# preon7/2019global

Measured on AMD Instinct MI355X. Metric: Mray/s + ms/frame at 1920x1080, depth 8; %HBM roofline, higher is better.
Workload: dtype f64

## Files before the change

### 2019global_amd/__init__.py

```python
from __future__ import annotations

import ctypes
import os
import threading
from typing import Optional, Sequence

import numpy as np

from . import scenes as _scenes

__all__ = [
    "GIError", "lib", "Camera", "Material", "Octree", "ImpSphere", "ImpTriangle", "ExpQuad",
    "ExpSphere", "ExpCube", "ExpCone", "ExpRectangle", "ExpBox",
    "RayTracer", "DeviceScene", "MODE_R", "MODE_X", "STAT_RAYS", "STAT_NODES", "STAT_PRIMS",
    "STAT_PIXELS", "TILE", "MultiScene", "devices_from_env", "obj_entities", "RAY_DOUBLES",
    "AOV_OUTPUTS", "camera_rays", "camera_rays_device",
    "DenoiseParams", "DENOISE_ALBEDO_STOP", "denoise", "denoise_scratch_bytes", "denoise_device",
    "MOMENTS_OUTPUTS", "DenoiseVarParams", "DENOISE_VAR_OUTPUTS", "DENOISE_VAR_SIGMA_V", "DENOISE_VAR_FLOOR",
    "denoise_var", "denoise_var_scratch_bytes", "denoise_var_device",
]

HERE = os.path.dirname(os.path.abspath(__file__))
LIB_PATH = os.environ.get("GI_LIB") or os.path.join(HERE, "libgi.so")

MODE_R, MODE_X = 0, 1
FLAG_STATS = 1
FLAG_R_DFS = 2
FLAG_TIME = 4
FLAG_X_NO_SHADOW = 8
FLAG_X_WF = 16
FLAG_X_MEGA = 32
FLAG_X_SEG = 64
KAT_X_TREE, KAT_X_HBM = 1, 2
X_FORMS = ("k_mode_x", "k_wf_bounce", "k_seg")
R_KERNELS = ("k_mode_r", "k_rf_walk", "k_mode_r_batch")
STAT_RAYS, STAT_NODES, STAT_PRIMS, STAT_PIXELS, STAT_X_PATH_MAX = 0, 1, 2, 3, 4
STAT_X_ITERS, STAT_X_TRAV, STAT_X_HANDLE, STAT_X_HLANES, STAT_X_HCLOSE, STAT_X_HSHADOW = 5, 6, 7, 8, 9, 10
STAT_X_CYC_TRAV, STAT_X_CYC_HIT, STAT_X_CYC_NEXT, STAT_X_CYC_ALL = 11, 12, 13, 14
STAT_X_RESOLVED = 15
STAT_X_IT_NODE, STAT_X_LN_NODE, STAT_X_IT_LEAF, STAT_X_LN_LEAF = 16, 17, 18, 19
STAT_X_IT_RS, STAT_X_LN_RS, STAT_X_IT_ST, STAT_X_LN_ST = 20, 21, 22, 23
STAT_R_PAIRS, STAT_R_OVF_TILES = 24, 25
STATS_N = 26
TILE = 8
ABI_VERSION = 18
RAY_DOUBLES = 8
AOV_OUTPUTS = ("t", "normal", "albedo", "prim", "entity", "uv")
_AOV_KINDS = {"t": (np.float64, ()), "normal": (np.float64, (3,)), "albedo": (np.float64, (3,)),
              "prim": (np.int32, ()), "entity": (np.int32, ()), "uv": (np.int32, (2,))}


class GIError(RuntimeError):
    pass


class EntityDesc(ctypes.Structure):
    _fields_ = [("kind", ctypes.c_int32), ("has_material", ctypes.c_int32), ("args", ctypes.c_double * 11),
                ("mat_color", ctypes.c_double * 3), ("mat_shader", ctypes.c_double * 3),
                ("mat_specular_power", ctypes.c_double), ("mat_reflectivity", ctypes.c_double)]


class SceneDesc(ctypes.Structure):
    _fields_ = [("octree_min", ctypes.c_double * 3), ("octree_max", ctypes.c_double * 3),
                ("n_entities", ctypes.c_int32), ("entities", ctypes.POINTER(EntityDesc))]


class CameraDesc(ctypes.Structure):
    _fields_ = [("pos", ctypes.c_double * 3), ("up", ctypes.c_double * 3), ("forward", ctypes.c_double * 3),
                ("focal", ctypes.c_double)]


class Opts(ctypes.Structure):
    _fields_ = [("mode", ctypes.c_int32), ("spp", ctypes.c_int32), ("depth", ctypes.c_int32),
                ("shard_count", ctypes.c_int32), ("shard_index", ctypes.c_int32), ("band_rows", ctypes.c_int32),
                ("flags", ctypes.c_uint32), ("reserved", ctypes.c_int32), ("seed", ctypes.c_uint64),
                ("stats", ctypes.c_void_p), ("sample_begin", ctypes.c_int32), ("sample_end", ctypes.c_int32)]


class SceneInfo(ctypes.Structure):
    _fields_ = [("n_entities", ctypes.c_int32), ("n_nodes", ctypes.c_int32), ("n_leaves", ctypes.c_int32),
                ("max_depth", ctypes.c_int32), ("n_reachable", ctypes.c_int32), ("n_dropped", ctypes.c_int32),
                ("x_nodes", ctypes.c_int32), ("x_prims", ctypes.c_int32), ("device_bytes", ctypes.c_int64),
                ("x_node_bytes", ctypes.c_int32), ("x_lds_resident", ctypes.c_int32),
                ("x_flat_leaves", ctypes.c_int32), ("x_fan_leaves", ctypes.c_int32)]


class Hit(ctypes.Structure):
    _fields_ = [("entity", ctypes.c_int32), ("u", ctypes.c_int32), ("v", ctypes.c_int32),
                ("point", ctypes.c_double * 3), ("normal", ctypes.c_double * 3)]


class AovFrame(ctypes.Structure):
    _fields_ = [("w", ctypes.c_int32), ("h", ctypes.c_int32), ("x0", ctypes.c_int32), ("y0", ctypes.c_int32),
                ("x1", ctypes.c_int32), ("y1", ctypes.c_int32)]


class Aov(ctypes.Structure):
    _fields_ = [("t", ctypes.c_void_p), ("normal", ctypes.c_void_p), ("albedo", ctypes.c_void_p),
                ("prim", ctypes.c_void_p), ("entity", ctypes.c_void_p), ("uv", ctypes.c_void_p)]


DENOISE_ALBEDO_STOP = 1
DENOISE_OUTPUTS = ("rgb", "rgb8")


class DenoiseParams(ctypes.Structure):
    _fields_ = [("levels", ctypes.c_int32), ("normal_pow_log2", ctypes.c_int32), ("flags", ctypes.c_uint32),
                ("reserved", ctypes.c_int32), ("sigma_c", ctypes.c_double), ("sigma_p", ctypes.c_double)]


class DenoiseIO(ctypes.Structure):
    _fields_ = [("rgb", ctypes.c_void_p), ("t", ctypes.c_void_p), ("normal", ctypes.c_void_p), ("albedo", ctypes.c_void_p),
                ("out_rgb", ctypes.c_void_p), ("out_rgb8", ctypes.c_void_p)]


MOMENTS_OUTPUTS = ("mean", "var", "samples")


class Moments(ctypes.Structure):
    _fields_ = [("mean", ctypes.c_void_p), ("var", ctypes.c_void_p), ("samples", ctypes.c_void_p)]


DENOISE_VAR_OUTPUTS = ("rgb", "var", "rgb8")
DENOISE_VAR_SIGMA_V = 1.0
DENOISE_VAR_FLOOR = 1e-6


class DenoiseVarParams(ctypes.Structure):
    _fields_ = [("levels", ctypes.c_int32), ("normal_pow_log2", ctypes.c_int32), ("flags", ctypes.c_uint32),
                ("reserved", ctypes.c_int32), ("sigma_v", ctypes.c_double), ("sigma_p", ctypes.c_double),
                ("var_floor", ctypes.c_double)]


class DenoiseVarIO(ctypes.Structure):
    _fields_ = [("rgb", ctypes.c_void_p), ("var", ctypes.c_void_p), ("t", ctypes.c_void_p), ("normal", ctypes.c_void_p),
                ("albedo", ctypes.c_void_p), ("out_rgb", ctypes.c_void_p), ("out_var", ctypes.c_void_p),
                ("out_rgb8", ctypes.c_void_p)]


TILE_CB = ctypes.CFUNCTYPE(None, ctypes.c_void_p, ctypes.c_int, ctypes.c_int, ctypes.POINTER(ctypes.c_uint8),
                           ctypes.POINTER(ctypes.c_double))

EXPORTS = ["gi_abi_version", "gi_last_error", "gi_camera_init", "gi_scene_create", "gi_scene_destroy",
           "gi_scene_get_info", "gi_render", "gi_render_device", "gi_shard_tiles", "gi_unshard_device",
           "gi_trace_ray", "gi_kat_expbox", "gi_kat_x_query", "gi_kat_x_variant", "gi_kat_x_texel", "gi_scene_kernel_ms", "gi_scene_x_form", "gi_scene_seg_ring", "gi_scene_r_kernel", "gi_octree_create", "gi_octree_destroy",
           "gi_octree_intersect", "gi_multi_create", "gi_multi_destroy", "gi_multi_info", "gi_multi_render", "gi_device_count",
           "gi_device_list", "gi_build_id", "gi_obj_parse", "gi_intersect", "gi_occluded", "gi_intersect_device",
           "gi_occluded_device", "gi_render_aov", "gi_render_aov_device", "gi_camera_rays", "gi_camera_rays_device",
           "gi_denoise_scratch_bytes", "gi_denoise_device", "gi_denoise",
           "gi_frame_samples_info", "gi_frame_moments_device", "gi_frame_moments",
           "gi_denoise_var_scratch_bytes", "gi_denoise_var_device", "gi_denoise_var"]

_lib = None
_lock = threading.Lock()


def lib():
    global _lib
    with _lock:
        if _lib is not None:
            return _lib
        if not os.path.exists(LIB_PATH):
            raise GIError(f"{LIB_PATH} is missing: run `python 2019global_amd/build.py` (no CPU fallback)")
        try:
            import torch
        except ImportError:
            pass
        L = ctypes.CDLL(LIB_PATH)
        vp, i32, dp = ctypes.c_void_p, ctypes.c_int, ctypes.POINTER(ctypes.c_double)
        L.gi_abi_version.restype = i32
        L.gi_last_error.restype = ctypes.c_char_p
        L.gi_camera_init.argtypes = [dp, dp, ctypes.c_double, ctypes.POINTER(CameraDesc)]
        L.gi_scene_create.argtypes = [ctypes.POINTER(SceneDesc), ctypes.POINTER(vp)]
        L.gi_scene_destroy.argtypes = [vp]
        L.gi_scene_destroy.restype = None
        L.gi_scene_get_info.argtypes = [vp, ctypes.POINTER(SceneInfo)]
        L.gi_render.argtypes = [vp, ctypes.POINTER(CameraDesc), dp, i32, i32, ctypes.POINTER(Opts), dp,
                                ctypes.POINTER(ctypes.c_uint8), ctypes.POINTER(ctypes.c_int), TILE_CB, vp]
        L.gi_render_device.argtypes = [vp, ctypes.POINTER(CameraDesc), dp, i32, i32, ctypes.POINTER(Opts), vp, vp, vp]
        L.gi_shard_tiles.argtypes = [i32, i32, i32]
        L.gi_shard_tiles.restype = ctypes.c_int64
        L.gi_unshard_device.argtypes = [i32, i32, i32, vp, vp, vp, vp, vp]
        L.gi_trace_ray.argtypes = [vp, dp, dp, dp, ctypes.POINTER(Hit), dp]
        L.gi_kat_expbox.argtypes = [i32, dp, ctypes.POINTER(ctypes.c_int32)]
        ip = ctypes.POINTER(ctypes.c_int32)
        L.gi_kat_x_query.argtypes = [vp, i32, dp, dp, i32, ip, dp, ip, ip, ip, dp, ip, dp]
        L.gi_kat_x_variant.argtypes = [vp, i32, ip]
        L.gi_kat_x_texel.argtypes = [vp, i32, dp, i32, dp, ip]
        i64 = ctypes.c_int64
        L.gi_intersect.argtypes = [vp, i64, dp, dp, ip, ip, dp]
        L.gi_occluded.argtypes = [vp, i64, dp, ip]
        L.gi_intersect_device.argtypes = [vp, i64, vp, vp, vp, vp, vp, vp]
        L.gi_occluded_device.argtypes = [vp, i64, vp, vp, vp]
        L.gi_render_aov.argtypes = [vp, ctypes.POINTER(CameraDesc), ctypes.POINTER(AovFrame), ctypes.POINTER(Aov)]
        L.gi_render_aov_device.argtypes = [vp, ctypes.POINTER(CameraDesc), ctypes.POINTER(AovFrame), ctypes.POINTER(Aov), vp]
        L.gi_camera_rays.argtypes = [ctypes.POINTER(CameraDesc), ctypes.POINTER(AovFrame), dp]
        L.gi_camera_rays_device.argtypes = [ctypes.POINTER(CameraDesc), ctypes.POINTER(AovFrame), vp, vp]
        L.gi_denoise_scratch_bytes.argtypes = [ctypes.POINTER(AovFrame), ctypes.POINTER(DenoiseParams)]
        L.gi_denoise_scratch_bytes.restype = ctypes.c_int64
        L.gi_denoise_device.argtypes = [ctypes.POINTER(CameraDesc), ctypes.POINTER(AovFrame), ctypes.POINTER(DenoiseParams),
                                        ctypes.POINTER(DenoiseIO), vp, ctypes.c_int64, vp]
        L.gi_denoise.argtypes = [ctypes.POINTER(CameraDesc), ctypes.POINTER(AovFrame), ctypes.POINTER(DenoiseParams),
                                 ctypes.POINTER(DenoiseIO)]
        L.gi_frame_samples_info.argtypes = [vp, ip, ip, ip, ip]
        L.gi_frame_moments_device.argtypes = [vp, ctypes.POINTER(AovFrame), ctypes.POINTER(Moments), vp]
        L.gi_frame_moments.argtypes = [vp, ctypes.POINTER(AovFrame), ctypes.POINTER(Moments)]
        L.gi_denoise_var_scratch_bytes.argtypes = [ctypes.POINTER(AovFrame), ctypes.POINTER(DenoiseVarParams)]
        L.gi_denoise_var_scratch_bytes.restype = ctypes.c_int64
        L.gi_denoise_var_device.argtypes = [ctypes.POINTER(CameraDesc), ctypes.POINTER(AovFrame), ctypes.POINTER(DenoiseVarParams),
                                            ctypes.POINTER(DenoiseVarIO), vp, ctypes.c_int64, vp]
        L.gi_denoise_var.argtypes = [ctypes.POINTER(CameraDesc), ctypes.POINTER(AovFrame), ctypes.POINTER(DenoiseVarParams),
                                     ctypes.POINTER(DenoiseVarIO)]
        L.gi_scene_kernel_ms.argtypes = [vp, ctypes.POINTER(ctypes.c_float), ctypes.POINTER(ctypes.c_int64)]
        L.gi_scene_x_form.argtypes = [vp, ctypes.POINTER(Opts), ctypes.POINTER(ctypes.c_int32)]
        L.gi_scene_seg_ring.argtypes = [vp, ctypes.POINTER(Opts), ctypes.POINTER(ctypes.c_int32)]
        L.gi_scene_r_kernel.argtypes = [vp, ctypes.POINTER(Opts), ctypes.POINTER(ctypes.c_int32)]
        L.gi_octree_create.argtypes = [ctypes.POINTER(SceneDesc), ctypes.POINTER(vp)]
        L.gi_octree_destroy.argtypes = [vp]
        L.gi_octree_destroy.restype = None
        L.gi_octree_intersect.argtypes = [vp, dp, dp, ctypes.POINTER(ctypes.c_int32), ctypes.c_int64,
                                          ctypes.POINTER(ctypes.c_int64)]
        L.gi_multi_create.argtypes = [ctypes.POINTER(SceneDesc), i32, ctypes.POINTER(ctypes.c_int), ctypes.POINTER(vp)]
        L.gi_multi_destroy.argtypes = [vp]
        L.gi_multi_destroy.restype = None
        L.gi_multi_info.argtypes = [vp, ctypes.POINTER(ctypes.c_int), ctypes.POINTER(ctypes.c_int),
                                    ctypes.POINTER(ctypes.c_int)]
        L.gi_multi_render.argtypes = [vp, ctypes.POINTER(CameraDesc), dp, i32, i32, ctypes.POINTER(Opts), dp,
                                      ctypes.POINTER(ctypes.c_uint8), ctypes.POINTER(ctypes.c_int), TILE_CB, vp]
        L.gi_device_list.argtypes = [ctypes.POINTER(ctypes.c_int32), i32]
        L.gi_build_id.restype = ctypes.c_char_p
        L.gi_obj_parse.argtypes = [ctypes.c_char_p, ctypes.c_int64, ctypes.POINTER(EntityDesc),
                                   ctypes.POINTER(EntityDesc), ctypes.c_int64, ctypes.POINTER(ctypes.c_int64)]
        if L.gi_abi_version() != ABI_VERSION:
            raise GIError(f"libgi ABI {L.gi_abi_version()} != {ABI_VERSION}")
        _lib = L
        return L


def build_id() -> str:
    return lib().gi_build_id().decode()


def _check(rc: int, what: str) -> None:
    if rc != 0:
        raise GIError(f"{what} failed ({rc}): {lib().gi_last_error().decode()}")


def _check_rays(rays) -> int:
    if not isinstance(rays, np.ndarray) or rays.dtype != np.float64 or rays.ndim != 2 or rays.shape[1] != RAY_DOUBLES or \
            not rays.flags.c_contiguous:
        raise ValueError(f"rays: a C-contiguous float64 array of shape (n, {RAY_DOUBLES}) -- o[3], d[3], tmax, reserved")
    return int(rays.shape[0])


def _aov_frame(w, h, window) -> AovFrame:
    def whole(v):
        return isinstance(v, (int, np.integer)) and not isinstance(v, bool)
    if not (whole(w) and whole(h)) or w <= 0 or h <= 0 or w >= 2 ** 31 or h >= 2 ** 31:
        raise ValueError("frame: w and h are positive integers")
    if window is None:
        window = (0, 0, w, h)
    window = tuple(window)
    if len(window) != 4 or not all(whole(v) for v in window):
        raise ValueError("window: four integers (x0, y0, x1, y1)")
    x0, y0, x1, y1 = (int(v) for v in window)
    if not (0 <= x0 <= x1 <= w and 0 <= y0 <= y1 <= h):
        raise ValueError(f"window {window}: reversed or not inside the {w} x {h} frame")
    return AovFrame(int(w), int(h), x0, y0, x1, y1)


def _d3(v) -> ctypes.Array:
    return (ctypes.c_double * 3)(*[float(x) for x in v])


class Material:

    def __init__(self, color, shader=(0.1, 0.7, 1.0), specular_power: float = 5.0, reflectivity: float = 0.0):
        self.color = tuple(float(c) for c in color)
        self.shader_parameters = tuple(float(c) for c in shader)
        self.specular_power = float(specular_power)
        self.reflectivity = float(reflectivity)


class _Entity:
    kind = 0

    def __init__(self, args: Sequence[float], material: Optional[Material]):
        self._args = tuple(float(a) for a in args)
        self._material = material

    @property
    def material(self) -> Optional[Material]:
        return self._material

    @material.setter
    def material(self, m: Material) -> None:
        self._material = m

    def _desc(self, d: EntityDesc) -> None:
        d.kind = self.kind
        for i, a in enumerate(self._args):
            d.args[i] = a
        m = self._material
        d.has_material = 1 if m is not None else 0
        if m is not None:
            for i in range(3):
                d.mat_color[i] = m.color[i]
                d.mat_shader[i] = m.shader_parameters[i]
            d.mat_specular_power = m.specular_power
            d.mat_reflectivity = m.reflectivity


class ImpSphere(_Entity):
    kind = _scenes.IMP_SPHERE

    def __init__(self, pos, radius, color):
        super().__init__((*pos, radius, *color), None)


class ImpTriangle(_Entity):
    kind = _scenes.IMP_TRIANGLE

    def __init__(self, p1, p2, p3):
        super().__init__((*p1, *p2, *p3), None)


class ExpQuad(_Entity):
    kind = _scenes.EXP_QUAD

    def __init__(self, pos, width, length, alpha, color):
        super().__init__((*pos, width, length, alpha, *color), None)


class ExpSphere(_Entity):
    kind = _scenes.EXP_SPHERE

    def __init__(self, pos, radius, color):
        super().__init__((*pos, radius, *color), None)


class ExpCube(_Entity):
    kind = _scenes.EXP_CUBE

    def __init__(self, pos, width, length, height, color):
        super().__init__((*pos, width, length, height, *color), None)


class ExpCone(_Entity):
    kind = _scenes.EXP_CONE

    def __init__(self, pos, dir, height, radius, color):
        super().__init__((*pos, *dir, height, radius, *color), None)


class ExpRectangle(_Entity):
    kind = _scenes.EXP_RECTANGLE

    def __init__(self, p1, p2, p3):
        super().__init__((*p1, *p2, *p3), None)


class ExpBox(_Entity):
    kind = _scenes.EXP_BOX

    def __init__(self, mn, mx):
        super().__init__((*mn, *mx), None)


# ... 39 lines not shown
        if self._host is None or self._host_gen != self.generation:
            self._close_host()
            d, keep = self._scene_desc()
            h = ctypes.c_void_p()
            _check(L.gi_octree_create(ctypes.byref(d), ctypes.byref(h)), "gi_octree_create")
            del keep
            self._host, self._host_gen = h, self.generation
        dv = np.asarray(direction, np.float64)
        dv = dv * (1.0 / np.sqrt((dv[0] * dv[0] + dv[1] * dv[1]) + dv[2] * dv[2]))
        n = ctypes.c_int64()
        _check(L.gi_octree_intersect(self._host, _d3(origin), _d3(dv), None, 0, ctypes.byref(n)), "gi_octree_intersect")
        out = (ctypes.c_int32 * max(1, n.value))()
        _check(L.gi_octree_intersect(self._host, _d3(origin), _d3(dv), out, n.value, ctypes.byref(n)),
               "gi_octree_intersect")
        return [self.entities[i] for i in out[:n.value]]

    def _close_host(self):
        if self._host is not None and self._host.value:
            lib().gi_octree_destroy(self._host)
        self._host = None

    def __del__(self):
        try:
            self._close_host()
        except Exception:
            pass

    @classmethod
    def from_scene(cls, s: "_scenes.Scene") -> "Octree":
        o = cls(s.octree_min, s.octree_max)
        for e in s.entities:
            ent = _Entity(e.args, None if e.material is None else
                          Material(e.material.color, e.material.shader, e.material.specular_power,
                                   e.material.reflectivity))
            ent.kind = e.kind
            o.push_back(ent)
        return o

    def _scene_desc(self):
        n = len(self.entities)
        arr = (EntityDesc * max(n, 1))()
        for i, e in enumerate(self.entities):
            e._desc(arr[i])
        d = SceneDesc()
        d.octree_min = _d3(self.min)
        d.octree_max = _d3(self.max)
        d.n_entities = n
        d.entities = ctypes.cast(arr, ctypes.POINTER(EntityDesc))
        return d, arr


class Camera:

    def __init__(self, pos, lookAt=(0.0, 0.0, 0.0), focal: float = 0.04):
        self._c = CameraDesc()
        _check(lib().gi_camera_init(_d3(pos), _d3(lookAt), float(focal), ctypes.byref(self._c)), "gi_camera_init")

    @property
    def pos(self):
        return tuple(self._c.pos)

    @property
    def up(self):
        return tuple(self._c.up)

    @property
    def forward(self):
        return tuple(self._c.forward)

    @property
    def focalDist(self):
        return self._c.focal


class DeviceScene:

    def __init__(self, octree: Octree):
        L = lib()
        d, keep = octree._scene_desc()
        h = ctypes.c_void_p()
        _check(L.gi_scene_create(ctypes.byref(d), ctypes.byref(h)), "gi_scene_create")
        self._h = h
        del keep

    @classmethod
    def from_scene(cls, s: "_scenes.Scene") -> "DeviceScene":
        return cls(Octree.from_scene(s))

    def close(self) -> None:
        if getattr(self, "_h", None) and self._h.value:
            lib().gi_scene_destroy(self._h)
            self._h = ctypes.c_void_p()

    def __del__(self):
        try:
            self.close()
        except Exception:
            pass

    def info(self) -> dict:
        i = SceneInfo()
        _check(lib().gi_scene_get_info(self._h, ctypes.byref(i)), "gi_scene_get_info")
        return {f: getattr(i, f) for f, _ in SceneInfo._fields_}

    @staticmethod
    def opts(mode=MODE_R, spp=1, depth=1, seed=0, shard_count=1, shard_index=0, band_rows=0, stats_ptr=0,
             flags=0, samples=None) -> Opts:
        o = Opts()
        o.mode, o.spp, o.depth, o.seed = mode, spp, depth, seed
        o.shard_count, o.shard_index, o.band_rows = shard_count, shard_index, band_rows
        o.flags = (FLAG_STATS if stats_ptr else 0) | flags
        o.stats = stats_ptr or None
        if samples is not None:
            o.sample_begin, o.sample_end = samples
        return o

    def render(self, cam: Camera, light, w: int, h: int, mode=MODE_R, spp=1, depth=1, seed=0, band_rows=0,
               cancel: Optional[ctypes.c_int] = None, callback=None, out=None, flags=0, samples=None):
        if out is None:
            rgb, rgb8 = np.zeros((h, w, 3), np.float64), np.zeros((h, w, 3), np.uint8)
        else:
            rgb, rgb8 = out
        for a, dt in ((rgb, np.float64), (rgb8, np.uint8)):
            if a is not None and (a.dtype != dt or a.size != w * h * 3 or not a.flags.c_contiguous):
                raise ValueError("render: out arrays must be C-contiguous [h, w, 3] float64 / uint8")
        cb = TILE_CB(callback) if callback is not None else TILE_CB()
        o = self.opts(mode, spp, depth, seed, band_rows=band_rows, flags=flags, samples=samples)
        _check(lib().gi_render(self._h, ctypes.byref(cam._c), _d3(light), w, h, ctypes.byref(o),
                               rgb.ctypes.data_as(ctypes.POINTER(ctypes.c_double)) if rgb is not None else None,
                               rgb8.ctypes.data_as(ctypes.POINTER(ctypes.c_uint8)) if rgb8 is not None else None,
                               ctypes.byref(cancel) if cancel is not None else None, cb, None), "gi_render")
        return rgb, rgb8

    def render_device(self, cam: Camera, light, w: int, h: int, d_rgb: int, d_rgb8: int = 0, stream: int = 0,
                      mode=MODE_R, spp=1, depth=1, seed=0, shard_count=1, shard_index=0, stats_ptr=0,
                      flags=0, samples=None) -> None:
        o = self.opts(mode, spp, depth, seed, shard_count, shard_index, stats_ptr=stats_ptr, flags=flags,
                      samples=samples)
        _check(lib().gi_render_device(self._h, ctypes.byref(cam._c), _d3(light), w, h, ctypes.byref(o),
                                      d_rgb or None, d_rgb8 or None, stream or None), "gi_render_device")

    def x_form(self, mode=MODE_X, spp=1, depth=1, flags=0) -> str:
        o = self.opts(mode, spp, depth, 0, flags=flags)
        f = ctypes.c_int32()
        _check(lib().gi_scene_x_form(self._h, ctypes.byref(o), ctypes.byref(f)), "gi_scene_x_form")
        return X_FORMS[f.value]

    def seg_ring(self, mode=MODE_X, spp=1, depth=1, flags=0) -> bool:
        o = self.opts(mode, spp, depth, 0, flags=flags)
        f = ctypes.c_int32()
        _check(lib().gi_scene_seg_ring(self._h, ctypes.byref(o), ctypes.byref(f)), "gi_scene_seg_ring")
        return bool(f.value)

    def r_kernel(self, flags=0) -> str:
        o = self.opts(MODE_R, 1, 1, 0, flags=flags)
        k = ctypes.c_int32()
        _check(lib().gi_scene_r_kernel(self._h, ctypes.byref(o), ctypes.byref(k)), "gi_scene_r_kernel")
        return R_KERNELS[k.value]

    def kernel_ms(self):
        ms, n = ctypes.c_float(), ctypes.c_int64()
        _check(lib().gi_scene_kernel_ms(self._h, ctypes.byref(ms), ctypes.byref(n)), "gi_scene_kernel_ms")
        return float(ms.value), int(n.value)

    def trace_ray(self, origin, direction, light):
        hit = Hit()
        rgb = (ctypes.c_double * 3)()
        _check(lib().gi_trace_ray(self._h, _d3(origin), _d3(direction), _d3(light), ctypes.byref(hit), rgb),
               "gi_trace_ray")
        return hit, tuple(rgb)

    INTERSECT_OUTPUTS = ("t", "prim", "entity", "normal")

    def intersect(self, rays: np.ndarray, want=INTERSECT_OUTPUTS) -> dict:
        n = _check_rays(rays)
        want = tuple(want)
        if not want or any(k not in self.INTERSECT_OUTPUTS for k in want) or len(set(want)) != len(want):
            raise ValueError(f"intersect: want is a non-empty selection of {self.INTERSECT_OUTPUTS}")
        m = max(n, 1)
        bufs = {"t": np.empty(m, np.float64), "prim": np.empty(m, np.int32), "entity": np.empty(m, np.int32),
                "normal": np.empty((m, 3), np.float64)}
        ip, dp = ctypes.POINTER(ctypes.c_int32), ctypes.POINTER(ctypes.c_double)
        ptr = {k: (bufs[k].ctypes.data_as(dp if bufs[k].dtype == np.float64 else ip) if k in want else None)
               for k in self.INTERSECT_OUTPUTS}
        _check(lib().gi_intersect(self._h, n, rays.ctypes.data_as(dp), ptr["t"], ptr["prim"], ptr["entity"], ptr["normal"]),
               "gi_intersect")
        return {k: bufs[k][:n] for k in want}

    def occluded(self, rays: np.ndarray) -> np.ndarray:
        n = _check_rays(rays)
        out = np.empty(max(n, 1), np.int32)
        _check(lib().gi_occluded(self._h, n, rays.ctypes.data_as(ctypes.POINTER(ctypes.c_double)),
                                 out.ctypes.data_as(ctypes.POINTER(ctypes.c_int32))), "gi_occluded")
        return out[:n]

    def intersect_device(self, n: int, d_rays: int, d_t: int = 0, d_prim: int = 0, d_entity: int = 0, d_normal: int = 0,
                         stream: int = 0) -> None:
        _check(lib().gi_intersect_device(self._h, int(n), d_rays or None, d_t or None, d_prim or None, d_entity or None,
                                         d_normal or None, stream or None), "gi_intersect_device")

    def occluded_device(self, n: int, d_rays: int, d_occluded: int, stream: int = 0) -> None:
        _check(lib().gi_occluded_device(self._h, int(n), d_rays or None, d_occluded or None, stream or None),
               "gi_occluded_device")

    def render_aov(self, cam: "Camera", w: int, h: int, window=None, want=AOV_OUTPUTS) -> dict:
        want = tuple(want)
        if not want or any(k not in AOV_OUTPUTS for k in want) or len(set(want)) != len(want):
            raise ValueError(f"render_aov: want is a non-empty selection of {AOV_OUTPUTS}")
        f = _aov_frame(w, h, window)
        rows, cols = f.y1 - f.y0, f.x1 - f.x0
        bufs = {k: np.empty((rows, cols) + _AOV_KINDS[k][1], _AOV_KINDS[k][0]) for k in want}
        a = Aov(**{k: bufs[k].ctypes.data if bufs[k].size else _scratch_ptr() for k in want})
        _check(lib().gi_render_aov(self._h, ctypes.byref(cam._c), ctypes.byref(f), ctypes.byref(a)), "gi_render_aov")
        return bufs

    def render_aov_device(self, cam: "Camera", w: int, h: int, window=None, d_t: int = 0, d_normal: int = 0,
                          d_albedo: int = 0, d_prim: int = 0, d_entity: int = 0, d_uv: int = 0, stream: int = 0) -> None:
        f = _aov_frame(w, h, window)
        a = Aov(d_t or None, d_normal or None, d_albedo or None, d_prim or None, d_entity or None, d_uv or None)
        _check(lib().gi_render_aov_device(self._h, ctypes.byref(cam._c), ctypes.byref(f), ctypes.byref(a), stream or None),
               "gi_render_aov_device")

    def frame_samples_info(self) -> dict:
        v = [ctypes.c_int32() for _ in range(4)]
        _check(lib().gi_frame_samples_info(self._h, *(ctypes.byref(x) for x in v)), "gi_frame_samples_info")
        return dict(zip(("w", "h", "n", "spp"), (int(x.value) for x in v)))

    def frame_moments(self, w: int, h: int, window=None, want=("mean", "var")) -> dict:
        want = tuple(want)
        if not want or any(k not in MOMENTS_OUTPUTS for k in want) or len(set(want)) != len(want):
            raise ValueError(f"frame_moments: want is a non-empty selection of {MOMENTS_OUTPUTS}")
        f = _aov_frame(w, h, window)
        rows, cols = f.y1 - f.y0, f.x1 - f.x0
        n = self.frame_samples_info()["n"] if "samples" in want else 0
        bufs = {k: np.empty((rows, cols, n, 3) if k == "samples" else (rows, cols, 3), np.float64) for k in want}
        m = Moments(**{k: bufs[k].ctypes.data if bufs[k].size else _scratch_ptr() for k in want})
        _check(lib().gi_frame_moments(self._h, ctypes.byref(f), ctypes.byref(m)), "gi_frame_moments")
        return bufs

    def frame_moments_device(self, w: int, h: int, window=None, d_mean: int = 0, d_var: int = 0, d_samples: int = 0,
                             stream: int = 0) -> None:
        f = _aov_frame(w, h, window)
        m = Moments(d_mean or None, d_var or None, d_samples or None)
        _check(lib().gi_frame_moments_device(self._h, ctypes.byref(f), ctypes.byref(m), stream or None), "gi_frame_moments_device")

    def kat_x_variant(self, flags: int = 0) -> dict:
        out = (ctypes.c_int32 * 6)()
        _check(lib().gi_kat_x_variant(self._h, int(flags), out), "gi_kat_x_variant")
        return dict(zip(("LDS", "W4", "SH", "TRI", "CN", "FLAT"), (bool(v) for v in out)))

    def kat_x_query(self, recs: np.ndarray, cam_pos, flags: int = 0) -> dict:
        recs = np.ascontiguousarray(recs, np.float64).reshape(-1, 12)
        n = recs.shape[0]
        out = dict(prim1=np.zeros(n, np.int32), t1=np.zeros(n), occl=np.zeros(n, np.int32), skip_s=np.zeros(n, np.int32),
                   prim2=np.zeros(n, np.int32), t2=np.zeros(n), skip2=np.zeros(n, np.int32))
        sc = ctypes.c_double(float("nan"))
        ip, dp = ctypes.POINTER(ctypes.c_int32), ctypes.POINTER(ctypes.c_double)
        _check(lib().gi_kat_x_query(self._h, n, recs.ctypes.data_as(dp), _d3(cam_pos), int(flags),
                                    out["prim1"].ctypes.data_as(ip), out["t1"].ctypes.data_as(dp),
                                    out["occl"].ctypes.data_as(ip), out["skip_s"].ctypes.data_as(ip),
                                    out["prim2"].ctypes.data_as(ip), out["t2"].ctypes.data_as(dp),
                                    out["skip2"].ctypes.data_as(ip), ctypes.byref(sc)), "gi_kat_x_query")
        out["skip_cos"] = sc.value if n else None
        return out

    def kat_x_texel(self, ents, points, exact: bool = False):
        pts = np.ascontiguousarray(points, np.float64).reshape(-1, 3)
        n = pts.shape[0]
        recs = np.empty((n, 4), np.float64)
        recs[:, 0] = np.asarray(ents, np.float64).reshape(n)
        recs[:, 1:] = pts
        tex, how = np.zeros((n, 3)), np.zeros(n, np.int32)
        ip, dp = ctypes.POINTER(ctypes.c_int32), ctypes.POINTER(ctypes.c_double)
        _check(lib().gi_kat_x_texel(self._h, n, recs.ctypes.data_as(dp), 1 if exact else 0, tex.ctypes.data_as(dp),
                                    how.ctypes.data_as(ip)), "gi_kat_x_texel")
        return tex, how


_scratch = None


def _scratch_ptr() -> int:
    global _scratch
    if _scratch is None:
        _scratch = np.zeros(8)
    return _scratch.ctypes.data


def camera_rays(cam: "Camera", w: int, h: int, window=None) -> np.ndarray:
    f = _aov_frame(w, h, window)
    rays = np.empty(((f.y1 - f.y0) * (f.x1 - f.x0), RAY_DOUBLES), np.float64)
    p = rays.ctypes.data_as(ctypes.POINTER(ctypes.c_double)) if rays.size else \
        ctypes.cast(_scratch_ptr(), ctypes.POINTER(ctypes.c_double))
    _check(lib().gi_camera_rays(ctypes.byref(cam._c), ctypes.byref(f), p), "gi_camera_rays")
    return rays


def camera_rays_device(cam: "Camera", w: int, h: int, d_rays: int, window=None, stream: int = 0) -> None:
    f = _aov_frame(w, h, window)
    _check(lib().gi_camera_rays_device(ctypes.byref(cam._c), ctypes.byref(f), d_rays or None, stream or None),
           "gi_camera_rays_device")


def _denoise_params(levels, sigma_c, sigma_p, normal_pow_log2, albedo_stop) -> DenoiseParams:
    return DenoiseParams(int(levels), int(normal_pow_log2), DENOISE_ALBEDO_STOP if albedo_stop else 0, 0, float(sigma_c),
                         float(sigma_p))
# ... 254 lines not shown
```

### 2019global_amd/csrc/gi_build.cpp

```cpp
#include <algorithm>
#include <cmath>
#include <cstdlib>
#include <cstring>
#include <string>

#include "gi.h"
#include "gi_fan_pair.h"
#include "gi_scene.h"

namespace gi {

namespace {

struct BEnt {
    REnt rec;
    V3 bmin, bmax;
    std::vector<TriRec> tris;
};

REnt blank_rec(int kind) {
    REnt r;
    memset(&r, 0, sizeof r);
    r.kind = kind;
    r.color[0] = 1; r.color[1] = 0; r.color[2] = 0;
// ... 280 lines not shown
    void push_obj(int ni, int32_t e) {
        nodes[ni].ents.push_back(e);
        partition(ni);
        if (nodes[ni].child0 < 0) return;
        const BEnt& E = (*ents)[e];
        for (int c = 0; c < 8; ++c) {
            const int ci = nodes[ni].child0 + c;
            if (le3(nodes[ci].mn, E.bmin) && le3(E.bmax, nodes[ci].mx)) push_obj(ci, e);
            else if (bb_overlap(nodes[ci].mn, nodes[ci].mx, E.bmin, E.bmax)) nodes[ci].ents.push_back(e);
        }
    }
};

struct Box {
    double mn[3], mx[3];
};
const int XLEAF_MAX = 4;
const int XMAX_DEPTH = 12;

bool tri_box_overlap(const double* c, const double* hs, const XPrim& p) {
    double v[3][3];
    for (int k = 0; k < 3; ++k) {
        v[0][k] = p.a[k] - c[k];
        v[1][k] = p.a[k] + p.b[k] - c[k];
        v[2][k] = p.a[k] + p.c[k] - c[k];
    }
    for (int k = 0; k < 3; ++k) {
        const double mn = std::min(std::min(v[0][k], v[1][k]), v[2][k]);
        const double mx = std::max(std::max(v[0][k], v[1][k]), v[2][k]);
        if (mn > hs[k] || mx < -hs[k]) return false;
    }
    double e[3][3];
    for (int k = 0; k < 3; ++k) {
        e[0][k] = v[1][k] - v[0][k];
        e[1][k] = v[2][k] - v[1][k];
        e[2][k] = v[0][k] - v[2][k];
    }
    for (int i = 0; i < 3; ++i)
        for (int j = 0; j < 3; ++j) {
            double a[3] = {0, 0, 0};
            const int j1 = (j + 1) % 3, j2 = (j + 2) % 3;
            a[j1] = -e[i][j2];
            a[j2] = e[i][j1];
            const double p0 = a[0] * v[0][0] + a[1] * v[0][1] + a[2] * v[0][2];
            const double p1 = a[0] * v[1][0] + a[1] * v[1][1] + a[2] * v[1][2];
            const double p2 = a[0] * v[2][0] + a[1] * v[2][1] + a[2] * v[2][2];
            const double r = hs[0] * std::fabs(a[0]) + hs[1] * std::fabs(a[1]) + hs[2] * std::fabs(a[2]);
            const double mn = std::min(std::min(p0, p1), p2), mx = std::max(std::max(p0, p1), p2);
            if (mn > r * (1 + 1e-12) || mx < -r * (1 + 1e-12)) return false;
        }
    const double n[3] = {e[0][1] * e[1][2] - e[0][2] * e[1][1], e[0][2] * e[1][0] - e[0][0] * e[1][2],
                         e[0][0] * e[1][1] - e[0][1] * e[1][0]};
    const double d = n[0] * v[0][0] + n[1] * v[0][1] + n[2] * v[0][2];
    const double r = hs[0] * std::fabs(n[0]) + hs[1] * std::fabs(n[1]) + hs[2] * std::fabs(n[2]);
    return std::fabs(d) <= r * (1 + 1e-12);
}

bool prim_box_overlap(const XPrim& p, const double* mn, const double* mx) {
    double c[3], hs[3];
    for (int k = 0; k < 3; ++k) { c[k] = 0.5 * (mn[k] + mx[k]); hs[k] = 0.5 * (mx[k] - mn[k]); }
    if (p.kind == 0) return tri_box_overlap(c, hs, p);
    double d2 = 0;
    for (int k = 0; k < 3; ++k) {
        const double q = std::max(mn[k] - p.a[k], std::max(0.0, p.a[k] - mx[k]));
        d2 += q * q;
    }
    return d2 <= p.b[0] * p.b[0] * (1 + 1e-12);
}

struct XBuild {
    const std::vector<Box>* pb;
    const std::vector<XPrim>* prims;
    std::vector<XNode>* out;
    std::vector<int32_t>* idx;
    double pad;
    int max_depth = 0;
    int leaf_max = XLEAF_MAX;

    static bool overlap(const Box& a, const Box& b) {
        for (int k = 0; k < 3; ++k)
            if (a.mx[k] < b.mn[k] || b.mx[k] < a.mn[k]) return false;
        return true;
    }
    Box tight(const Box& cell, const std::vector<int32_t>& prims) const {
        Box u;
        for (int k = 0; k < 3; ++k) { u.mn[k] = INFINITY; u.mx[k] = -INFINITY; }
        for (int32_t p : prims)
            for (int k = 0; k < 3; ++k) {
                u.mn[k] = std::min(u.mn[k], (*pb)[p].mn[k]);
                u.mx[k] = std::max(u.mx[k], (*pb)[p].mx[k]);
            }
        Box t;
        for (int k = 0; k < 3; ++k) {
            t.mn[k] = std::max(cell.mn[k], u.mn[k]) - pad;
            t.mx[k] = std::min(cell.mx[k], u.mx[k]) + pad;
        }
        return t;
    }
    void build(int ni, const Box& cell, std::vector<int32_t>& prims, int depth) {
        max_depth = std::max(max_depth, depth);
        const Box tb = tight(cell, prims);
        XNode& n0 = (*out)[ni];
        for (int k = 0; k < 3; ++k) { n0.mn[k] = tb.mn[k]; n0.mx[k] = tb.mx[k]; }
        n0.child_base = -1; n0.child_mask = 0; n0.prim_off = 0; n0.prim_cnt = 0;
        std::vector<int32_t> kids[8];
        Box cb[8];
        bool split = (int)prims.size() > leaf_max && depth < XMAX_DEPTH;
        if (split) {
            double mid[3];
            for (int k = 0; k < 3; ++k) mid[k] = 0.5 * (cell.mn[k] + cell.mx[k]);
            bool progress = false;
            for (int c = 0; c < 8; ++c) {
                for (int k = 0; k < 3; ++k) {
                    const bool hi = (c >> k) & 1;
                    cb[c].mn[k] = hi ? mid[k] : cell.mn[k];
                    cb[c].mx[k] = hi ? cell.mx[k] : mid[k];
                }
                Box test = cb[c];
                for (int k = 0; k < 3; ++k) { test.mn[k] -= pad; test.mx[k] += pad; }
                for (int32_t p : prims)
                    if (overlap(test, (*pb)[p]) && prim_box_overlap((*this->prims)[p], test.mn, test.mx)) kids[c].push_back(p);
                if (!kids[c].empty() && kids[c].size() < prims.size()) progress = true;
            }
            split = progress;
        }
        if (!split) {
            XNode& n = (*out)[ni];
            n.prim_off = (int32_t)idx->size();
            n.prim_cnt = (int32_t)prims.size();
            idx->insert(idx->end(), prims.begin(), prims.end());
            return;
        }
        int mask = 0, cnt = 0;
        for (int c = 0; c < 8; ++c)
            if (!kids[c].empty()) { mask |= 1 << c; ++cnt; }
        const int base = (int)out->size();
        out->resize(out->size() + cnt);
        (*out)[ni].child_base = base;
        (*out)[ni].child_mask = mask;
        std::vector<int32_t>().swap(prims);
        int k = 0;
        for (int c = 0; c < 8; ++c)
            if (!kids[c].empty()) build(base + k++, cb[c], kids[c], depth + 1);
    }
};

constexpr int kXNoPlane = 255;
void assign_plane_groups(HostScene& hs) {
    const size_t np = hs.xprims.size();
    hs.x_skip_a = 0.0;
    hs.x_skip_b = 2.0;
    for (XPrim& p : hs.xprims) p.pad[0] = kXNoPlane;
    for (XWNode& w : hs.xwnodes) memset(w.pad, 0xFF, sizeof w.pad);
    double E = 0.0;
    for (const XPrim& p : hs.xprims)
        for (int k = 0; k < 3; ++k) {
            if (p.kind == 1) {
                E = std::max(E, std::fabs(p.a[k]) + std::fabs(p.b[0]));
            } else {
                E = std::max(E, std::fabs(p.a[k]));
                E = std::max(E, std::fabs(p.a[k] + p.b[k]));
                E = std::max(E, std::fabs(p.a[k] + p.c[k]));
            }
        }
    struct G {
        V3 n;
        double off;
    };
    std::vector<G> groups;
    double s_min = 1.0, tau = 0.0;
    const double tol = 1e-12 * std::max(E, 1.0);
    for (size_t i = 0; i < np; ++i) {
        XPrim& p = hs.xprims[i];
        if (p.kind != 0) continue;
        const V3 v0 = ld3(p.a), e1 = ld3(p.b), e2 = ld3(p.c), e3 = e2 - e1;
        const V3 cr = cross(e1, e2);
        const double area2 = std::sqrt(dot(cr, cr)), l1 = std::sqrt(dot(e1, e1)), l2 = std::sqrt(dot(e2, e2)),
                     l3 = std::sqrt(dot(e3, e3));
        if (!(area2 > 0.0) || !std::isfinite(area2)) continue;
        const double s = std::min(std::min(area2 / (l1 * l2), area2 / (l1 * l3)), area2 / (l2 * l3));
        if (!(s >= 1e-3)) continue;
        V3 n = cr * (1.0 / area2);
        if (n.x < 0 || (n.x == 0 && (n.y < 0 || (n.y == 0 && n.z < 0)))) n = -n;
        const V3 vs[3] = {v0, v0 + e1, v0 + e2};
        int g = -1;
        double dev = 0.0;
        for (size_t k = 0; k < groups.size() && g < 0; ++k) {
            const V3 dn = n - groups[k].n;
            if (std::max(std::fabs(dn.x), std::max(std::fabs(dn.y), std::fabs(dn.z))) > 1e-12) continue;
            double m = 0.0;
            for (const V3& v : vs) m = std::max(m, std::fabs(dot(groups[k].n, v) - groups[k].off));
            if (m <= tol) {
                g = (int)k;
                dev = m;
            }
        }
        if (g < 0) {
            if (groups.size() >= 254) continue;
            groups.push_back(G{n, dot(n, v0)});
            g = (int)groups.size() - 1;
            for (const V3& v : vs) dev = std::max(dev, std::fabs(dot(n, v) - groups[g].off));
        }
        p.pad[0] = g;
        tau = std::max(tau, dev);
        s_min = std::min(s_min, s);
    }
    if (groups.empty()) return;
    for (XWNode& w : hs.xwnodes) {
        uint8_t* b = reinterpret_cast<uint8_t*>(w.pad);
        for (int c = 0; c < 8; ++c) {
            if (w.child[c] >= 0 || w.child[c] == XEMPTY || w.cnt[c] == 0) continue;
            int g = hs.xprims[hs.xhot[~w.child[c]].prim].pad[0];
            for (int j = 1; j < w.cnt[c] && g != kXNoPlane; ++j)
                if (hs.xprims[hs.xhot[~w.child[c] + j].prim].pad[0] != g) g = kXNoPlane;
            b[c] = (uint8_t)g;
        }
    }
    const double K = 2000.0, u = 0x1.0p-53, tmin = 1e-7;
    hs.x_skip_a = K * u / (s_min * tmin);
    hs.x_skip_b = K * (4.0 * u * E / s_min + tau + 4.0 * u * E) / tmin;
}

}

void build_xflat(HostScene& hs) {
    hs.xflat.clear();
    hs.n_fan_leaves = 0;
    bool ok = true;
    for (const XWNode& w : hs.xwnodes) {
        const uint8_t* g = reinterpret_cast<const uint8_t*>(w.pad);
        for (int c = 0; c < 8; ++c) {
            if (w.child[c] >= 0 || w.child[c] == XEMPTY) continue;
            XFlatLeaf f;
            for (int k = 0; k < 3; ++k) { f.lo[k] = w.lo[k][c]; f.hi[k] = w.hi[k][c]; }
            f.off = ~w.child[c];
            f.cnt = w.cnt[c];
            f.group = g[c];
            f.fan = (f.cnt == 2 && fan_pair_ok(hs.xhot[(size_t)f.off], hs.xhot[(size_t)f.off + 1])) ? 1 : 0;
            hs.n_fan_leaves += f.fan;
            ok = ok && f.cnt <= 255 && f.off < 65536;
            hs.xflat.push_back(f);
        }
    }
    hs.x_flat_ok = ok && hs.xflat.size() <= (size_t)GI_XFLAT_MAX;
    hs.x_fan_all = !hs.xflat.empty() && (size_t)hs.n_fan_leaves == hs.xflat.size();
}

bool build_host_scene(const gi_scene_desc& desc, HostScene& hs, std::string& err) {
    std::vector<BEnt> ents((size_t)desc.n_entities);
    for (int i = 0; i < desc.n_entities; ++i)
        if (!build_entity(desc.entities[i], ents[i], err)) return false;

    hs.ents.clear();
    hs.tris.clear();
    for (BEnt& e : ents) {
        e.rec.tri_first = (int32_t)hs.tris.size();
        e.rec.tri_count = (int32_t)e.tris.size();
        hs.tris.insert(hs.tris.end(), e.tris.begin(), e.tris.end());
        hs.ents.push_back(e.rec);
    }

    RBuild rb;
    rb.ents = &ents;
    RBuild::N root;
    root.mn = v3(desc.octree_min[0], desc.octree_min[1], desc.octree_min[2]);
    root.mx = v3(desc.octree_max[0], desc.octree_max[1], desc.octree_max[2]);
    rb.nodes.push_back(root);
    hs.n_dropped = 0;
    for (int32_t i = 0; i < desc.n_entities; ++i) {
        if (!bb_overlap(rb.nodes[0].mn, rb.nodes[0].mx, ents[i].bmin, ents[i].bmax)) { ++hs.n_dropped; continue; }
        rb.push_obj(0, i);
    }
    const size_t nn = rb.nodes.size();
    hs.rnodes.assign(nn, RNode());
    hs.leaf_ents.clear();
    std::vector<int32_t> depth(nn, 0);
    std::vector<char> reach((size_t)desc.n_entities, 0);
    hs.n_leaves = 0;
    hs.max_depth = 0;
    for (size_t i = 0; i < nn; ++i) {
        const RBuild::N& s = rb.nodes[i];
        RNode& d = hs.rnodes[i];
        st3(d.mn, s.mn);
        st3(d.mx, s.mx);
        d.child0 = s.child0;
        if (i == 0) d.parent = -1;
        d.ent_cnt = (int32_t)s.ents.size();
        d.ent_off = -1;
        if (s.child0 < 0) {
            d.ent_off = (int32_t)hs.leaf_ents.size();
            hs.leaf_ents.insert(hs.leaf_ents.end(), s.ents.begin(), s.ents.end());
            for (int32_t e : s.ents) reach[e] = 1;
            ++hs.n_leaves;
        } else {
            for (int c = 0; c < 8; ++c) {
                hs.rnodes[s.child0 + c].parent = (int32_t)i;
                depth[s.child0 + c] = depth[i] + 1;
            }
        }
        hs.max_depth = std::max(hs.max_depth, depth[i]);
    }
    hs.n_reachable = 0;
    for (char r : reach) hs.n_reachable += r;
    build_rcand(hs);

    hs.xprims.clear();
    std::vector<Box> pb;
    for (int32_t i = 0; i < desc.n_entities; ++i) {
        const REnt& r = hs.ents[i];
        if (r.kind == K_IMP_SPHERE) {
            XPrim p;
            memset(&p, 0, sizeof p);
            p.kind = 1; p.ent = i;
            p.a[0] = r.pos[0]; p.a[1] = r.pos[1]; p.a[2] = r.pos[2];
            p.b[0] = (double)r.radius;
            hs.xprims.push_back(p);
            Box b;
            for (int k = 0; k < 3; ++k) { b.mn[k] = r.pos[k] - (double)r.radius; b.mx[k] = r.pos[k] + (double)r.radius; }
            pb.push_back(b);
        } else {
            for (int t = 0; t < r.tri_count; ++t) {
                const TriRec& tr = hs.tris[r.tri_first + t];
                XPrim p;
                memset(&p, 0, sizeof p);
                p.kind = 0; p.ent = i;
                const V3 p1 = ld3(tr.p1), e1 = ld3(tr.p2) - p1, e2 = ld3(tr.p3) - p1;
                st3(p.a, p1); st3(p.b, e1); st3(p.c, e2);
                for (int k = 0; k < 3; ++k) p.n[k] = tr.n[k];
                hs.xprims.push_back(p);
                Box b;
                for (int k = 0; k < 3; ++k) {
                    b.mn[k] = std::min(std::min(tr.p1[k], tr.p2[k]), tr.p3[k]);
                    b.mx[k] = std::max(std::max(tr.p1[k], tr.p2[k]), tr.p3[k]);
                }
                pb.push_back(b);
            }
        }
    }
    hs.xnodes.clear();
    hs.xprim_idx.clear();
    const char* accel = std::getenv("GI_XACCEL");
    if (!(accel && std::string(accel) == "octree")) {
        std::vector<double> bounds(6 * pb.size());
        for (size_t i = 0; i < pb.size(); ++i)
            for (int k = 0; k < 3; ++k) { bounds[6 * i + k] = pb[i].mn[k]; bounds[6 * i + 3 + k] = pb[i].mx[k]; }
        int leaf_max = 4;
        if (const char* lm = std::getenv("GI_XLEAF_MAX")) leaf_max = std::max(1, std::atoi(lm));
        build_xbvh(hs.xprims, bounds, leaf_max, hs, true);
        assign_plane_groups(hs);
        build_xflat(hs);
        return true;
    }
    hs.xnodes.resize(1);
    Box rootb;
    for (int k = 0; k < 3; ++k) { rootb.mn[k] = INFINITY; rootb.mx[k] = -INFINITY; }
    for (const Box& b : pb)
        for (int k = 0; k < 3; ++k) { rootb.mn[k] = std::min(rootb.mn[k], b.mn[k]); rootb.mx[k] = std::max(rootb.mx[k], b.mx[k]); }
    if (pb.empty()) {
        for (int k = 0; k < 3; ++k) { rootb.mn[k] = 0; rootb.mx[k] = 0; }
    }
    double ext = 1.0;
    for (int k = 0; k < 3; ++k) ext = std::max(ext, std::max(std::fabs(rootb.mn[k]), std::fabs(rootb.mx[k])));
    XBuild xb;
    xb.pb = &pb;
    xb.prims = &hs.xprims;
    xb.out = &hs.xnodes;
    xb.idx = &hs.xprim_idx;
    xb.pad = 1e-9 * ext;
    if (const char* lm = std::getenv("GI_XLEAF_MAX")) xb.leaf_max = std::max(1, std::atoi(lm));
    std::vector<int32_t> all(pb.size());
    for (size_t i = 0; i < pb.size(); ++i) all[i] = (int32_t)i;
    if (pb.empty()) {
        XNode& n = hs.xnodes[0];
        memset(&n, 0, sizeof n);
        n.mn[0] = n.mn[1] = n.mn[2] = 1.0;
        n.mx[0] = n.mx[1] = n.mx[2] = -1.0;
        n.child_base = -1;
    } else {
        xb.build(0, rootb, all, 0);
    }
    hs.x_max_depth = xb.max_depth;

    double pad32 = 1e-5 * ext;
    auto lo32 = [&](double v) {
        float f = (float)(v - pad32);
        if ((double)f > v - pad32) f = std::nextafter(f, -INFINITY);
        return f;
    };
    auto hi32 = [&](double v) {
        float f = (float)(v + pad32);
        if ((double)f < v + pad32) f = std::nextafter(f, INFINITY);
        return f;
    };
    const size_t nx = hs.xnodes.size();
    std::vector<int32_t> ref(nx, 0);
    int32_t nwide = 0, nleaf = 0;
    for (size_t i = 0; i < nx; ++i) {
        if (hs.xnodes[i].child_mask != 0) ref[i] = nwide++;
// ... 73 lines not shown
```

### 2019global_amd/csrc/gi_capi.cpp

```cpp
#include <hip/hip_runtime_api.h>

#include <algorithm>
#include <cmath>
#include <cstring>
#include <memory>
#include <mutex>
#include <new>
#include <string>
#include <vector>

#include "gi.h"
#include "gi_internal.h"
#include "gi_launch.h"
#include "gi_scene.h"

using namespace gi;

struct HostPath {
    static constexpr int kSlots = 2;
    hipStream_t render = nullptr, copy = nullptr;
    hipEvent_t rendered[kSlots] = {}, copied[kSlots] = {};
    double* d_rgb[kSlots] = {};
    uint8_t* d_rgb8[kSlots] = {};
    double* h_rgb[kSlots] = {};
// ... 326 lines not shown
    const V3 fwd = v3(c.forward[0], c.forward[1], c.forward[2]);
    d.rx = 0.0002;
    d.ry = 0.0002;
    d.left = normalize(cross(d.up, fwd));
    d.top_left = (((d.pos + c.focal * fwd) + ((d.left * (double)w) * 0.5) * d.rx) + ((d.up * (double)w) * 0.5) * d.ry) - d.pos;
    return d;
}

int check_opts(int w, int h, const gi_opts* o) {
    if (!o) return fail(GI_ERR_ARG, "null opts");
    if (w <= 0 || h <= 0 || (int64_t)w * h > (int64_t)1 << 34) return fail(GI_ERR_ARG, "bad frame size");
    if (o->mode != GI_MODE_R && o->mode != GI_MODE_X) return fail(GI_ERR_ARG, "bad mode");
    if (o->shard_count < 1 || o->shard_index < 0 || o->shard_index >= o->shard_count) return fail(GI_ERR_ARG, "bad shard");
    if (o->mode == GI_MODE_X && (o->spp < 1 || o->depth < 1 || o->depth > 0xFFFF))
        return fail(GI_ERR_ARG, "mode X needs spp >= 1, 1 <= depth <= 65535");
    if ((o->flags & GI_FLAG_STATS) && !o->stats) return fail(GI_ERR_ARG, "GI_FLAG_STATS without stats buffer");
    if ((o->sample_begin != 0 || o->sample_end != 0) &&
        (o->mode != GI_MODE_X || o->spp < 2 || o->sample_begin < 0 || o->sample_begin >= o->sample_end || o->sample_end > o->spp))
        return fail(GI_ERR_ARG, "progressive pass: mode X, spp > 1, 0 <= sample_begin < sample_end <= spp");
    return GI_OK;
}

namespace {
uint64_t prog_key(const gi_camera& c, const double light[3], int w, int h, const gi_opts& o) {
    uint64_t k = 1469598103934665603ull;
    auto mix = [&](const void* p, size_t n) {
        for (size_t i = 0; i < n; ++i) k = (k ^ static_cast<const unsigned char*>(p)[i]) * 1099511628211ull;
    };
    mix(&c, sizeof c);
    mix(light, 3 * sizeof(double));
    const int64_t v[8] = {w, h, o.spp, o.depth, (int64_t)o.seed, o.shard_count, o.shard_index,
                          (int64_t)(o.flags & ~(GI_FLAG_STATS | GI_FLAG_TIME))};
    mix(v, sizeof v);
    return k;
}
int prog_check(gi_scene* s, const gi_camera& c, const double light[3], int w, int h, const gi_opts& o) {
    if (o.sample_end == 0) {
        s->prog_next = -1;
        return GI_OK;
    }
    const uint64_t key = prog_key(c, light, w, h, o);
    if (o.sample_begin > 0 && s->prog_next == o.sample_begin && s->launched) {
        const hipError_t e = hipEventQuery(s->last);
        if (e != hipSuccess && e != hipErrorNotReady) {
            s->prog_next = -1;
            return hip_fail(e, "progressive pass: the previous pass failed on the device; restart the frame at sample 0");
        }
    }
    if (o.sample_begin > 0 && (s->prog_next != o.sample_begin || s->prog_key != key)) {
        s->prog_next = -1;
        return fail(GI_ERR_ARG, "progressive pass out of order: a pass continues the previous pass's frame "
                                "(same camera, light, size, spp, depth, seed, shard) from its sample_end");
    }
    s->prog_key = key;
    s->prog_next = -1;
    return GI_OK;
}
void prog_done(gi_scene* s, const gi_opts& o) {
    s->prog_next = (o.sample_end > 0 && o.sample_end < o.spp) ? o.sample_end : -1;
}
void keep_frame(gi_scene* s, const CamDev& cd, int w, int h, const gi_opts& o) {
    if (o.mode != GI_MODE_X || o.spp < 2 || o.shard_count != 1) return;
    s->keep_w = w;
    s->keep_h = h;
    s->keep_n = o.sample_end > 0 ? o.sample_end : o.spp;
    s->keep_spp = o.spp;
    s->keep_cam = cd;
}
}

int band_rows_of(const gi_opts* o, int h) {
    int band = o->band_rows > 0 ? o->band_rows : h;
    band = ((band + GI_TILE - 1) / GI_TILE) * GI_TILE;
    return std::min(band, ((h + GI_TILE - 1) / GI_TILE) * GI_TILE);
}

int scene_create_on(const gi_scene_desc* desc, int device, gi_scene** out) {
    *out = nullptr;
    int rc = bind_device(device);
    if (rc || (rc = check_device(device))) return rc;
    std::unique_ptr<gi_scene, void (*)(gi_scene*)> s(new gi_scene(), [](gi_scene* p) { destroy_scene(p); });
    s->device = device;
    std::string err;
    if (!build_host_scene(*desc, s->host, err)) return fail(GI_ERR_SCENE, err);
    DevScene& d = s->dev;
    memset(&d, 0, sizeof d);
    const HostScene& h = s->host;
    hipError_t e;
    gi_scene* sp = s.get();
    if ((e = upload(sp, h.rnodes, &d.rnodes)) != hipSuccess || (e = upload(sp, h.leaf_ents, &d.leaf_ents)) != hipSuccess ||
        (e = upload(sp, h.ents, &d.ents)) != hipSuccess || (e = upload(sp, h.tris, &d.tris)) != hipSuccess ||
        (e = upload(sp, h.xwnodes, &d.xwnodes)) != hipSuccess || (e = upload(sp, h.xhot, &d.xhot)) != hipSuccess ||
        (e = upload(sp, h.xbox, &d.xbox)) != hipSuccess ||
        (e = upload(sp, h.xprims, &d.xprims)) != hipSuccess || (e = upload(sp, h.xflat, &d.xflat)) != hipSuccess ||
        (e = upload(sp, std::vector<unsigned>(16, 0u), const_cast<const unsigned**>(&d.work))) != hipSuccess ||
        (e = upload(sp, h.app_off, &d.app_off)) != hipSuccess || (e = upload(sp, h.app_rec, &d.app_rec)) != hipSuccess ||
        (e = upload(sp, h.rpath_rec, &d.rpath_rec)) != hipSuccess || (e = upload(sp, h.rc_nodes, &d.rc_nodes)) != hipSuccess ||
        (e = upload(sp, h.rc_ent, &d.rc_ent)) != hipSuccess || (e = upload(sp, h.rc_maxkey, &d.rc_maxkey)) != hipSuccess ||
        (e = upload(sp, h.r_always, &d.r_always)) != hipSuccess ||
        (e = upload(sp, h.r_leaf_of_rank, &d.r_leaf_of_rank)) != hipSuccess)
        return hip_fail(e, "scene upload");
    d.n_rnodes = (int32_t)h.rnodes.size();
    d.n_ents = (int32_t)h.ents.size();
    d.n_xwnodes = (int32_t)h.xwnodes.size();
    d.n_xprims = (int32_t)h.xprims.size();
    d.x_max_depth = h.x_max_depth;
    d.x_handle8 = h.x_handle8;
    d.x_flags = h.x_flags;
    d.x_skip_a = h.x_skip_a;
    d.x_skip_b = h.x_skip_b;
    d.n_xhot = (int32_t)h.xhot.size();
    d.n_r_always = (int32_t)h.r_always.size();
    d.rc_ext = (float)h.rc_ext;
    {
        const size_t bytes = h.xwnodes.size() * sizeof(XWNode) + h.xhot.size() * sizeof(XHot) +
                             h.xprims.size() * sizeof(XPrim) + h.ents.size() * sizeof(REnt);
        d.x_lds_bytes = bytes <= 40 * 1024 ? (int32_t)bytes : 0;
        d.n_xflat = (int32_t)h.xflat.size();
        d.x_flat = (d.x_lds_bytes > 0 && h.x_flat_ok) ? 1 : 0;
        d.x_fan = (d.x_flat && h.x_fan_all && x_env().fan) ? 1 : 0;
        const size_t per_wg = bytes + 256 * 10 * sizeof(double) + 4 * 68 * sizeof(unsigned);
        d.x_waves4 = (d.x_lds_bytes > 0 && 4 * per_wg <= 160 * 1024) ? 1 : 0;
        d.x_tri_only = 1;
        for (const REnt& r : h.ents)
            if (r.kind == K_IMP_SPHERE || r.kind == K_EXP_SPHERE || r.kind == K_EXP_CONE || r.kind == K_EXP_RECTANGLE) {
                d.x_waves4 = 0;
                d.x_tri_only = 0;
            }
        for (const XPrim& xp : h.xprims)
            if (xp.kind != 0) d.x_tri_only = 0;
        d.r_tri_only = 1;
        for (const REnt& r : h.ents)
            if (r.kind != K_IMP_TRIANGLE) d.r_tri_only = 0;
    }
    const bool want_cn = h.xwnodes.size() * sizeof(XWNode) > (size_t)2 << 20;
    if (d.x_lds_bytes == 0 && want_cn && encode_xcnodes(h.xwnodes, s->host.xcnodes) &&
        (e = upload(sp, h.xcnodes, &d.xcnodes)) != hipSuccess)
        return hip_fail(e, "scene upload (quantised nodes)");
    for (int k = 0; k < 3; ++k) { d.root_lo[k] = INFINITY; d.root_hi[k] = -INFINITY; }
    if (!h.xwnodes.empty())
        for (int c = 0; c < 8; ++c)
            if (h.xwnodes[0].child[c] != XEMPTY)
                for (int k = 0; k < 3; ++k) {
                    d.root_lo[k] = std::min(d.root_lo[k], h.xwnodes[0].lo[k][c]);
                    d.root_hi[k] = std::max(d.root_hi[k], h.xwnodes[0].hi[k][c]);
                }
    d.x_far_r = INFINITY;
    for (int k = 0; k < 3; ++k)
        if (d.root_lo[k] <= d.root_hi[k]) {
            const float m = 16.0f * std::max(std::fabs(d.root_lo[k]), std::fabs(d.root_hi[k]));
            d.x_far_r = std::isinf(d.x_far_r) ? m : std::max(d.x_far_r, m);
        }
    if ((e = x_launch_config(d, device, s->xcfg)) != hipSuccess) return hip_fail(e, "occupancy query");
    *out = s.release();
    return GI_OK;
}

void scene_destroy(gi_scene* s) noexcept { destroy_scene(s); }
int scene_device(const gi_scene* s) { return s->device; }
std::mutex& scene_mutex(gi_scene* s) { return s->mu; }

int scene_render_band(gi_scene* s, const CamDev& cd, const double light[3], int w, int h, int y0, const gi_opts& o,
                      double* d_rgb, uint8_t* d_rgb8, hipStream_t stream, bool timer) {
    s->keep_n = 0;
    int rc = bind_device(s->device);
    if (rc || (rc = ensure_xscratch(s, w, h, &o)) || (timer && (rc = ensure_timer(s, &o)))) return rc;
    return issue_render(s, cd, v3(light[0], light[1], light[2]), w, h, y0, o, d_rgb, d_rgb8, stream, timer);
}

int unshard(int w, int h, int n, const double* packed, const uint8_t* packed8, double* rgb, uint8_t* rgb8,
            hipStream_t stream) {
    const hipError_t e = launch_unshard(w, h, n, packed, packed8, rgb, rgb8, stream);
    return e == hipSuccess ? GI_OK : hip_fail(e, "unshard launch");
}

}

extern "C" {

int gi_abi_version(void) { return GI_ABI_VERSION; }
const char* gi_last_error(void) { return g_err.c_str(); }

int gi_device_list(int32_t* out, int cap) {
    int ndev = 0, n = 0;
    if (hipGetDeviceCount(&ndev) != hipSuccess) return 0;
    for (int d = 0; d < ndev; ++d) {
        hipDeviceProp_t prop;
        if (hipGetDeviceProperties(&prop, d) == hipSuccess && std::strncmp(prop.gcnArchName, "gfx950", 6) == 0) {
            if (out && n < cap) out[n] = d;
            ++n;
        }
    }
    return n;
}

int gi_device_count(void) { return gi_device_list(nullptr, 0); }

#ifndef GI_BUILD_ID
#define GI_BUILD_ID "unknown"
#endif
const char* gi_build_id(void) { return GI_BUILD_ID; }

int gi_camera_init(const double pos[3], const double look_at[3], double focal, gi_camera* out) {
    if (!pos || !look_at || !out) return fail(GI_ERR_ARG, "null argument");
    const V3 p = v3(pos[0], pos[1], pos[2]);
    const V3 f = normalize(v3(look_at[0], look_at[1], look_at[2]) - p);
    st3(out->pos, p);
    out->up[0] = 0; out->up[1] = 0; out->up[2] = 1.0;
    st3(out->forward, f);
    out->focal = focal;
    return GI_OK;
}

int gi_scene_create(const gi_scene_desc* desc, gi_scene** out) {
    return guard([&]() -> int {
        if (!desc || !out || desc->n_entities < 0 || (desc->n_entities > 0 && !desc->entities))
            return fail(GI_ERR_ARG, "bad scene descriptor");
        *out = nullptr;
        int ndev = 0;
        hipError_t e = hipGetDeviceCount(&ndev);
        if (e != hipSuccess || ndev <= 0) return fail(GI_ERR_DEVICE, "no HIP device (libgi renders only on gfx950)");
        int dev = 0;
        if ((e = hipGetDevice(&dev)) != hipSuccess) return hip_fail(e, "hipGetDevice");
        return scene_create_on(desc, dev, out);
    });
}

void gi_scene_destroy(gi_scene* s) { destroy_scene(s); }

int gi_scene_get_info(const gi_scene* s, gi_scene_info* info) {
    if (!s || !info) return fail(GI_ERR_ARG, "null argument");
    info->n_entities = (int32_t)s->host.ents.size();
    info->n_nodes = (int32_t)s->host.rnodes.size();
    info->n_leaves = s->host.n_leaves;
    info->max_depth = s->host.max_depth;
    info->n_reachable = s->host.n_reachable;
    info->n_dropped = s->host.n_dropped;
    info->x_nodes = (int32_t)(s->host.xnodes.empty() ? s->host.xwnodes.size() : s->host.xnodes.size());
    info->x_prims = (int32_t)s->host.xprims.size();
    info->device_bytes = s->bytes;
    info->x_node_bytes = s->dev.xcnodes ? (int32_t)sizeof(XCNode) : (int32_t)sizeof(XWNode);
    info->x_lds_resident = s->dev.x_lds_bytes > 0 ? 1 : 0;
    info->x_flat_leaves = (int32_t)s->host.xflat.size();
    info->x_fan_leaves = s->host.n_fan_leaves;
    return GI_OK;
}

int64_t gi_shard_tiles(int w, int h, int shard_count) {
    if (w <= 0 || h <= 0 || shard_count < 1) return -1;
    return shard_tiles(w, h, shard_count);
}

int gi_render_device(gi_scene* s, const gi_camera* cam, const double light[3], int w, int h, const gi_opts* o,
                     double* d_rgb, uint8_t* d_rgb8, void* stream) {
    return guard([&]() -> int {
        DeviceRestore keep;
        if (!s) return fail(GI_ERR_ARG, "null scene");
        std::lock_guard<std::mutex> lk(s->mu);
        s->keep_n = 0;
        int rc = check_opts(w, h, o);
        if (rc) return rc;
        if (!cam || !light) return fail(GI_ERR_ARG, "null camera or light");
        if ((rc = prog_check(s, *cam, light, w, h, *o))) return rc;
        const CamDev cd = make_cam(*cam, w);
        rc = scene_render_band(s, cd, light, w, h, 0, *o, d_rgb, d_rgb8, static_cast<hipStream_t>(stream), true);
        if (rc == GI_OK) {
            prog_done(s, *o);
            keep_frame(s, cd, w, h, *o);
        }
        return rc;
    });
}

int gi_render(gi_scene* s, const gi_camera* cam, const double light[3], int w, int h, const gi_opts* o, double* rgb,
              uint8_t* rgb8, const volatile int* cancel, gi_tile_cb cb, void* user) {
    return guard([&]() -> int {
        DeviceRestore keep;
        if (!s) return fail(GI_ERR_ARG, "null scene");
        std::lock_guard<std::mutex> lk(s->mu);
        s->keep_n = 0;
        int rc = check_opts(w, h, o);
        if (rc) return rc;
        if (!cam || !light) return fail(GI_ERR_ARG, "null camera or light");
        if (o->shard_count != 1) return fail(GI_ERR_ARG, "gi_render renders whole frames; use gi_render_device or gi_multi to shard");
        if ((rc = bind_device(s->device))) return rc;
        const int band = band_rows_of(o, h);
        const size_t band_px = (size_t)w * (size_t)band;
        const int n_bands = (h + band - 1) / band;
        if (o->sample_end > 0 && n_bands > 1)
            return fail(GI_ERR_ARG, "progressive passes render whole frames: band_rows 0 or >= h");
        if ((rc = prog_check(s, *cam, light, w, h, *o))) return rc;
        if ((rc = ensure_hostpath(s, band_px, std::min(n_bands, HostPath::kSlots)))) return rc;
        HostPath& hp = s->hp;
        const CamDev cd = make_cam(*cam, w);
        const bool want_rgb = rgb || cb, want_rgb8 = rgb8 || cb;
        const bool direct = n_bands == 1;
        double* const dst_rgb = direct && rgb ? rgb : hp.h_rgb[0];
        uint8_t* const dst_rgb8 = direct && rgb8 ? rgb8 : hp.h_rgb8[0];
        auto issue = [&](int i) -> int {
            const int k = i % HostPath::kSlots, y0 = i * band, rows = std::min(band, h - y0);
            const size_t n = (size_t)w * rows * 3;
            hipError_t e = hipSuccess;
            if (i >= HostPath::kSlots && (e = hipStreamWaitEvent(hp.render, hp.copied[k], 0)) != hipSuccess)
                return hip_fail(e, "render");
            const int r = scene_render_band(s, cd, light, w, rows, y0, *o, hp.d_rgb[k], hp.d_rgb8[k], hp.render, false);
            if (r) return r;
            e = hipEventRecord(hp.rendered[k], hp.render);
            if (e == hipSuccess) e = hipStreamWaitEvent(hp.copy, hp.rendered[k], 0);
            double* const to = i == 0 ? dst_rgb : hp.h_rgb[k];
            uint8_t* const to8 = i == 0 ? dst_rgb8 : hp.h_rgb8[k];
            if (e == hipSuccess && want_rgb) e = hipMemcpyAsync(to, hp.d_rgb[k], n * sizeof(double), hipMemcpyDeviceToHost, hp.copy);
            if (e == hipSuccess && want_rgb8) e = hipMemcpyAsync(to8, hp.d_rgb8[k], n, hipMemcpyDeviceToHost, hp.copy);
            if (e == hipSuccess) e = hipEventRecord(hp.copied[k], hp.copy);
            return e == hipSuccess ? GI_OK : hip_fail(e, "render");
        };
        hipError_t e = hipSuccess;
        if (cancel && *cancel) rc = fail(GI_ERR_CANCELLED, "cancelled");
        else rc = issue(0);
        for (int i = 0; rc == GI_OK && i < n_bands; i++) {
            if (i + 1 < n_bands) {
                if (cancel && *cancel) { rc = fail(GI_ERR_CANCELLED, "cancelled"); break; }
                if ((rc = issue(i + 1)) != GI_OK) break;
            }
            const int k = i % HostPath::kSlots, y0 = i * band, rows = std::min(band, h - y0);
            const size_t n = (size_t)w * rows * 3;
            if ((e = hipEventSynchronize(hp.copied[k])) != hipSuccess) { rc = hip_fail(e, "render"); break; }
            const double* hr = i == 0 ? dst_rgb : hp.h_rgb[k];
            const uint8_t* hr8 = i == 0 ? dst_rgb8 : hp.h_rgb8[k];
            if (rgb && hr != rgb) { std::memcpy(rgb + (size_t)y0 * w * 3, hr, n * sizeof(double)); hr = rgb + (size_t)y0 * w * 3; }
            if (rgb8 && hr8 != rgb8) { std::memcpy(rgb8 + (size_t)y0 * w * 3, hr8, n); hr8 = rgb8 + (size_t)y0 * w * 3; }
            if (cb) cb(user, y0, rows, hr8, hr);
        }
        const hipError_t e1 = hipStreamSynchronize(hp.render), e2 = hipStreamSynchronize(hp.copy);
        if (rc == GI_OK && (e1 != hipSuccess || e2 != hipSuccess)) rc = hip_fail(e1 != hipSuccess ? e1 : e2, "render");
        if (rc == GI_OK) prog_done(s, *o);
        if (rc == GI_OK && n_bands == 1) keep_frame(s, cd, w, h, *o);
        else s->keep_n = 0;
        return rc;
    });
}

int gi_scene_kernel_ms(gi_scene* s, float* avg_ms, int64_t* n) {
    return guard([&]() -> int {
        DeviceRestore keep;
        if (!s || !avg_ms) return fail(GI_ERR_ARG, "null argument");
        std::lock_guard<std::mutex> lk(s->mu);
        KTimer& kt = s->kt;
        if (kt.recorded == 0) return fail(GI_ERR_ARG, "no render issued with GI_FLAG_TIME since the last read");
        int rc = bind_device(s->device);
        if (rc) return rc;
        const long long first = kt.recorded > KTimer::kRing ? kt.recorded - KTimer::kRing : 0;
        for (long long r = std::max(first, kt.folded); r < kt.recorded; r++) {
            const hipError_t e = fold_timer(kt, (int)(r % KTimer::kRing));
            if (e != hipSuccess) return hip_fail(e, "gi_scene_kernel_ms");
        }
        *avg_ms = (float)(kt.sum_ms / (double)kt.folded);
        if (n) *n = kt.folded;
        kt.recorded = 0;
        kt.folded = 0;
        kt.sum_ms = 0.0;
        return GI_OK;
    });
}

int gi_scene_x_form(gi_scene* s, const gi_opts* o, int32_t* form) {
    return guard([&]() -> int {
        if (!s || !o || !form) return fail(GI_ERR_ARG, "null argument");
        std::lock_guard<std::mutex> lk(s->mu);
        *form = x_form_choice(s->dev, s->xcfg, *o);
        return GI_OK;
    });
}

int gi_scene_seg_ring(gi_scene* s, const gi_opts* o, int32_t* on) {
    return guard([&]() -> int {
        if (!s || !o || !on) return fail(GI_ERR_ARG, "null argument");
        std::lock_guard<std::mutex> lk(s->mu);
        *on = (x_form_choice(s->dev, s->xcfg, *o) == XFORM_SEG && s->xcfg.seg_ring) ? 1 : 0;
        return GI_OK;
    });
}

int gi_scene_r_kernel(gi_scene* s, const gi_opts* o, int32_t* kernel) {
    return guard([&]() -> int {
        if (!s || !o || !kernel) return fail(GI_ERR_ARG, "null argument");
        std::lock_guard<std::mutex> lk(s->mu);
        *kernel = r_kernel_choice(s->dev, *o);
        if (*kernel == RK_FLAT && s->xs.rf_failed > 0 && s->xs.rf_slots == 0) *kernel = RK_BATCH;
        return GI_OK;
    });
}

int gi_unshard_device(int w, int h, int shard_count, const double* d_packed, const uint8_t* d_packed8, double* d_rgb,
                      uint8_t* d_rgb8, void* stream) {
    return guard([&]() -> int {
        if (w <= 0 || h <= 0 || shard_count < 1) return fail(GI_ERR_ARG, "bad unshard arguments");
        if ((d_rgb && !d_packed) || (d_rgb8 && !d_packed8)) return fail(GI_ERR_ARG, "missing packed input");
        return unshard(w, h, shard_count, d_packed, d_packed8, d_rgb, d_rgb8, static_cast<hipStream_t>(stream));
    });
}

int gi_trace_ray(gi_scene* s, const double origin[3], const double dir[3], const double light[3], gi_hit* hit,
                 double rgb[3]) {
    return guard([&]() -> int {
        DeviceRestore keep;
        if (!s || !origin || !dir || !light || !hit || !rgb) return fail(GI_ERR_ARG, "null argument");
        std::lock_guard<std::mutex> lk(s->mu);
        int rc = bind_device(s->device);
        if (rc) return rc;
        int32_t* d_i = nullptr;
        double* d_d = nullptr;
        hipError_t e;
        if ((e = hipMalloc((void**)&d_i, 4 * sizeof(int32_t))) != hipSuccess) return hip_fail(e, "hipMalloc");
        if ((e = hipMalloc((void**)&d_d, 9 * sizeof(double))) != hipSuccess) { (void)hipFree(d_i); return hip_fail(e, "hipMalloc"); }
        const V3 o = v3(origin[0], origin[1], origin[2]);
        const V3 d = normalize(v3(dir[0], dir[1], dir[2]));
        e = launch_trace_ray(s->dev, o, d, v3(light[0], light[1], light[2]), d_i, d_d, nullptr);
        int32_t hi[3] = {-1, 0, 0};
        double hd[9] = {0};
        if (e == hipSuccess) e = hipMemcpy(hi, d_i, 3 * sizeof(int32_t), hipMemcpyDeviceToHost);
        if (e == hipSuccess) e = hipMemcpy(hd, d_d, 9 * sizeof(double), hipMemcpyDeviceToHost);
        (void)hipFree(d_i);
        (void)hipFree(d_d);
        if (e != hipSuccess) return hip_fail(e, "trace_ray");
        hit->entity = hi[0];
        hit->u = hi[1];
        hit->v = hi[2];
        for (int k = 0; k < 3; ++k) { hit->point[k] = hd[k]; hit->normal[k] = hd[3 + k]; rgb[k] = hd[6 + k]; }
        return GI_OK;
    });
}

namespace {
int check_ray_args(const gi_scene* s, int64_t n, const double* rays) {
    if (!s) return fail(GI_ERR_ARG, "null scene");
    if (n < 0) return fail(GI_ERR_ARG, "negative ray count");
    if (n > 0 && !rays) return fail(GI_ERR_ARG, "null rays");
    return GI_OK;
}
int ray_query_device(gi_scene* s, bool any, const CastIO& io, hipStream_t stream) {
    if (reinterpret_cast<uintptr_t>(io.rays) & 15) return fail(GI_ERR_ARG, "device ray records must be 16-byte aligned");
    int rc = bind_device(s->device);
    if (rc) return rc;
    const hipError_t e = launch_cast(s->dev, x_query_cfg(s->xcfg, 0, any ? WK_OCCL : WK_CAST), any, io, stream);
    return e == hipSuccess ? GI_OK : hip_fail(e, any ? "gi_occluded launch" : "gi_intersect launch");
}
struct DevBuf {
    void* p = nullptr;
    ~DevBuf() { (void)hipFree(p); }
    hipError_t alloc(size_t bytes) { return hipMalloc(&p, bytes); }
};
}

int gi_intersect_device(gi_scene* s, int64_t n, const double* d_rays, double* d_t, int32_t* d_prim, int32_t* d_entity,
                        double* d_normal, void* stream) {
    return guard([&]() -> int {
        DeviceRestore keep;
        int rc = check_ray_args(s, n, d_rays);
        if (rc) return rc;
        if (!d_t && !d_prim && !d_entity && !d_normal) return fail(GI_ERR_ARG, "gi_intersect: every output is null");
        if (n == 0) return GI_OK;
        return ray_query_device(s, false, CastIO{d_rays, (long long)n, d_t, d_prim, d_entity, d_normal, nullptr},
                                static_cast<hipStream_t>(stream));
    });
}

int gi_occluded_device(gi_scene* s, int64_t n, const double* d_rays, int32_t* d_occluded, void* stream) {
    return guard([&]() -> int {
        DeviceRestore keep;
        int rc = check_ray_args(s, n, d_rays);
        if (rc) return rc;
        if (!d_occluded) return fail(GI_ERR_ARG, "gi_occluded: null output");
        if (n == 0) return GI_OK;
        return ray_query_device(s, true, CastIO{d_rays, (long long)n, nullptr, nullptr, nullptr, nullptr, d_occluded},
                                static_cast<hipStream_t>(stream));
    });
}

int gi_intersect(gi_scene* s, int64_t n, const double* rays, double* t, int32_t* prim, int32_t* entity, double* normal) {
    return guard([&]() -> int {
        DeviceRestore keep;
        int rc = check_ray_args(s, n, rays);
        if (rc) return rc;
        if (!t && !prim && !entity && !normal) return fail(GI_ERR_ARG, "gi_intersect: every output is null");
        if (n == 0) return GI_OK;
        if ((rc = bind_device(s->device))) return rc;
        const size_t m = (size_t)n;
        DevBuf dr, dt, dp, de, dn;
        hipError_t e = dr.alloc(m * GI_RAY_DOUBLES * sizeof(double));
        if (e == hipSuccess && t) e = dt.alloc(m * sizeof(double));
        if (e == hipSuccess && prim) e = dp.alloc(m * sizeof(int32_t));
        if (e == hipSuccess && entity) e = de.alloc(m * sizeof(int32_t));
        if (e == hipSuccess && normal) e = dn.alloc(m * 3 * sizeof(double));
        if (e != hipSuccess) return hip_fail(e, "hipMalloc (ray query staging)");
        if ((e = hipMemcpy(dr.p, rays, m * GI_RAY_DOUBLES * sizeof(double), hipMemcpyHostToDevice)) != hipSuccess)
            return hip_fail(e, "gi_intersect");
        rc = ray_query_device(s, false, CastIO{static_cast<const double*>(dr.p), (long long)n, static_cast<double*>(dt.p),
                                               static_cast<int32_t*>(dp.p), static_cast<int32_t*>(de.p),
                                               static_cast<double*>(dn.p), nullptr}, nullptr);
        if (rc) return rc;
        if (t) e = hipMemcpy(t, dt.p, m * sizeof(double), hipMemcpyDeviceToHost);
        if (e == hipSuccess && prim) e = hipMemcpy(prim, dp.p, m * sizeof(int32_t), hipMemcpyDeviceToHost);
        if (e == hipSuccess && entity) e = hipMemcpy(entity, de.p, m * sizeof(int32_t), hipMemcpyDeviceToHost);
        if (e == hipSuccess && normal) e = hipMemcpy(normal, dn.p, m * 3 * sizeof(double), hipMemcpyDeviceToHost);
        return e == hipSuccess ? GI_OK : hip_fail(e, "gi_intersect");
    });
}

int gi_occluded(gi_scene* s, int64_t n, const double* rays, int32_t* occluded) {
    return guard([&]() -> int {
        DeviceRestore keep;
        int rc = check_ray_args(s, n, rays);
        if (rc) return rc;
        if (!occluded) return fail(GI_ERR_ARG, "gi_occluded: null output");
        if (n == 0) return GI_OK;
        if ((rc = bind_device(s->device))) return rc;
        const size_t m = (size_t)n;
        DevBuf dr, dc;
        hipError_t e = dr.alloc(m * GI_RAY_DOUBLES * sizeof(double));
        if (e == hipSuccess) e = dc.alloc(m * sizeof(int32_t));
        if (e != hipSuccess) return hip_fail(e, "hipMalloc (ray query staging)");
        if ((e = hipMemcpy(dr.p, rays, m * GI_RAY_DOUBLES * sizeof(double), hipMemcpyHostToDevice)) != hipSuccess)
            return hip_fail(e, "gi_occluded");
        rc = ray_query_device(s, true, CastIO{static_cast<const double*>(dr.p), (long long)n, nullptr, nullptr, nullptr, nullptr,
                                              static_cast<int32_t*>(dc.p)}, nullptr);
        if (rc) return rc;
// ... 490 lines not shown
```

### 2019global_amd/csrc/gi_kernels.hip

```cpp
#include <hip/hip_runtime.h>

#include <algorithm>
#include <cfloat>
#include <cmath>
#include <cstdlib>
#include <mutex>

#include "gi.h"
#include "gi_dev.h"
#include "gi_launch.h"
#include "gi_scene.h"

namespace gi {

namespace {

enum : int { PH_CLOSEST = 0, PH_SHADOW = 1, PH_NEED = 2, PH_START = 3, PH_DEAD = 4, PH_DONEPX = 5, PH_HELP = 6 };

#ifndef GI_X_START_BURST
#define GI_X_START_BURST 16
#endif
#ifndef GI_X_MIN_WAVES
#define GI_X_MIN_WAVES 3
#endif
// ... 787 lines not shown
    const double* mine = s_row + lane * kMomRow;
    const double n = (double)a.n;
    double sa = 0, sb = 0, sc = 0, ma = 0, mb = 0, mc = 0;
    double* out = (a.samples && o >= 0) ? a.samples + 3 * (size_t)o * (size_t)a.n : nullptr;
    for (int pass = 0; pass < 2; ++pass) {
        if (pass == 1 && !a.var && !a.samples) break;
        for (int s0 = 0; s0 < a.n; s0 += kMomChunk) {
            const unsigned cn = (unsigned)(a.n - s0 < kMomChunk ? a.n - s0 : kMomChunk), per = 3u * cn, total = cnt * per;
            for (unsigned e = lane; e < total; e += 64u) {
                const unsigned px = e / per, k = e - px * per;
                s_row[px * kMomRow + k] = rows[3 * ((size_t)px * (size_t)a.spp + (size_t)s0) + k];
            }
            __syncthreads();
            if (o >= 0) {
                for (unsigned k = 0; k < cn; ++k) {
                    const double x0 = mine[3 * k], x1 = mine[3 * k + 1], x2 = mine[3 * k + 2];
                    if (pass == 0) {
                        sa = sa + x0;
                        sb = sb + x1;
                        sc = sc + x2;
                    } else {
                        const double da = x0 - ma, db = x1 - mb, dc = x2 - mc;
                        sa = sa + da * da;
                        sb = sb + db * db;
                        sc = sc + dc * dc;
                        if (out) { out[3 * (s0 + k)] = x0; out[3 * (s0 + k) + 1] = x1; out[3 * (s0 + k) + 2] = x2; }
                    }
                }
            }
            __syncthreads();
        }
        if (pass == 0) {
            ma = sa / n; mb = sb / n; mc = sc / n;
            if (o >= 0) moments_store(a, o, ma, mb, mc, 0, 0, 0, false);
            sa = sb = sc = 0;
        } else if (o >= 0) {
            moments_store(a, o, 0, 0, 0, sa, sb, sc, true);
        }
    }
}
#endif

__global__ __launch_bounds__(256) void k_x_moments_fill(DevScene sc, CamDev cam, XMoments a) {
    const long long n_px = (long long)a.cols * (long long)a.rows;
    for (long long o = (long long)blockIdx.x * blockDim.x + threadIdx.x; o < n_px; o += (long long)gridDim.x * blockDim.x) {
        const int y = (int)(o / a.cols), x = (int)(o - (long long)y * a.cols);
        if (!pixel_misses_box(cam, x + a.x0, y + a.y0, sc.root_lo, sc.root_hi)) continue;
        if (a.mean) { a.mean[3 * o] = 0; a.mean[3 * o + 1] = 0; a.mean[3 * o + 2] = 0; }
        if (a.var) { a.var[3 * o] = 0; a.var[3 * o + 1] = 0; a.var[3 * o + 2] = 0; }
        if (a.samples) {
            double* out = a.samples + 3 * (size_t)o * (size_t)a.n;
            for (int k = 0; k < 3 * a.n; ++k) out[k] = 0;
        }
    }
}

__global__ __launch_bounds__(256) void k_unshard(TileMap m, const double* packed, const uint8_t* packed8, double* rgb,
                                                  uint8_t* rgb8) {
    const long long i = (long long)blockIdx.x * blockDim.x + threadIdx.x;
    const long long t = i / (kTile * kTile);
    if (t >= m.n_tiles) return;
    const int lane = (int)(i % (kTile * kTile));
    const int ty = (int)(t / m.tiles_x), tx = (int)(t % m.tiles_x);
    const int x = tx * kTile + (lane & 7), y = ty * kTile + (lane >> 3);
    if (x >= m.w || y >= m.h) return;
    const long long r = t % m.shard_count, lt = t / m.shard_count;
    const long long src = (r * m.n_local + lt) * (kTile * kTile) + lane;
    const long long dst = (long long)y * m.w + x;
    if (rgb) { rgb[3 * dst] = packed[3 * src]; rgb[3 * dst + 1] = packed[3 * src + 1]; rgb[3 * dst + 2] = packed[3 * src + 2]; }
    if (rgb8) { rgb8[3 * dst] = packed8[3 * src]; rgb8[3 * dst + 1] = packed8[3 * src + 1]; rgb8[3 * dst + 2] = packed8[3 * src + 2]; }
}


}

long long shard_tiles(int w, int h, int shard_count) { return make_map(w, h, shard_count, 0).n_local; }

const XEnv& x_env() {
    static XEnv env;
    static std::once_flag once;
    std::call_once(once, [] {
        if (const char* v = std::getenv("GI_X_HELP")) env.help = std::atoi(v) != 0;
        if (const char* v = std::getenv("GI_X_FLAT")) env.flat = std::atoi(v) != 0;
        if (const char* v = std::getenv("GI_X_FAN")) env.fan = std::atoi(v) != 0;
        if (const char* v = std::getenv("GI_SEG_RING")) env.seg_ring = std::atoi(v) != 0;
        if (const char* v = std::getenv("GI_R_FLAT")) env.r_flat = std::atoi(v);
        if (const char* v = std::getenv("GI_RF_PER_SLOT")) env.rf_per_slot = std::max(0, std::min(1024, std::atoi(v)));
        if (const char* v = std::getenv("GI_X_WF")) env.wf = std::atoi(v);
        if (const char* v = std::getenv("GI_RF_GROUP")) env.rf_group = (std::atoi(v) == 1 || std::atoi(v) == 4) ? std::atoi(v) : 0;
        const char* v = std::getenv("GI_X_MAX_RUN");
        const int r = v ? std::max(1, std::min(128, std::atoi(v))) : GI_X_MAX_RUN;
        int lg = 0;
        while ((2 << lg) <= r) ++lg;
        env.run_log2 = lg;
    });
    return env;
}

#ifndef GI_WF_MAX_DEPTH
#define GI_WF_MAX_DEPTH 64
#endif
XForm x_form_choice(const DevScene& sc, const XLaunchCfg& xc, const gi_opts& o) {
    if (o.mode != GI_MODE_X || (o.flags & GI_FLAG_X_MEGA)) return XFORM_MEGA;
    if (o.flags & GI_FLAG_X_SEG) return XFORM_SEG;
    const XForm wf = o.depth <= GI_WF_MAX_DEPTH ? XFORM_WF : XFORM_MEGA;
    if (o.flags & GI_FLAG_X_WF) return wf;
    const XEnv& env = x_env();
    if (env.wf >= 0) return env.wf == XFORM_WF ? wf : env.wf == XFORM_SEG ? XFORM_SEG : XFORM_MEGA;
    return (xc.var.lds || (size_t)sc.n_xwnodes * sizeof(XWNode) <= ((size_t)1 << 20)) ? XFORM_SEG : XFORM_MEGA;
}

namespace {
template <typename F>
void x_dispatch(const DevScene& sc, bool help, bool stats, F&& f) {
    with_bools([&](auto S, auto HP, auto C, auto H, auto T) { f(&k_mode_x<S.value, HP.value, C.value, H.value, T.value>); },
               stats, help, sc.xcnodes != nullptr, sc.x_max_depth <= 7, sc.x_tri_only != 0);
}

hipError_t launch_mode_x(const DevScene& sc, const XLaunchCfg& xc, const CamDev& cam, V3 light, const TileMap& m,
                         const gi_opts& o, double* rgb, uint8_t* rgb8, const XScratch& xs, hipStream_t stream,
                         hipEvent_t ev_begin, hipEvent_t ev_end) {
    const dim3 block(64 * kWavesPerBlock);
    unsigned long long* st = reinterpret_cast<unsigned long long*>(o.stats);
    const bool stats = (o.flags & GI_FLAG_STATS) && st;
    const XEnv& env = x_env();
    const long long n_slots = m.n_local * (kTile * kTile);
    const bool help = env.help && n_slots * (long long)o.spp <= 32ll * 256ll * (long long)xc.resident;
    const long long want = (n_slots * (long long)o.spp / 64 + kWavesPerBlock - 1) / kWavesPerBlock;
    const dim3 pgrid((unsigned)std::max<long long>(1, std::min<long long>(want, xc.resident)));
    if (!xs.list || (unsigned long long)xs.cap < (unsigned long long)n_slots || (o.spp > 1 && (!xs.part || xs.spp < o.spp)))
        return hipErrorInvalidValue;
    const int s0 = o.sample_end > 0 ? o.sample_begin : 0, s1 = o.sample_end > 0 ? o.sample_end : o.spp;
    const bool cont = s0 > 0;
    hipError_t e = hipMemsetAsync(sc.work, 0, (cont ? 1 : 16) * sizeof(unsigned), stream);
    if (e == hipSuccess && cont) e = hipMemsetAsync(sc.work + 2, 0, 14 * sizeof(unsigned), stream);
    if (e != hipSuccess) return e;
    const XWork wk{xs.list, sc.work + 1, xs.part, sc.work, s0, s1};
    const dim3 sgrid((unsigned)((n_slots + 255) / 256));
    const dim3 cgrid((unsigned)((n_slots + kClassifyBlock - 1) / kClassifyBlock));
    const XForm form = x_form_choice(sc, xc, o);
    unsigned* zero2 = form == XFORM_SEG ? xs.wcnt : nullptr;
    unsigned* cl = cont ? nullptr : xs.list;
    with_bools([&](auto S) {
        hipLaunchKernelGGL(k_x_classify<S.value>, cgrid, dim3(kClassifyBlock), 0, stream, sc, cam, m, s1 - s0, rgb, rgb8, cl, sc.work + 1, st, zero2);
    }, stats);
    const int h8 = sc.x_handle8;
    const int xf = sc.x_flags | (env.run_log2 << XF_RUN_SHIFT) | ((o.flags & GI_FLAG_X_NO_SHADOW) ? XF_NO_SHADOW : 0) |
                   (env.help ? XF_HANDOFF : 0) | (help ? XF_SPREAD : 0) | XF_PIXEL_MAJOR | (env.flat ? 0 : XF_NO_FLAT) |
                   (xc.seg_ring ? XF_SEG_RING : 0);
    if (form != XFORM_MEGA) {
        if (!xs.wcnt || (form == XFORM_WF && (!xs.wq[0] || !xs.wq[1] || xs.wcap <= 0))) return hipErrorInvalidValue;
        const bool seg = form == XFORM_SEG;
        const XKernelCfg c{xc.var, env.flat != 0, seg ? xc.seg_lds_bytes : xc.wf_lds_bytes, xc.wf_grid[seg ? WK_SEG : WK_BOUNCE]};
        e = launch_wf(sc, c, form, cam, light, m.w, m.h, m.y0, o, rgb, rgb8, xs, sc.work + 1, stats ? st : nullptr, xf, stream,
                      ev_begin, ev_end);
        if (e != hipSuccess) return e;
    } else {
        if (ev_begin) (void)hipEventRecord(ev_begin, stream);
        x_dispatch(sc, help, stats, [&](auto kernel) {
            hipLaunchKernelGGL(kernel, pgrid, block, xc.lds_bytes, stream, sc, cam, light, m, o.spp, o.depth, o.seed, rgb, rgb8, st, wk,
                               h8, xf);
        });
        if (ev_end) (void)hipEventRecord(ev_end, stream);
    }
    if (o.spp > 1) hipLaunchKernelGGL(k_x_reduce, sgrid, dim3(256), 0, stream, m, wk, o.spp, rgb, rgb8);
    return hipSuccess;
}
}

hipError_t x_launch_config(const DevScene& sc, int device, XLaunchCfg& cfg) {
    const bool lds = sc.x_lds_bytes > 0;
    cfg.lds_bytes = 16 * 256 * sizeof(int) + 256 * (7 * sizeof(double) + 2 * sizeof(int));
    cfg.var = XVariant{lds, lds && sc.x_waves4};
    int cus = 0, per_cu = 0;
    hipError_t e = hipDeviceGetAttribute(&cus, hipDeviceAttributeMultiprocessorCount, device);
    if (e != hipSuccess) return e;
    x_dispatch(sc, false, false, [&](auto kernel) {
        e = hipOccupancyMaxActiveBlocksPerMultiprocessor(&per_cu, reinterpret_cast<const void*>(kernel), 64 * kWavesPerBlock,
                                                         cfg.lds_bytes);
    });
    if (e != hipSuccess) return e;
    cfg.resident = std::max(1, cus) * std::max(1, per_cu);
    const bool flat = sc.x_flat && x_env().flat;
    cfg.wf_lds_bytes = wf_lds_bytes(sc, lds, flat);
    cfg.wf_tree_lds_bytes = wf_lds_bytes(sc, lds, false);
    int wf_per_cu[WK_COUNT] = {};
    for (int k = 0; k < WK_COUNT; ++k) {
        const XKernelCfg c{cfg.var, flat, cfg.wf_lds_bytes + (k == WK_SEG_RING ? wf_seg_ring_bytes() : 0), 0};
        e = wf_occupancy(sc, (WfKernel)k, c, &wf_per_cu[k]);
        if (e != hipSuccess) return e;
        cfg.wf_grid[k] = std::max(1, cus) * std::max(1, wf_per_cu[k]);
    }
    cfg.seg_ring = x_env().seg_ring && wf_per_cu[WK_SEG_RING] >= wf_per_cu[WK_SEG] && wf_per_cu[WK_SEG] >= 1;
    cfg.seg_lds_bytes = cfg.wf_lds_bytes + (cfg.seg_ring ? wf_seg_ring_bytes() : 0);
    return hipSuccess;
}

hipError_t launch_render(const DevScene& sc, const XLaunchCfg& xc, const CamDev& cam, V3 light, int w, int h, int y0,
                         const gi_opts& o, double* rgb, uint8_t* rgb8, const XScratch& xs, KTimer* kt,
                         hipStream_t stream) {
    const bool timed = (o.flags & GI_FLAG_TIME) && kt && kt->ev0[0];
    const int slot = timed ? (int)(kt->recorded % KTimer::kRing) : 0;
    hipEvent_t ev_begin = timed ? static_cast<hipEvent_t>(kt->ev0[slot]) : nullptr;
    hipEvent_t ev_end = timed ? static_cast<hipEvent_t>(kt->ev1[slot]) : nullptr;
    const TileMap m = make_map(w, h, o.shard_count, o.shard_index, y0);
    if (m.n_local == 0) return hipSuccess;
    const hipError_t e = o.mode == GI_MODE_R ? launch_mode_r(sc, cam, light, w, h, y0, o, rgb, rgb8, xs, stream, ev_begin, ev_end)
                                             : launch_mode_x(sc, xc, cam, light, m, o, rgb, rgb8, xs, stream, ev_begin, ev_end);
    if (e != hipSuccess) return e;
    if (timed) kt->recorded++;
    return hipGetLastError();
}

hipError_t launch_unshard(int w, int h, int shard_count, const double* packed, const uint8_t* packed8, double* rgb,
                          uint8_t* rgb8, hipStream_t stream) {
    const TileMap m = make_map(w, h, shard_count, 0);
    const long long n = m.n_tiles * kTile * kTile;
    hipLaunchKernelGGL(k_unshard, dim3((unsigned)((n + 255) / 256)), dim3(256), 0, stream, m, packed, packed8, rgb, rgb8);
    return hipGetLastError();
}

hipError_t launch_moments(const DevScene& sc, const XScratch& xs, const CamDev& cam, int w, int h, const MomentsIO& io,
                          hipStream_t stream) {
    const TileMap m = make_map(w, h, 1, 0);
    const long long n_slots = m.n_local * (kTile * kTile);
    if (!xs.list || !xs.part || xs.cap < n_slots || xs.spp < io.spp || io.n < 2 || io.n > io.spp) return hipErrorInvalidValue;
    const XMoments a{xs.list, sc.work + 1, xs.part, io.spp, io.n, io.x0, io.y0, io.cols, io.rows, io.mean, io.var, io.samples};
    const long long n_px = (long long)io.cols * (long long)io.rows;
    const long long fgrid = std::min<long long>((n_px + 255) / 256, 1ll << 20);
    hipLaunchKernelGGL(k_x_moments_fill, dim3((unsigned)fgrid), dim3(256), 0, stream, sc, cam, a);
    const int block = GI_MOMENTS_LDS ? 64 : 256;
    hipLaunchKernelGGL(k_x_moments, dim3((unsigned)((n_slots + block - 1) / block)), dim3(block), 0, stream, m, a);
    return hipGetLastError();
}

}
```

### 2019global_amd/csrc/gi_launch.h

```cpp
#pragma once

#include <hip/hip_runtime_api.h>

#include "gi.h"
#include "gi_scene.h"

namespace gi {

struct XEnv {
    int run_log2 = 0, help = 1, wf = -1, flat = 1, seg_ring = 1, fan = 1;
    int r_flat = -1;
    int rf_per_slot = 16;
    int rf_group = 0;
};
const XEnv& x_env();

struct XKernelCfg {
    XVariant var;
    bool flat;
    size_t lds_bytes;
    int resident;
};

long long shard_tiles(int w, int h, int shard_count);
constexpr long long kXWfChunk = 8ll << 20;
hipError_t x_launch_config(const DevScene& sc, int device, XLaunchCfg& cfg);
XForm x_form_choice(const DevScene& sc, const XLaunchCfg& xc, const gi_opts& o);
hipError_t launch_render(const DevScene& sc, const XLaunchCfg& xc, const CamDev& cam, V3 light, int w, int h, int y0,
                         const gi_opts& o, double* rgb, uint8_t* rgb8, const XScratch& xs, KTimer* kt,
                         hipStream_t stream);
hipError_t launch_unshard(int w, int h, int shard_count, const double* packed, const uint8_t* packed8, double* rgb,
                          uint8_t* rgb8, hipStream_t stream);

struct MomentsIO {
    int x0, y0, cols, rows;
    int spp, n;
    double *mean, *var, *samples;
};
hipError_t launch_moments(const DevScene& sc, const XScratch& xs, const CamDev& cam, int w, int h, const MomentsIO& io,
                          hipStream_t stream);

RKernel r_kernel_choice(const DevScene& sc, const gi_opts& o);
unsigned rf_own_pairs();
unsigned rf_page_pairs();
unsigned rf_max_pages();
unsigned rf_seg_pairs();
hipError_t launch_mode_r(const DevScene& sc, const CamDev& cam, V3 light, int w, int h, int y0, const gi_opts& o,
                         double* rgb, uint8_t* rgb8, const XScratch& xs, hipStream_t stream, hipEvent_t ev_begin,
                         hipEvent_t ev_end);
hipError_t launch_trace_ray(const DevScene& sc, V3 o, V3 d, V3 light, int32_t* out_i, double* out_d, hipStream_t stream);
hipError_t launch_box_kat(int n, const double* recs, int32_t* out, hipStream_t stream);

size_t wf_lds_bytes(const DevScene& sc, bool lds, bool flat);
size_t wf_seg_ring_bytes();
hipError_t wf_occupancy(const DevScene& sc, WfKernel k, const XKernelCfg& c, int* per_cu);
XKernelCfg x_query_cfg(const XLaunchCfg& xc, int flags, WfKernel k);
hipError_t launch_wf(const DevScene& sc, const XKernelCfg& c, XForm form, const CamDev& cam, V3 light, int w, int h, int y0,
                     const gi_opts& o, double* rgb, uint8_t* rgb8, const XScratch& xs, const unsigned* n_list_dev,
                     unsigned long long* stats, int xflags, hipStream_t stream, hipEvent_t ev_begin, hipEvent_t ev_end);
hipError_t launch_x_query_kat(const DevScene& sc, const XKernelCfg& c, V3 cam_pos, int n, const double* recs, int32_t* oi,
                              double* od, hipStream_t stream);
hipError_t launch_x_texel_kat(const DevScene& sc, XVariant var, int n, int mode, const double* recs, int32_t* oi, double* od,
                              hipStream_t stream);
hipError_t launch_cast(const DevScene& sc, const XKernelCfg& c, bool any, const CastIO& io, hipStream_t stream);
hipError_t launch_aov(const DevScene& sc, const XKernelCfg& c, const CamDev& cam, const AovIO& io, hipStream_t stream);
hipError_t launch_cam_rays(const CamDev& cam, int x0, int y0, int cols, int rows, double* rays, hipStream_t stream);
void wf_variant(const DevScene& sc, const XKernelCfg& c, int32_t out[6]);

struct DnIO {
    int x0, y0, cols, rows;
    const double *rgb, *t, *nrm, *alb;
    double* out;
    uint8_t* out8;
};
long long dn_scratch_bytes(long long n_px, int levels, bool albedo_stop);
hipError_t launch_denoise(const CamDev& cam, const DnIO& io, const gi_denoise_params& p, void* scratch, hipStream_t stream);
struct DnvIO {
    int x0, y0, cols, rows;
    const double *rgb, *var, *t, *nrm, *alb;
    double *out, *out_var;
    uint8_t* out8;
};
long long dnv_scratch_bytes(long long n_px, int levels, bool albedo_stop);
hipError_t launch_denoise_var(const CamDev& cam, const DnvIO& io, const gi_denoise_var_params& p, void* scratch, hipStream_t stream);

}
```

### 2019global_amd/csrc/gi_scene.h

```cpp
#pragma once
#include <stdint.h>
#include <string>
#include <type_traits>
#include <vector>

#include "gi.h"
#include "gi_math.h"

namespace gi {

struct CamDev {
    V3 pos, up, left, top_left;
    double rx, ry;
};

enum EntKind : int32_t { K_IMP_SPHERE = 1, K_IMP_TRIANGLE = 2, K_EXP_QUAD = 3, K_EXP_SPHERE = 4, K_EXP_CUBE = 5,
                         K_EXP_CONE = 6, K_EXP_RECTANGLE = 7, K_EXP_BOX = 8 };

struct RNode {
    double mn[3], mx[3];
    int32_t child0;
    int32_t parent;
    int32_t ent_off;
    int32_t ent_cnt;
};
static_assert(sizeof(RNode) == 64, "RNode layout");

struct RPathRec {
    double mn[3], mx[3];
    int32_t node;
    int32_t ent_cnt;
    int32_t pad[2];
};
static_assert(sizeof(RPathRec) == 64, "RPathRec layout");
struct RApp {
    int64_t rank;
    int32_t p0, p1;
};
static_assert(sizeof(RApp) == 16, "RApp layout");

struct REnt {
    int32_t kind, tri_first, tri_count, pad0;
    double pos[3];
    float radius, width, length, alpha;
    double qv0[3], qv1[3], qv2[3];
    double color[3], shader[3];
    double spec_pow;
    float height, pad1;
    double sin_theta;
    double refl;
};
static_assert(sizeof(REnt) == 208, "REnt layout");

struct XPrim {
    double a[3];
    double b[3];
    double c[3];
    double n[3];
    int32_t kind;
    int32_t ent;
    int32_t pad[2];
};
static_assert(sizeof(XPrim) == 112, "XPrim layout");

struct XNode {
    double mn[3], mx[3];
    int32_t child_base;
    int32_t child_mask;
    int32_t prim_off;
    int32_t prim_cnt;
};
static_assert(sizeof(XNode) == 64, "XNode layout");

constexpr int32_t XEMPTY = (int32_t)0x80000000;
struct XWNode {
    float lo[3][8];
    float hi[3][8];
    int32_t child[8];
    int32_t parent;
    uint16_t cnt[8];
    int32_t exists;
    int32_t pad[2];
};
static_assert(sizeof(XWNode) == 256, "XWNode layout");
struct XCNode {
    float org[3];
    int8_t ex[3];
    uint8_t exists;
    uint8_t qlo[3][8];
    uint8_t qhi[3][8];
    int32_t child[8];
    uint8_t cnt[8];
    int32_t parent;
    int32_t pad[5];
};
static_assert(sizeof(XCNode) == 128, "XCNode layout");
bool encode_xcnodes(const std::vector<XWNode>& w, std::vector<XCNode>& out);

struct XHot {
    double a[3], b[3], c[3];
    int32_t prim;
    int32_t kind;
};
static_assert(sizeof(XHot) == 80, "XHot layout");
struct XBox {
    float lo[3], hi[3];
    int32_t pad[2];
};
static_assert(sizeof(XBox) == 32, "XBox layout");
struct XLeaf {
    int32_t off, cnt;
};
#ifndef GI_XFLAT_MAX
#define GI_XFLAT_MAX 32
#endif
static_assert(GI_XFLAT_MAX >= 1 && GI_XFLAT_MAX <= 32, "the candidate mask is one 32-bit word");
struct XFlatLeaf {
    float lo[3], hi[3];
    int32_t off;
    uint16_t cnt;
    uint8_t group;
    uint8_t fan;
};
static_assert(sizeof(XFlatLeaf) == 32, "XFlatLeaf layout");

struct HostScene {
    std::vector<RNode> rnodes;
    std::vector<int32_t> leaf_ents;
    std::vector<REnt> ents;
    std::vector<TriRec> tris;
    int32_t max_depth = 0, n_leaves = 0, n_reachable = 0, n_dropped = 0;
    std::vector<XNode> xnodes;
    std::vector<XWNode> xwnodes;
    std::vector<XCNode> xcnodes;
    std::vector<XLeaf> xleaves;
    std::vector<int32_t> xprim_idx;
    std::vector<XHot> xhot;
    std::vector<XBox> xbox;
    std::vector<XPrim> xprims;
    int32_t x_max_depth = 0;
    std::vector<int32_t> app_off;
    std::vector<int32_t> app_leaf;
    std::vector<int64_t> app_rank;
    std::vector<int32_t> rpath_off;
    std::vector<int32_t> rpath;
    std::vector<RPathRec> rpath_rec;
    std::vector<RApp> app_rec;
    std::vector<XWNode> rc_nodes;
    std::vector<int32_t> rc_ent;
    std::vector<int64_t> rc_maxkey;
    std::vector<int32_t> r_always;
    std::vector<int32_t> r_leaf_of_rank;
    double rc_ext = 0;
    int32_t x_handle8 = 6;
    int32_t x_flags = 0;
    double x_est_nodes = 0, x_est_prims = 0;
    bool x_spatial = false;
    double x_skip_a = 0.0, x_skip_b = 2.0;
    std::vector<XFlatLeaf> xflat;
    bool x_flat_ok = false;
    int32_t n_fan_leaves = 0;
    bool x_fan_all = false;
};
bool build_host_scene(const gi_scene_desc& desc, HostScene& hs, std::string& err);
void build_xflat(HostScene& hs);

inline void finalize_xwnodes(std::vector<XWNode>& w) {
    for (XWNode& n : w) {
        n.exists = 0;
        for (int c = 0; c < 8; ++c)
            if (n.child[c] != XEMPTY) n.exists |= 1 << c;
    }
}

void build_xbvh(const std::vector<XPrim>& prims, const std::vector<double>& bounds, int leaf_max, HostScene& hs,
                bool geometric = false);
void build_rcand(HostScene& hs);

struct DevScene {
    const RNode* rnodes;
    const int32_t* leaf_ents;
    const REnt* ents;
    const TriRec* tris;
    const XWNode* xwnodes;
    const XCNode* xcnodes;
    const XHot* xhot;
    const XBox* xbox;
    const XPrim* xprims;
    unsigned* work;
    int32_t n_rnodes, n_ents, n_xwnodes, n_xprims;
    int32_t x_max_depth;
    int32_t x_handle8;
    int32_t x_flags;
    int32_t n_xhot;
    int32_t x_lds_bytes;
    int32_t x_waves4;
    int32_t x_tri_only;
    int32_t r_tri_only;
    float root_lo[3], root_hi[3];
    double x_skip_a, x_skip_b;
    const int32_t* app_off;
    const RApp* app_rec;
    const RPathRec* rpath_rec;
    const XWNode* rc_nodes;
    const int32_t* rc_ent;
    const int64_t* rc_maxkey;
    const int32_t* r_always;
    const int32_t* r_leaf_of_rank;
    int32_t n_r_always;
    float rc_ext;
    const XFlatLeaf* xflat;
    int32_t n_xflat;
    int32_t x_flat;
    float x_far_r;
    int32_t x_fan;
};
static_assert(sizeof(DevScene) == 264, "DevScene layout");

struct KTimer {
    static constexpr int kRing = 64;
    void* ev0[kRing] = {};
    void* ev1[kRing] = {};
    long long recorded = 0;
    double sum_ms = 0.0;
    long long folded = 0;
};

struct XScratch {
    unsigned* list = nullptr;
    double* part = nullptr;
    long long cap = 0;
    int spp = 0;
    double* wq[2] = {nullptr, nullptr};
    unsigned* wid[2] = {nullptr, nullptr};
    unsigned* wcnt = nullptr;
    long long wcap = 0;
    unsigned* rf_pairs = nullptr;
    unsigned* rf_pt = nullptr;
    unsigned long long* rf_best = nullptr;
    double* rf_dir = nullptr;
    unsigned* rf_cnt = nullptr;
    unsigned* rf_ovf = nullptr;
    unsigned* rf_rcnt = nullptr;
    unsigned* rf_soff = nullptr;
    unsigned* rf_shc = nullptr;
    unsigned* rf_sreg = nullptr;
    unsigned* rf_hoff = nullptr;
    unsigned rf_pages = 0;
    long long rf_slots = 0;
    size_t rf_bytes = 0;
    long long rf_failed = 0;
};

enum XFlag : int {
    XF_INLINE_SHADOW = 1 << 0,
    XF_NO_SHADOW = 1 << 2,
    XF_HANDOFF = 1 << 3,
    XF_SPREAD = 1 << 4,
    XF_PIXEL_MAJOR = 1 << 5,
    XF_NO_FLAT = 1 << 6,
    XF_SEG_RING = 1 << 7,
    XF_RUN_SHIFT = 8, XF_RUN_MASK = 7,
};

struct XVariant {
    bool lds = false;
    bool w4 = false;
};
template <bool STATS, bool LDS, bool W4, bool SH, bool TRI, bool CN, bool FLAT>
struct XTag {
    static constexpr bool stats = STATS, lds = LDS, w4 = W4, sh = SH, tri = TRI, cn = CN, flat = FLAT;
};
template <bool... Bs, typename F>
void with_bools(F&& f) {
    f(std::integral_constant<bool, Bs>{}...);
}
template <bool... Bs, typename F, typename... R>
void with_bools(F&& f, bool b, R... r) {
    if (b) with_bools<Bs..., true>(f, r...);
    else with_bools<Bs..., false>(f, r...);
}

enum XForm : int { XFORM_MEGA = 0, XFORM_WF = 1, XFORM_SEG = 2 };
enum RKernel : int { RK_PIXEL = 0, RK_FLAT = 1, RK_BATCH = 2 };
enum WfKernel { WK_BOUNCE, WK_SEG, WK_SEG_RING, WK_CAST, WK_OCCL, WK_AOV, WK_COUNT };

struct XLaunchCfg {
    XVariant var;
    size_t lds_bytes = 0;
    int resident = 1;
    size_t wf_lds_bytes = 0;
    size_t wf_tree_lds_bytes = 0;
    int wf_grid[WK_COUNT] = {};
    bool seg_ring = false;
    size_t seg_lds_bytes = 0;
};

struct CastIO {
    const double* rays;
    long long n;
    double* t;
    int32_t* prim;
    int32_t* ent;
    double* nrm;
    int32_t* occl;
};

struct AovIO {
    int x0, y0, cols, rows;
    double* t;
    double* nrm;
    double* alb;
    int32_t* prim;
    int32_t* ent;
    int32_t* uv;
};

}
```

### 2019global_amd/csrc/gi_wf.hip

```cpp
#include <hip/hip_runtime.h>

#include <algorithm>
#include <cstdlib>
#include <mutex>
#include <type_traits>

#include "gi.h"
#include "gi_dev.h"
#include "gi_fan_pair.h"
#include "gi_launch.h"
#include "gi_scene.h"
#include "gi_seg_ring.h"

namespace gi {
namespace {

constexpr long long kWfTile = 8;

#ifndef GI_WF_MIN_WAVES_LDS
#define GI_WF_MIN_WAVES_LDS 4
#endif
#ifndef GI_WF_MIN_WAVES
#define GI_WF_MIN_WAVES 3
#endif
// ... 16 lines not shown
struct WFQ {
    double* r;
    uint2* id;
    long long cap;
};

template <bool ANY, bool PAIR, bool AXIS, bool SH, bool TRI, bool NST, typename NodeP, typename HotP>
__device__ __forceinline__ int wf_trace(float far_r, NodeP W, HotP H, V3 o, V3 d, double tmax, bool act, int* nst, double& t_out,
                                        uint32_t& nnode, uint32_t& nprim, uint32_t& nsteps, int skip = 254) {
    constexpr bool kSkip = std::is_same<NodeP, const XWNode*>::value;
    const F3 of = ray_org32(o, d, far_r);
    const F3 ivf = inv_dir(d);
    const int dmask = (d.x < 0 ? 1 : 0) | (d.y < 0 ? 2 : 0) | (d.z < 0 ? 4 : 0);
    double tb = tmax;
    float tbf = up32(tmax);
    int best = -1;
    uint64_t mlo = 0, mhi = 0;
    int node = 0, level = 0;
    bool raying = false;
    if (act) {
        uint32_t rm;
        if constexpr (kSkip) rm = children_mask<AXIS, true>(W, of, ivf, tbf, dmask, skip);
        else rm = children_mask<AXIS>(W, of, ivf, tbf, dmask);
        lvl_set<SH>(mlo, mhi, 0, rm);
        raying = rm != 0;
    }
    while (raying) {
        ++nsteps;
        const auto* nd = W + node;
        const uint32_t msk = lvl_get<SH>(mlo, mhi, level);
        const int kc = __builtin_ctz(msk);
        lvl_set<SH>(mlo, mhi, level, msk & (msk - 1));
        const int c = kc ^ dmask;
        bool keep = true;
        if (!ANY && !NST && best >= 0) {
            keep = child_hit(nd, c, of, ivf, tbf);
        }
        const int ch = nd->child[c];
        if (keep) {
            if (ch < 0) {
                const int cnt = nd->cnt[c];
                const auto* hp = H + ~ch;
                if constexpr (PAIR) {
                    for (int j = 0; j < cnt; j += 2) {
                        const bool two = j + 1 < cnt;
                        const XHotR r0 = load_hot(hp + j), r1 = load_hot(hp + (two ? j + 1 : j));
                        const double ta = x_prim_t<TRI>(r0.h, o, d, MX_TMIN);
                        const double tq = two ? x_prim_t<TRI>(r1.h, o, d, MX_TMIN) : INFINITY;
                        nprim += two ? 2 : 1;
                        if (ANY) {
                            if ((ta < tmax) | (tq < tmax)) {
                                best = ta < tmax ? r0.h.prim : r1.h.prim;
                                break;
                            }
                        } else {
                            const bool ua = (ta < tb) | ((ta == tb) & (r0.h.prim < best));
                            tb = ua ? ta : tb;
                            best = ua ? r0.h.prim : best;
                            const bool uq = (tq < tb) | ((tq == tb) & (r1.h.prim < best));
                            tb = uq ? tq : tb;
                            best = uq ? r1.h.prim : best;
                            tbf = up32(tb);
                        }
                    }
                } else {
                    XHotR cur = load_hot(hp);
                    for (int j = 0; j < cnt; ++j) {
                        const XHotR rec = cur;
                        if (j + 1 < cnt) cur = load_hot(hp + j + 1);
                        ++nprim;
                        const double t = x_prim_t<TRI>(rec.h, o, d, MX_TMIN);
                        if (ANY) {
                            if (t < tmax) { best = rec.h.prim; break; }
                        } else {
                            const bool u = (t < tb) | ((t == tb) & (rec.h.prim < best));
                            tb = u ? t : tb;
                            best = u ? rec.h.prim : best;
                            tbf = u ? up32(t) : tbf;
                        }
                    }
                }
            } else {
                ++nnode;
                uint32_t cm;
                if constexpr (kSkip) cm = children_mask<AXIS, true>(W + ch, of, ivf, tbf, dmask, skip);
                else cm = children_mask<AXIS>(W + ch, of, ivf, tbf, dmask);
                if (cm) {
                    node = ch;
                    ++level;
                    lvl_set<SH>(mlo, mhi, level, cm);
                    if (NST) nst[level * 256] = ch;
                }
            }
        }
        if (ANY && best >= 0) break;
        uint32_t rest = lvl_get<SH>(mlo, mhi, level);
        if (rest == 0 && level > 0) {
            if constexpr (NST) {
                const uint64_t lm = level >= 8 ? mlo : mlo & ((1ull << (8 * level)) - 1);
                const uint64_t hm = level <= 8 ? 0ull : mhi & ((1ull << (8 * (level - 8))) - 1);
                level = hm ? 8 + (63 - __clzll((long long)hm)) / 8 : lm ? (63 - __clzll((long long)lm)) / 8 : 0;
                rest = lvl_get<SH>(mlo, mhi, level);
                node = level == 0 ? 0 : nst[level * 256];
            } else {
                do {
                    --level;
                    node = level == 0 ? 0 : W[node].parent;
                    rest = lvl_get<SH>(mlo, mhi, level);
                } while (rest == 0 && level > 0);
            }
        }
        raying = rest != 0;
    }
    t_out = tb;
    return best;
}

constexpr size_t kFlatPkBytes = GI_XFLAT_MAX * sizeof(uint32_t);
typedef uint32_t u32x8 __attribute__((ext_vector_type(8)));
__device__ __forceinline__ u32x8 flat_rec_uniform(const XFlatLeaf* tab, int k) {
    return *(const __attribute__((address_space(4))) u32x8*)(uintptr_t)(tab + k);
}
__device__ __forceinline__ uint32_t flat_pack(uint32_t off, int k, uint32_t w7) { return off | ((uint32_t)k << 16) | ((w7 & 0xFFu) << 24); }
__device__ __forceinline__ uint32_t flat_shift_in(uint32_t m, unsigned long long hm) {
    uint32_t r;
    asm("v_addc_co_u32 %0, vcc, %1, %1, %2" : "=v"(r) : "v"(m), "s"(hm) : "vcc");
    return r;
}
__device__ __forceinline__ int flat_key(float tn, int k) {
    int r;
    asm("v_bfi_b32 %0, 31, %1, %2" : "=v"(r) : "s"(k), "v"(tn));
    return r;
}
__device__ __forceinline__ int flat_med3(int a, int b, int c) { return max(min(a, b), min(max(a, b), c)); }
__device__ __forceinline__ float flat_key_floor(int e) { return __int_as_float(e & ~31); }
__device__ __forceinline__ uint32_t flat_pk_of(const uint32_t* pkw, int k) { return pkw[k]; }
__device__ __forceinline__ bool flat_hit(const XFlatLeaf* r, F3 no, F3 ivf, int sm, float tmax, uint32_t& pk, int k) {
    const int4* q = reinterpret_cast<const int4*>(r);
    const int4 a = q[0], b = q[1];
    const float lx = __int_as_float(a.x), ly = __int_as_float(a.y), lz = __int_as_float(a.z);
    const float hx = __int_as_float(a.w), hy = __int_as_float(b.x), hz = __int_as_float(b.y);
    const float nx = (sm & 1) ? hx : lx, fx = (sm & 1) ? lx : hx;
    const float ny = (sm & 2) ? hy : ly, fy = (sm & 2) ? ly : hy;
    const float nz = (sm & 4) ? hz : lz, fz = (sm & 4) ? lz : hz;
    const float tn = fmaxf(fmaxf(__builtin_fmaf(nx, ivf.x, no.x), __builtin_fmaf(ny, ivf.y, no.y)),
                           fmaxf(__builtin_fmaf(nz, ivf.z, no.z), 0.0f));
    const float tf = fminf(fminf(__builtin_fmaf(fx, ivf.x, no.x), __builtin_fmaf(fy, ivf.y, no.y)),
                           fminf(__builtin_fmaf(fz, ivf.z, no.z), tmax));
    pk = flat_pack((uint32_t)b.z, k, (uint32_t)b.w);
    return tn <= tf;
}
template <bool ANY, bool TRI>
__device__ __forceinline__ int wf_flat(float far_r, const XFlatLeaf* tab, const uint32_t* pkw, int n, const XHot* H, V3 o, V3 d, double tmax, bool act,
                                       double& t_out, uint32_t& nnode, uint32_t& nprim, uint32_t& nsteps, int skip, bool fan) {
    const F3 of = ray_org32(o, d, far_r);
    const F3 ivf = inv_dir(d);
    const F3 no = neg_oiv(of, ivf);
    const int sm = iv_signs(ivf);
    const bool sx = (sm & 1) != 0, sy = (sm & 2) != 0, sz = (sm & 4) != 0;
    double tb = tmax;
    float tbf = up32(tmax);
    int best = -1;
    const float tfa = __builtin_canonicalizef(act ? tbf : -1.0f);
    constexpr int kNone = 0x7F800000;
    uint32_t m = 0, pk = 0;
    int e1 = kNone, e2 = kNone;
    auto step = [&](const u32x8 w, int k) {
        const float lx = __uint_as_float(w[0]), ly = __uint_as_float(w[1]), lz = __uint_as_float(w[2]);
        const float hx = __uint_as_float(w[3]), hy = __uint_as_float(w[4]), hz = __uint_as_float(w[5]);
        const float ax = __builtin_fmaf(lx, ivf.x, no.x), bx = __builtin_fmaf(hx, ivf.x, no.x);
        const float ay = __builtin_fmaf(ly, ivf.y, no.y), by = __builtin_fmaf(hy, ivf.y, no.y);
        const float az = __builtin_fmaf(lz, ivf.z, no.z), bz = __builtin_fmaf(hz, ivf.z, no.z);
        const float tn = fmaxf(fmaxf(sx ? bx : ax, sy ? by : ay), fmaxf(sz ? bz : az, 0.0f));
        const float tf = fminf(fminf(sx ? ax : bx, sy ? ay : by), fminf(sz ? az : bz, tfa));
        const bool in = tn <= tf, other = (int)((w[7] >> 16) & 0xFFu) != skip;
        m = flat_shift_in(m, __builtin_amdgcn_ballot_w64(in) & __builtin_amdgcn_ballot_w64(other));
        if (!ANY) {
            const int key = flat_key(tn, k);
            const int eh = (in & other) ? key : kNone;
            e2 = flat_med3(e1, e2, eh);
            e1 = min(e1, eh);
        }
    };
    int k0 = 0;
    for (; k0 + 4 <= n; k0 += 4) {
        const u32x8 w0 = flat_rec_uniform(tab, k0), w1 = flat_rec_uniform(tab, k0 + 1);
        const u32x8 w2 = flat_rec_uniform(tab, k0 + 2), w3 = flat_rec_uniform(tab, k0 + 3);
        step(w0, k0);
        step(w1, k0 + 1);
        step(w2, k0 + 2);
        step(w3, k0 + 3);
    }
#pragma unroll 1
    for (int k = k0; k < n; ++k) step(flat_rec_uniform(tab, k), k);
    if (act) nnode += (uint32_t)((n * (int)sizeof(XFlatLeaf) + 255) / 256);
    bool go = m != 0;
    if (go) {
        const int bit = (ANY || e1 == kNone) ? __builtin_ctz(m) : n - 1 - (e1 & 31);
        m &= ~(1u << bit);
        pk = flat_pk_of(pkw, n - 1 - bit);
    }
    while (go) {
        ++nsteps;
        const int cnt = (int)(pk >> 24);
        const XHot* hp = H + (pk & 0xFFFFu);
        if (TRI && fan) {
            const XHotR r0 = load_hot(hp);
            const int ch = fan_pair_choice(r0.h, o, d);
            const XHotR rc = load_hot(hp + (ch == FAN_T2 ? 1 : 0));
            const double ta = x_prim_t<TRI>(rc.h, o, d, MX_TMIN);
            double tq = INFINITY;
            int pq = rc.h.prim;
            if (__builtin_amdgcn_ballot_w64(ch == FAN_BOTH) != 0) {
                if (ch == FAN_BOTH) {
                    const XHotR r1 = load_hot(hp + 1);
                    tq = x_prim_t<TRI>(r1.h, o, d, MX_TMIN);
                    pq = r1.h.prim;
                }
            }
            nprim += 2;
            if (ANY) {
                if ((ta < tmax) | (tq < tmax)) best = ta < tmax ? rc.h.prim : pq;
            } else {
                const bool ua = (ta < tb) | ((ta == tb) & (rc.h.prim < best));
                tb = ua ? ta : tb;
                best = ua ? rc.h.prim : best;
                const bool uq = (tq < tb) | ((tq == tb) & (pq < best));
                tb = uq ? tq : tb;
                best = uq ? pq : best;
                tbf = up32(tb);
            }
        } else
        for (int j = 0; j < cnt; j += 2) {
            const bool two = j + 1 < cnt;
            const XHotR r0 = load_hot(hp + j), r1 = load_hot(hp + (two ? j + 1 : j));
            const double ta = x_prim_t<TRI>(r0.h, o, d, MX_TMIN);
            const double tq = two ? x_prim_t<TRI>(r1.h, o, d, MX_TMIN) : INFINITY;
            nprim += two ? 2 : 1;
            if (ANY) {
                if ((ta < tmax) | (tq < tmax)) {
                    best = ta < tmax ? r0.h.prim : r1.h.prim;
                    break;
                }
            } else {
                const bool ua = (ta < tb) | ((ta == tb) & (r0.h.prim < best));
                tb = ua ? ta : tb;
                best = ua ? r0.h.prim : best;
                const bool uq = (tq < tb) | ((tq == tb) & (r1.h.prim < best));
                tb = uq ? tq : tb;
                best = uq ? r1.h.prim : best;
                tbf = up32(tb);
            }
        }
        go = false;
        if (ANY) {
            if (best < 0 && m != 0) {
                const int bit = __builtin_ctz(m);
                m &= m - 1;
                pk = flat_pk_of(pkw, n - 1 - bit);
                go = true;
            }
        } else {
            if (flat_key_floor(e2) > tbf) m = 0;
            while (m != 0) {
                const int bit = 31 - __builtin_clz(m);
                m &= ~(1u << bit);
                const int k = n - 1 - bit;
                if (flat_hit(tab + k, no, ivf, sm, tbf, pk, k)) {
                    go = true;
                    break;
                }
            }
        }
    }
    t_out = tb;
    return best;
}

struct WFArgs {
    const unsigned* list;
    const unsigned* n_list;
    double* part;
    unsigned* take;
    const unsigned* n_in;
    unsigned* n_out;
    unsigned long long u0, u1;
    unsigned s0, ns;
};

struct WFView {
    const XWNode* LW = nullptr;
    const XHot* LH = nullptr;
    const XPrim* XP = nullptr;
    const REnt* EN = nullptr;
    const XFlatLeaf* FT = nullptr;
    const uint32_t* FP = nullptr;
    int* nst = nullptr;
    double* pl = nullptr;
};
template <bool LDS, bool FLAT = false>
__device__ __forceinline__ WFView wf_stage(const DevScene& sc, int4* lds) {
    WFView v;
    v.XP = sc.xprims;
    v.EN = sc.ents;
    v.FT = sc.xflat;
    if constexpr (LDS) {
        const int nw = FLAT ? 0 : sc.n_xwnodes * (int)(sizeof(XWNode) / sizeof(int4));
        const int nh = sc.n_xhot * (int)(sizeof(XHot) / sizeof(int4));
        const int np = sc.n_xprims * (int)(sizeof(XPrim) / sizeof(int4));
        const int ne = sc.n_ents * (int)(sizeof(REnt) / sizeof(int4));
        const int4* gw = reinterpret_cast<const int4*>(sc.xwnodes);
        const int4* gh = reinterpret_cast<const int4*>(sc.xhot);
        const int4* gp = reinterpret_cast<const int4*>(sc.xprims);
        const int4* ge = reinterpret_cast<const int4*>(sc.ents);
        for (int i = threadIdx.x; i < nw; i += blockDim.x) lds[i] = gw[i];
        for (int i = threadIdx.x; i < nh; i += blockDim.x) lds[nw + i] = gh[i];
        for (int i = threadIdx.x; i < np; i += blockDim.x) lds[nw + nh + i] = gp[i];
        for (int i = threadIdx.x; i < ne; i += blockDim.x) lds[nw + nh + np + i] = ge[i];
        constexpr int nk = FLAT ? (int)(kFlatPkBytes / sizeof(int4)) : 0;
        if constexpr (FLAT) {
            uint32_t* pkw = reinterpret_cast<uint32_t*>(lds + nw + nh + np + ne);
            for (int i = threadIdx.x; i < sc.n_xflat; i += blockDim.x) pkw[i] = flat_pack((uint32_t)sc.xflat[i].off, i, (uint32_t)sc.xflat[i].cnt);
            v.FP = pkw;
        }
        __syncthreads();
        if constexpr (!FLAT) v.LW = reinterpret_cast<const XWNode*>(lds);
        v.LH = reinterpret_cast<const XHot*>(lds + nw);
        v.XP = reinterpret_cast<const XPrim*>(lds + nw + nh);
        v.EN = reinterpret_cast<const REnt*>(lds + nw + nh + np);
        v.pl = reinterpret_cast<double*>(lds + nw + nh + np + ne + nk) + threadIdx.x;
    } else {
        v.nst = reinterpret_cast<int*>(lds) + threadIdx.x;
        v.pl = reinterpret_cast<double*>(reinterpret_cast<int*>(lds) + 16 * 256) + threadIdx.x;
    }
    return v;
}

__device__ __forceinline__ V3 wf_primary(const CamDev& cam, const TileMap& m, unsigned ps, int spp, uint64_t seed,
                                         unsigned li, unsigned smp, long long& idx, uint64_t& key) {
    int x = 0, y = 0;
    slot_pixel(m, (long long)(ps >> 6), (int)(ps & 63), idx, x, y);
    y += m.y0;
    if (spp > 1) idx = (long long)li;
    key = mx_key(seed, (uint64_t)y * (uint64_t)m.w + (uint64_t)x);
    double jx = 0.0, jy = 0.0;
    if (spp > 1) {
        jx = mx_u01k(key, smp, 0xFFFF, 0);
        jy = mx_u01k(key, smp, 0xFFFF, 1);
    }
    return primary_dir(cam, (double)x + jx, (double)y + jy);
}
__device__ __forceinline__ bool wf_primary_misses(const DevScene& sc, const CamDev& cam, V3 d0) {
    const F3 iv0 = f3(__builtin_amdgcn_rcpf((float)d0.x), __builtin_amdgcn_rcpf((float)d0.y), __builtin_amdgcn_rcpf((float)d0.z));
    return !root_hit(sc, ray_org32(cam.pos, d0, ray_far_r(sc, cam.pos)), iv0);
}
__device__ __forceinline__ void wf_store(double* part, double* rgb, uint8_t* rgb8, int spp, long long idx, unsigned smp, V3 L) {
    if (spp > 1) {
        double* q = part + 3 * ((size_t)idx * (size_t)spp + (size_t)smp);
        q[0] = L.x; q[1] = L.y; q[2] = L.z;
    } else {
        const double c0 = smin((0.0 + L.x) / 1.0, 1.0), c1 = smin((0.0 + L.y) / 1.0, 1.0), c2 = smin((0.0 + L.z) / 1.0, 1.0);
        if (rgb) { rgb[3 * idx] = c0; rgb[3 * idx + 1] = c1; rgb[3 * idx + 2] = c2; }
        if (rgb8) quantize(c0, c1, c2, rgb8 + 3 * idx);
    }
}

struct WFSegStats {
    uint64_t it_c = 0, ln_c = 0, it_s = 0, ln_s = 0, segs = 0, live = 0, iters = 0;
    uint64_t cyc_c = 0, cyc_s = 0, cyc_sh = 0, cyc_ref = 0, cyc_all = 0;
};
__device__ __forceinline__ void wf_wave_steps(uint32_t n, uint64_t& it, uint64_t& ln) {
    uint32_t mx = n, sm = n;
    for (int off = 32; off > 0; off >>= 1) {
        mx = max(mx, (uint32_t)__shfl_xor(mx, off));
        sm += __shfl_xor(sm, off);
    }
    if ((threadIdx.x & 63) == 0) { it += mx; ln += sm; }
}
template <bool ANY, bool LDS, bool SH, bool TRI, bool CN, bool FLAT>
__device__ __forceinline__ int x_query(const DevScene& sc, const WFView& v, float far_r, const V3& o, const V3& d, double tmax,
                                       bool act, double& t_out, uint32_t& nnode, uint32_t& nprim, uint32_t& st_steps, int skip) {
    if constexpr (FLAT) return wf_flat<ANY, TRI>(far_r, v.FT, v.FP, sc.n_xflat, v.LH, o, d, tmax, act, t_out, nnode, nprim, st_steps, skip, sc.x_fan != 0);
    else if constexpr (LDS) return wf_trace<ANY, true, false, SH, TRI, false>(far_r, v.LW, v.LH, o, d, tmax, act, v.nst, t_out, nnode, nprim, st_steps, skip);
    else if constexpr (CN) return wf_trace<ANY, false, false, SH, TRI, true>(far_r, sc.xcnodes, sc.xhot, o, d, tmax, act, v.nst, t_out, nnode, nprim, st_steps);
    else return wf_trace<ANY, false, false, SH, TRI, true>(far_r, sc.xwnodes, sc.xhot, o, d, tmax, act, v.nst, t_out, nnode, nprim, st_steps, skip);
}
__device__ __forceinline__ int x_own_plane(int pg, const V3& pn, const V3& dir, double skip_cos) {
    return (pg < 254 && fabs(dot(dir, pn)) >= skip_cos) ? pg : 254;
}
struct XHitFrame { V3 P, Ld, pn; double ldist; int pg; };
__device__ __forceinline__ XHitFrame x_hit_frame(const WFView& v, const V3& light, const V3& o, const V3& d, bool hit, int best, double t) {
    XHitFrame h{o, v3(0, 0, 1), v3(0, 0, 1), 0.0, 254};
    if (hit) {
        h.P = o + t * d;
        const V3 lv = light - h.P;
        h.ldist = gsqrt(dot(lv, lv));
        h.Ld = normalize(lv);
        const XPrim& px = v.XP[best];
        h.pg = px.pad[0] < 254 ? px.pad[0] : 254;
        h.pn = ld3(px.n);
    }
    return h;
}

template <bool STATS, bool LDS, bool SH, bool TRI, bool CN, bool FLAT, typename KeyF>
__device__ __forceinline__ bool x_segment(const DevScene& sc, const WFView& v, const V3& light, int depth, bool no_shadow, bool act,
                                          const KeyF& id_of, V3& o, V3& d, V3& L, V3& T,
                                          uint32_t& nnode, uint32_t& nprim, uint32_t& nrays, WFSegStats& ws,
                                          double skip_cos = 2.0, int* splane = nullptr, float far_r = INFINITY) {
    uint32_t st_steps = 0;
    uint64_t c0 = STATS ? clock64() : 0;
    bool occl = false;
    double tbest = INFINITY;
    const int skip_c = splane ? (*splane & kSegPlaneMask) : 254;
    const int best = x_query<false, LDS, SH, TRI, CN, FLAT>(sc, v, far_r, o, d, INFINITY, act, tbest, nnode, nprim, st_steps, skip_c);
    if (act) ++nrays;
    if (STATS) {
        wf_wave_steps(st_steps, ws.it_c, ws.ln_c);
        st_steps = 0;
        const uint64_t c1 = clock64();
        ws.cyc_c += c1 - c0;
        c0 = c1;
    }
    const bool hit = act && best >= 0;
    const XHitFrame h = x_hit_frame(v, light, o, d, hit, best, tbest);
    const V3 &P = h.P, &Ld = h.Ld;
    if (!no_shadow) {
        double tdummy;
        const int skip_s = x_own_plane(h.pg, h.pn, Ld, skip_cos);
        occl = x_query<true, LDS, SH, TRI, CN, FLAT>(sc, v, INFINITY, P, Ld, h.ldist, hit, tdummy, nnode, nprim, st_steps, skip_s) >= 0;
        if (STATS) wf_wave_steps(st_steps, ws.it_s, ws.ln_s);
    }
    if (STATS) {
        const uint64_t c1 = clock64();
        ws.cyc_s += c1 - c0;
        c0 = c1;
    }
    {
        L = v3(v.pl[0], v.pl[256], v.pl[512]);
        T = v3(v.pl[768], v.pl[1024], v.pl[1280]);
    }
    bool cont = false;
    if (hit) {
        ++nrays;
        const XPrim& p = v.XP[best];
        V3 N = (TRI || p.kind == 0) ? ld3(p.n) : normalize(P - ld3(p.a));
        N = dot(d, N) < 0 ? N : -N;
        const REnt& e = v.EN[p.ent];
        const V3 tc = x_texel<TRI>(sc, e, P);
        const V3 la = tc * e.shader[0];
        V3 loc = la;
        if (!occl) {
            const V3 ldf = (smax(0.0, dot(N, Ld)) * (tc * 0.5)) * e.shader[1];
            const V3 bis = normalize(normalize(-d) + Ld);
            const double spw = mx_pow(smax(0.0, dot(N, bis)), e.spec_pow);
            const V3 ls = v3(spw, spw, spw) * e.shader[2];
            loc = (la + ldf) + ls;
        }
        L = L + vmul(T, v3(smin(loc.x, 1.0), smin(loc.y, 1.0), smin(loc.z, 1.0)));
        const PathId id = id_of();
        const uint64_t key = id.key;
        const unsigned smp = id.smp;
        const int b = id.b;
        if (b != depth - 1) {
            if (e.refl > 0.0 && mx_u01k(key, smp, b, 4) < e.refl) {
                d = normalize(d - N * (2.0 * dot(d, N)));
                cont = true;
            } else {
                T = vmul(T, tc * 0.5);
                if (!((T.x == 0.0) & (T.y == 0.0) & (T.z == 0.0))) {
                    double sx, sy, r2;
                    mx_disk(mx_u01k(key, smp, b, 2), mx_u01k(key, smp, b, 3), sx, sy, r2);
                    const double sz = gsqrt(1.0 - r2);
                    const double sg = N.z >= 0.0 ? 1.0 : -1.0;
                    const double aa = -1.0 / (sg + N.z);
                    const double bb = N.x * N.y * aa;
                    const V3 bt1 = v3(1.0 + sg * N.x * N.x * aa, sg * bb, -sg * N.x);
                    const V3 bt2 = v3(bb, sg + N.y * N.y * aa, -N.y);
                    d = normalize((bt1 * sx + bt2 * sy) + N * sz);
                    cont = true;
                }
            }
            o = P;
        }
        if (cont) {
            v.pl[0] = L.x; v.pl[256] = L.y; v.pl[512] = L.z;
            v.pl[768] = T.x; v.pl[1024] = T.y; v.pl[1280] = T.z;
            if (splane) *splane = (*splane & ~kSegPlaneMask) | x_own_plane(h.pg, h.pn, d, skip_cos);
        }
    }
    if (STATS) ws.cyc_sh += clock64() - c0;
    return cont;
}

template <bool STATS, bool LDS, bool W4, bool SH, bool TRI, bool CN, bool FLAT>
__global__ __launch_bounds__(256, (LDS && W4) ? GI_WF_MIN_WAVES_LDS : GI_WF_MIN_WAVES) void k_wf_bounce(
    DevScene sc, CamDev cam, V3 light, TileMap m, int spp, int depth, uint64_t seed, int b, double* rgb, uint8_t* rgb8,
    unsigned long long* stats, WFArgs a, WFQ qin, WFQ qout, int xflags) {
    unsigned n_in;
    if (b == 0) {
        const unsigned long long tot = (unsigned long long)*a.n_list * (unsigned long long)a.ns;
        n_in = (unsigned)(min(tot, a.u1) > a.u0 ? min(tot, a.u1) - a.u0 : 0ull);
    } else {
        n_in = *a.n_in;
    }
    if (*(volatile unsigned*)a.take >= n_in) return;
    extern __shared__ int4 lds_dyn[];
    const WFView v = wf_stage<LDS, FLAT>(sc, lds_dyn);
    const bool no_shadow = (xflags & XF_NO_SHADOW) != 0;
    const int lane = threadIdx.x & 63;
    uint32_t nnode = 0, nprim = 0, nrays = 0, nres = 0, npx = 0;
    const long long qc = qin.cap, oc = qout.cap;
    const unsigned take = (unsigned)max(1u, min((unsigned)GI_WF_TAKE, n_in / (64u * 8u * (gridDim.x * (blockDim.x >> 6)))));
    unsigned base = 0, left = 0;
    for (;;) {
        if (left == 0) {
            if (lane == 0) base = atomicAdd(a.take, 64u * take);
            base = __shfl(base, 0);
            left = take;
        }
        if (base >= n_in) break;
        const unsigned j = base + (unsigned)lane;
        base += 64u;
        --left;
        bool act = j < n_in;
        unsigned li = 0, smp = 0;
        V3 o = cam.pos, d = v3(1, 0, 0), L = v3(0, 0, 0), T = v3(1, 1, 1);
        long long idx = -1;
        uint64_t key = 0;
        if (act) {
            if (b == 0) {
                const unsigned long long u = a.u0 + j;
                if (u < (1ull << 32)) {
                    li = (unsigned)u / a.ns;
                    smp = a.s0 + ((unsigned)u - li * a.ns);
                } else {
                    li = (unsigned)(u / (unsigned long long)a.ns);
                    smp = a.s0 + (unsigned)(u - (unsigned long long)li * (unsigned long long)a.ns);
                }
            } else {
                const uint2 id = qin.id[j];
                li = id.x;
                smp = id.y;
                const double* r = qin.r + j;
                o = v3(r[0], r[qc], r[2 * qc]);
                d = v3(r[3 * qc], r[4 * qc], r[5 * qc]);
                L = v3(r[6 * qc], r[7 * qc], r[8 * qc]);
                T = v3(r[9 * qc], r[10 * qc], r[11 * qc]);
            }
            const V3 d0 = wf_primary(cam, m, a.list[li], spp, seed, li, smp, idx, key);
            if (b == 0) {
                if (smp == 0) ++npx;
                if (wf_primary_misses(sc, cam, d0)) {
                    ++nrays;
                    ++nres;
                    act = false;
                    wf_store(a.part, rgb, rgb8, spp, idx, smp, v3(0, 0, 0));
                } else {
                    d = normalize(d0);
                }
            }
            v.pl[0] = L.x; v.pl[256] = L.y; v.pl[512] = L.z;
            v.pl[768] = T.x; v.pl[1024] = T.y; v.pl[1280] = T.z;
        }
        WFSegStats ws;
        const double skip_cos = x_skip_cos(sc, cam.pos);
        const float far_r = ray_far_r(sc, cam.pos);
        int splane = 254;
        const bool cont = x_segment<false, LDS, SH, TRI, CN, FLAT>(sc, v, light, depth, no_shadow, act, [&] { return PathId{key, smp, b}; }, o, d, L, T,
                                                             nnode, nprim, nrays, ws, skip_cos, &splane, far_r);
        const unsigned long long mc = __ballot(cont);
        if (mc) {
            const int leader = __ffsll((long long)mc) - 1;
            unsigned ob = 0;
            if (lane == leader) ob = atomicAdd(a.n_out, (unsigned)__popcll(mc));
            ob = __shfl(ob, leader);
            if (cont) {
                const unsigned k = ob + (unsigned)__popcll(mc & ((1ull << lane) - 1));
                qout.id[k] = make_uint2(li, smp);
                double* r = qout.r + k;
                r[0] = o.x; r[oc] = o.y; r[2 * oc] = o.z;
                r[3 * oc] = d.x; r[4 * oc] = d.y; r[5 * oc] = d.z;
                r[6 * oc] = L.x; r[7 * oc] = L.y; r[8 * oc] = L.z;
                r[9 * oc] = T.x; r[10 * oc] = T.y; r[11 * oc] = T.z;
            }
        }
        if (act && !cont) wf_store(a.part, rgb, rgb8, spp, idx, smp, L);
    }
    if (STATS) {
        wave_add_stats(stats, nrays, nnode, nprim, npx);
        uint64_t r = nres;
        for (int off = 32; off > 0; off >>= 1) r += __shfl_xor(r, off);
        if (lane == 0 && r) atomicAdd(stats + GI_STAT_X_RESOLVED, (unsigned long long)r);
    }
}

#ifndef GI_SEG_BURST
#define GI_SEG_BURST 16
#endif
#ifndef GI_SEG_TAKE
#define GI_SEG_TAKE 2
#endif
#ifndef GI_SEG_TAKE_TRI
#define GI_SEG_TAKE_TRI 1
#endif
struct SegRay {
    V3 d;
    uint64_t key, is;
};
__device__ __forceinline__ bool seg_make_unit(const DevScene& sc, const CamDev& cam, const TileMap& m, const WFArgs& a, int spp,
                                              uint64_t seed, double* rgb, uint8_t* rgb8, unsigned long long u, SegRay& r,
                                              uint32_t& nrays, uint32_t& nres, uint32_t& npx) {
    unsigned li, smp;
    if (u < (1ull << 32)) {
        li = (unsigned)u / a.ns;
        smp = a.s0 + ((unsigned)u - li * a.ns);
    } else {
        li = (unsigned)(u / (unsigned long long)a.ns);
        smp = a.s0 + (unsigned)(u - (unsigned long long)li * (unsigned long long)a.ns);
    }
    const unsigned ps = a.list[li];
    long long idx = -1;
    const V3 d0 = wf_primary(cam, m, ps, spp, seed, li, smp, idx, r.key);
    if (smp == 0) ++npx;
    if (wf_primary_misses(sc, cam, d0)) {
        ++nrays;
        ++nres;
        wf_store(a.part, rgb, rgb8, spp, idx, smp, v3(0, 0, 0));
        return false;
    }
    r.d = normalize(d0);
    r.is = (uint64_t)(uint32_t)idx | ((uint64_t)smp << 32);
    return true;
}
__device__ __forceinline__ unsigned seg_rank(unsigned long long mask) {
    return __builtin_amdgcn_mbcnt_hi((unsigned)(mask >> 32), __builtin_amdgcn_mbcnt_lo((unsigned)mask, 0u));
}
__device__ __forceinline__ unsigned long long seg_uniform64(unsigned long long v) {
    const unsigned lo = (unsigned)__builtin_amdgcn_readfirstlane((int)(unsigned)v);
    const unsigned hi = (unsigned)__builtin_amdgcn_readfirstlane((int)(unsigned)(v >> 32));
    return ((unsigned long long)hi << 32) | lo;
}

template <bool STATS, bool LDS, bool W4, bool SH, bool TRI, bool CN, bool FLAT, bool RING>
__global__ __launch_bounds__(256, (LDS && W4) ? GI_WF_MIN_WAVES_LDS : GI_WF_MIN_WAVES) void k_seg(
    DevScene sc, CamDev cam, V3 light, TileMap m, int spp, int depth, uint64_t seed, double* rgb, uint8_t* rgb8,
    unsigned long long* stats, WFArgs a, int xflags) {
    extern __shared__ int4 lds_dyn[];
    const WFView v = wf_stage<LDS, FLAT>(sc, lds_dyn);
    const bool no_shadow = (xflags & XF_NO_SHADOW) != 0;
    const int lane = threadIdx.x & 63;
    const unsigned long long total = (unsigned long long)*a.n_list * (unsigned long long)a.ns;
    constexpr long long kTake = (LDS && TRI) ? GI_SEG_TAKE_TRI : GI_SEG_TAKE;
    const unsigned long long n_waves = (unsigned long long)gridDim.x * (blockDim.x >> 6);
    const unsigned long long run = 64ull * (unsigned long long)max(1ll, min(kTake, (long long)(total / (64ull * 8ull * n_waves))));
    uint32_t nnode = 0, nprim = 0, nrays = 0, nres = 0, npx = 0;
    SegUnits su;
    bool live = false;
    V3 o = cam.pos, d = v3(1, 0, 0), L = v3(0, 0, 0), T = v3(1, 1, 1);
    int splane = 254;
    uint64_t* const rq = reinterpret_cast<uint64_t*>(v.pl - threadIdx.x + kWfSlotBytes / sizeof(double)) +
                         (threadIdx.x >> 6) * (kSegRingPlanes * kSegBatch);
    auto begin_path = [&](const V3& dir, uint64_t key, uint64_t is) {
        live = true;
        o = cam.pos;
        d = dir;
        splane = 254;
        L = v3(0, 0, 0);
        T = v3(1, 1, 1);
        v.pl[0] = 0.0; v.pl[256] = 0.0; v.pl[512] = 0.0;
        v.pl[768] = 1.0; v.pl[1024] = 1.0; v.pl[1280] = 1.0;
        slot_put_u64(v.pl, 6, key);
        slot_put_u64(v.pl, 7, is);
    };
    const double skip_cos = x_skip_cos(sc, cam.pos);
    const float far_r = ray_far_r(sc, cam.pos);
    WFSegStats ws;
    const uint64_t t_begin = STATS ? clock64() : 0;
    for (;;) {
        if (STATS && lane == 0) ++ws.iters;
        const uint64_t t_ref = STATS ? clock64() : 0;
        for (int burst = 0; burst < GI_SEG_BURST; ++burst) {
            const unsigned long long m_need = __ballot(!live);
            if (m_need == 0 || su.done()) break;
            const unsigned rank = seg_rank(m_need);
            const unsigned n_need = (unsigned)__popcll(m_need);
            if constexpr (RING) {
                if (su.wants_batch(n_need)) {
                    if (su.wants_run()) {
                        unsigned long long nb = 0;
                        if (lane == 0) nb = atomicAdd(reinterpret_cast<unsigned long long*>(a.take), run);
                        su.give_run(seg_uniform64(nb), run, total);
                    }
                    unsigned long long first = 0;
                    const unsigned n_batch = su.take_batch(first);
                    if (n_batch != 0) {
                        __builtin_amdgcn_fence(__ATOMIC_ACQ_REL, "wavefront");
                        __builtin_amdgcn_wave_barrier();
                        SegRay r{};
                        bool hit = false;
                        if ((unsigned)lane < n_batch) hit = seg_make_unit(sc, cam, m, a, spp, seed, rgb, rgb8, first + (unsigned)lane, r, nrays, nres, npx);
                        const unsigned long long m_hit = __ballot(hit);
                        if (hit) {
                            uint64_t* e = rq + seg_rank(m_hit);
                            e[0] = (uint64_t)__double_as_longlong(r.d.x);
                            e[kSegBatch] = (uint64_t)__double_as_longlong(r.d.y);
                            e[2 * kSegBatch] = (uint64_t)__double_as_longlong(r.d.z);
                            e[3 * kSegBatch] = r.key;
                            e[4 * kSegBatch] = r.is;
                        }
                        su.push((unsigned)__popcll(m_hit));
                        __builtin_amdgcn_fence(__ATOMIC_ACQ_REL, "wavefront");
                        __builtin_amdgcn_wave_barrier();
                    }
                }
                unsigned first_e = 0;
                const unsigned k = su.pop(n_need, first_e);
                if (!live && rank < k) {
                    const uint64_t* e = rq + (first_e + rank);
                    begin_path(v3(__longlong_as_double((long long)e[0]), __longlong_as_double((long long)e[kSegBatch]),
                                  __longlong_as_double((long long)e[2 * kSegBatch])),
                               e[3 * kSegBatch], e[4 * kSegBatch]);
                }
                continue;
            }
            unsigned long long u = ~0ull;
            const unsigned long long avail = su.cur_end - su.cur;
            if (n_need > avail && !su.exhausted) {
                unsigned long long nb = 0;
                if (lane == 0) nb = atomicAdd(reinterpret_cast<unsigned long long*>(a.take), run);
                nb = seg_uniform64(nb);
                if (nb >= total) {
                    su.exhausted = true;
                    if (!live && rank < avail) u = su.cur + rank;
                    su.cur = su.cur_end;
                } else {
                    const unsigned long long ne = min(total, nb + run);
                    if (!live) {
                        if (rank < avail) u = su.cur + rank;
                        else if (nb + (rank - avail) < ne) u = nb + (rank - avail);
                    }
                    su.cur = min(ne, nb + (n_need - avail));
                    su.cur_end = ne;
                    if (ne == total) su.exhausted = true;
                }
            } else {
                if (!live && rank < avail) u = su.cur + rank;
                su.cur += min((unsigned long long)n_need, avail);
            }
            if (!live && u != ~0ull) {
                SegRay r{};
                if (seg_make_unit(sc, cam, m, a, spp, seed, rgb, rgb8, u, r, nrays, nres, npx)) begin_path(r.d, r.key, r.is);
            }
        }
        if (STATS) ws.cyc_ref += clock64() - t_ref;
        if (__ballot(live) == 0) {
            if (su.done()) break;
            continue;
        }
        if (STATS) {
            const unsigned long long ml = __ballot(live);
            if (lane == 0) { ++ws.segs; ws.live += __popcll(ml); }
        }
        const bool cont = x_segment<STATS, LDS, SH, TRI, CN, FLAT>(
            sc, v, light, depth, no_shadow, live,
            [&] { return PathId{slot_get_u64(v.pl, 6), (unsigned)(slot_get_u64(v.pl, 7) >> 32), splane >> kSegPlaneBits}; },
            o, d, L, T, nnode, nprim, nrays, ws, skip_cos, &splane, far_r);
        if (live) {
            if (cont) {
                splane += 1 << kSegPlaneBits;
            } else {
                const uint64_t is = slot_get_u64(v.pl, 7);
                wf_store(a.part, rgb, rgb8, spp, (long long)(uint32_t)is, (unsigned)(is >> 32), L);
                live = false;
            }
        }
    }
    if (STATS && lane == 0) {
        atomicAdd(stats + GI_STAT_X_ITERS, (unsigned long long)ws.iters);
        atomicAdd(stats + GI_STAT_X_HANDLE, (unsigned long long)ws.segs);
        atomicAdd(stats + GI_STAT_X_HLANES, (unsigned long long)ws.live);
        atomicAdd(stats + GI_STAT_X_IT_LEAF, (unsigned long long)ws.it_c);
        atomicAdd(stats + GI_STAT_X_LN_LEAF, (unsigned long long)ws.ln_c);
        atomicAdd(stats + GI_STAT_X_IT_NODE, (unsigned long long)ws.it_s);
        atomicAdd(stats + GI_STAT_X_LN_NODE, (unsigned long long)ws.ln_s);
        atomicAdd(stats + GI_STAT_X_CYC_TRAV, (unsigned long long)(ws.cyc_c + ws.cyc_s));
        atomicAdd(stats + GI_STAT_X_IT_RS, (unsigned long long)ws.cyc_c);
        atomicAdd(stats + GI_STAT_X_CYC_HIT, (unsigned long long)ws.cyc_sh);
        atomicAdd(stats + GI_STAT_X_CYC_NEXT, (unsigned long long)ws.cyc_ref);
        atomicAdd(stats + GI_STAT_X_CYC_ALL, (unsigned long long)(clock64() - t_begin));
    }
    if (STATS) {
        wave_add_stats(stats, nrays, nnode, nprim, npx);
        uint64_t r = nres;
        for (int off = 32; off > 0; off >>= 1) r += __shfl_xor(r, off);
        if (lane == 0 && r) atomicAdd(stats + GI_STAT_X_RESOLVED, (unsigned long long)r);
    }
}

template <bool LDS, bool W4, bool SH, bool TRI, bool CN, bool FLAT>
__global__ __launch_bounds__(256, (LDS && W4) ? GI_WF_MIN_WAVES_LDS : GI_WF_MIN_WAVES) void k_x_query_kat(
    DevScene sc, V3 cam_pos, int n, const double* recs, int32_t* oi, double* od) {
    extern __shared__ int4 lds_dyn[];
    const WFView v = wf_stage<LDS, FLAT>(sc, lds_dyn);
    const long long i = (long long)blockIdx.x * 256 + threadIdx.x;
    const bool act = i < (long long)n;
    const double skip_cos = x_skip_cos(sc, cam_pos);
    const float far_r = ray_far_r(sc, cam_pos);
    V3 o = v3(0, 0, 0), d = v3(1, 0, 0), light = v3(0, 0, 0), d2 = v3(1, 0, 0);
    if (act) {
        const double* q = recs + 12 * i;
        o = v3(q[0], q[1], q[2]);
        d = v3(q[3], q[4], q[5]);
        light = v3(q[6], q[7], q[8]);
        d2 = v3(q[9], q[10], q[11]);
    }
    uint32_t nnode = 0, nprim = 0, st_steps = 0;
    double t1 = INFINITY;
    const int p1 = x_query<false, LDS, SH, TRI, CN, FLAT>(sc, v, far_r, o, d, INFINITY, act, t1, nnode, nprim, st_steps, 254);
    const bool hit = act && p1 >= 0;
    const XHitFrame h = x_hit_frame(v, light, o, d, hit, p1, t1);
    double tdummy;
    const int skip_s = x_own_plane(h.pg, h.pn, h.Ld, skip_cos);
    const int sb = x_query<true, LDS, SH, TRI, CN, FLAT>(sc, v, INFINITY, h.P, h.Ld, h.ldist, hit, tdummy, nnode, nprim, st_steps, skip_s);
    const int skip2 = x_own_plane(h.pg, h.pn, d2, skip_cos);
    double t2 = INFINITY;
    const int p2 = x_query<false, LDS, SH, TRI, CN, FLAT>(sc, v, far_r, h.P, d2, INFINITY, hit, t2, nnode, nprim, st_steps, skip2);
    if (act) {
        oi[5 * i] = p1 >= 0 ? p1 : -1;
        oi[5 * i + 1] = hit ? (sb >= 0 ? 1 : 0) : -1;
        oi[5 * i + 2] = skip_s;
        oi[5 * i + 3] = (hit && p2 >= 0) ? p2 : -1;
        oi[5 * i + 4] = skip2;
        od[2 * i] = p1 >= 0 ? t1 : INFINITY;
        od[2 * i + 1] = (hit && p2 >= 0) ? t2 : INFINITY;
    }
    if (i == 0) od[2 * (long long)n] = skip_cos;
}

template <bool TRI>
__global__ __launch_bounds__(256) void k_x_texel_kat(DevScene sc, int n, int mode, const double* recs, int32_t* oi, double* od) {
    const long long i = (long long)blockIdx.x * 256 + threadIdx.x;
    const bool act = i < (long long)n;
    int ent = 0;
    V3 P = v3(0, 0, 0);
    if (act) {
        const double* q = recs + 4 * i;
        ent = (int)q[0];
        P = v3(q[1], q[2], q[3]);
    }
    const REnt& e = sc.ents[ent];
    int how = 2;
    V3 tc;
    if (mode == 0) {
        tc = x_texel<TRI>(sc, e, P, &how);
    } else {
        int32_t tu, tv;
        x_texcoord<TRI>(sc, e, P, tu, tv);
        tc = texel(ld3(e.color), tu, tv);
    }
    if (act) {
        od[3 * i] = tc.x; od[3 * i + 1] = tc.y; od[3 * i + 2] = tc.z;
        oi[i] = how;
    }
}

template <bool ANY, bool LDS, bool W4, bool SH, bool TRI, bool CN, bool FLAT>
__global__ __launch_bounds__(256, (LDS && W4) ? GI_WF_MIN_WAVES_LDS : GI_WF_MIN_WAVES) void k_cast(DevScene sc, CastIO io) {
    extern __shared__ int4 lds_dyn[];
    const WFView v = wf_stage<LDS, FLAT>(sc, lds_dyn);
    const int lane = threadIdx.x & 63;
    const long long stride = 64ll * (long long)gridDim.x * (long long)(blockDim.x >> 6);
    for (long long base = 64ll * ((long long)blockIdx.x * (blockDim.x >> 6) + (threadIdx.x >> 6)); base < io.n; base += stride) {
        const long long i = base + lane;
        const bool in = i < io.n;
        V3 o = v3(0, 0, 0), d = v3(1, 0, 0);
        double tmax = INFINITY;
        bool act = false;
        if (in) {
            const double2* q = reinterpret_cast<const double2*>(io.rays) + 4 * i;
            const double2 q0 = q[0], q1 = q[1], q2 = q[2], q3 = q[3];
            const V3 ro = v3(q0.x, q0.y, q1.x), rd = v3(q1.y, q2.x, q2.y);
            const bool fin = __builtin_isfinite(ro.x) & __builtin_isfinite(ro.y) & __builtin_isfinite(ro.z) &
                             __builtin_isfinite(rd.x) & __builtin_isfinite(rd.y) & __builtin_isfinite(rd.z);
            const bool nz = (rd.x != 0.0) | (rd.y != 0.0) | (rd.z != 0.0);
            act = fin & nz & (q3.x > MX_TMIN);
            if (act) {
                o = ro;
                d = rd;
                tmax = q3.x;
            }
        }
        uint32_t nnode = 0, nprim = 0, nsteps = 0;
        double tb = INFINITY;
        const int best = x_query<ANY, LDS, SH, TRI, CN, FLAT>(sc, v, sc.x_far_r, o, d, tmax, act, tb, nnode, nprim, nsteps, 254);
        const bool hit = act && best >= 0;
        if constexpr (ANY) {
            if (in) io.occl[i] = hit ? 1 : 0;
        } else {
            if (in) {
                if (io.t) io.t[i] = hit ? tb : INFINITY;
                if (io.prim) io.prim[i] = hit ? best : -1;
                if (io.ent || io.nrm) {
                    int ent = -1;
                    V3 N = v3(0, 0, 0);
                    if (hit) {
                        const XPrim& p = v.XP[best];
                        ent = p.ent;
                        const V3 P = o + tb * d;
                        N = (TRI || p.kind == 0) ? ld3(p.n) : normalize(P - ld3(p.a));
                        N = dot(d, N) < 0 ? N : -N;
                    }
                    if (io.ent) io.ent[i] = ent;
                    if (io.nrm) {
                        double* q = io.nrm + 3 * i;
                        q[0] = N.x; q[1] = N.y; q[2] = N.z;
                    }
                }
            }
        }
// ... 3 lines not shown
__host__ __device__ inline long long aov_batches(int cols, int rows) { return ((long long)cols * (long long)rows + 63) / 64; }
__device__ __forceinline__ bool aov_pixel(int cols, int rows, long long b, int lane, int& px, int& py) {
    const long long i = 64 * b + lane;
    if (i < (1ll << 32)) {
        const unsigned q = (unsigned)i / (unsigned)cols;
        py = (int)q;
        px = (int)((unsigned)i - q * (unsigned)cols);
    } else {
        const long long q = i / (long long)cols;
        py = (int)q;
        px = (int)(i - q * (long long)cols);
    }
    return i < (long long)cols * (long long)rows;
}

template <bool LDS, bool W4, bool SH, bool TRI, bool CN, bool FLAT>
__global__ __launch_bounds__(256, (LDS && W4) ? GI_WF_MIN_WAVES_LDS : GI_WF_MIN_WAVES) void k_aov(DevScene sc, CamDev cam, AovIO io) {
    extern __shared__ int4 lds_dyn[];
    const WFView v = wf_stage<LDS, FLAT>(sc, lds_dyn);
    const int lane = threadIdx.x & 63;
    const float far_r = ray_far_r(sc, cam.pos);
    const long long n_batches = aov_batches(io.cols, io.rows);
    const long long stride = (long long)gridDim.x * (long long)(blockDim.x >> 6);
    const bool want_tex = io.alb || io.uv;
    for (long long b = (long long)blockIdx.x * (blockDim.x >> 6) + (threadIdx.x >> 6); b < n_batches; b += stride) {
        int px = 0, py = 0;
        const bool in = aov_pixel(io.cols, io.rows, b, lane, px, py);
        const V3 o = cam.pos;
        V3 d = v3(1, 0, 0);
        bool act = false;
        if (in) {
            const V3 d0 = primary_dir(cam, (double)(io.x0 + px), (double)(io.y0 + py));
            if (!wf_primary_misses(sc, cam, d0)) {
                act = true;
                d = normalize(d0);
            }
        }
        uint32_t nnode = 0, nprim = 0, nsteps = 0;
        double tb = INFINITY;
        const int best = x_query<false, LDS, SH, TRI, CN, FLAT>(sc, v, far_r, o, d, INFINITY, act, tb, nnode, nprim, nsteps, 254);
        const bool hit = act && best >= 0;
        if (in) {
            const long long i = (long long)py * (long long)io.cols + (long long)px;
            int ent = -1, tu = 0, tv = 0;
            V3 N = v3(0, 0, 0), tc = v3(0, 0, 0);
            if (hit) {
                const XPrim& p = v.XP[best];
                ent = p.ent;
                const V3 P = o + tb * d;
                N = (TRI || p.kind == 0) ? ld3(p.n) : normalize(P - ld3(p.a));
                N = dot(d, N) < 0 ? N : -N;
                if (want_tex) {
                    const REnt& e = v.EN[p.ent];
                    x_texcoord<TRI>(sc, e, P, tu, tv);
                    tc = texel(ld3(e.color), tu, tv);
                }
            }
            if (io.t) io.t[i] = hit ? tb : INFINITY;
            if (io.prim) io.prim[i] = hit ? best : -1;
            if (io.ent) io.ent[i] = ent;
            if (io.nrm) {
                double* q = io.nrm + 3 * i;
                q[0] = N.x; q[1] = N.y; q[2] = N.z;
            }
            if (io.alb) {
                double* q = io.alb + 3 * i;
                q[0] = tc.x; q[1] = tc.y; q[2] = tc.z;
            }
            if (io.uv) {
                int32_t* q = io.uv + 2 * i;
                q[0] = tu; q[1] = tv;
            }
        }
    }
}

__global__ __launch_bounds__(256) void k_cam_rays(CamDev cam, int x0, int y0, int cols, int rows, double* rays) {
    const long long n_batches = aov_batches(cols, rows);
    const long long stride = (long long)gridDim.x * (long long)(blockDim.x >> 6);
    const int lane = threadIdx.x & 63;
    for (long long b = (long long)blockIdx.x * (blockDim.x >> 6) + (threadIdx.x >> 6); b < n_batches; b += stride) {
        int px = 0, py = 0;
        if (!aov_pixel(cols, rows, b, lane, px, py)) continue;
        const V3 d = normalize(primary_dir(cam, (double)(x0 + px), (double)(y0 + py)));
        double2* q = reinterpret_cast<double2*>(rays) + 4 * (64 * b + lane);
        q[0] = make_double2(cam.pos.x, cam.pos.y);
        q[1] = make_double2(cam.pos.z, d.x);
        q[2] = make_double2(d.y, d.z);
        q[3] = make_double2(INFINITY, 0.0);
    }
}

}

constexpr size_t kWfStackBytes = 16 * 256 * sizeof(int);
size_t wf_lds_bytes(const DevScene& sc, bool lds, bool flat) {
    const size_t nodes = (flat && sc.x_flat) ? (size_t)sc.n_xwnodes * sizeof(XWNode) : 0;
    return (lds ? (size_t)sc.x_lds_bytes - nodes + (sc.x_flat ? kFlatPkBytes : 0) : kWfStackBytes) + kWfSlotBytes;
}
size_t wf_seg_ring_bytes() { return kSegRingBytes; }

namespace {
template <typename F>
void wf_dispatch(const DevScene& sc, const XKernelCfg& c, bool stats, F&& f) {
    const XVariant var = c.var;
    if (var.lds && c.flat && sc.x_flat)
        with_bools([&](auto S, auto W) { f(XTag<S.value, true, W.value, true, W.value, false, true>{}); }, stats, var.w4);
    else if (var.lds)
        with_bools([&](auto S, auto W, auto H) { f(XTag<S.value, true, W.value, H.value, W.value, false, false>{}); },
                   stats, var.w4, sc.x_max_depth <= 7);
    else
        with_bools([&](auto S, auto T, auto C) { f(XTag<S.value, false, false, false, T.value, C.value, false>{}); },
                   stats, sc.x_tri_only != 0, sc.xcnodes != nullptr);
}
template <bool RING, typename V>
constexpr auto seg_kernel(V) { return &k_seg<V::stats, V::lds, V::w4, V::sh, V::tri, V::cn, V::flat, RING>; }
template <typename V>
constexpr auto bounce_kernel(V) { return &k_wf_bounce<V::stats, V::lds, V::w4, V::sh, V::tri, V::cn, V::flat>; }

template <bool ANY, typename V>
constexpr auto cast_kernel(V) { return &k_cast<ANY, V::lds, V::w4, V::sh, V::tri, V::cn, V::flat>; }

template <typename V>
constexpr auto aov_kernel(V) { return &k_aov<V::lds, V::w4, V::sh, V::tri, V::cn, V::flat>; }
}

XKernelCfg x_query_cfg(const XLaunchCfg& xc, int flags, WfKernel k) {
    const bool hbm = (flags & 2) != 0 && xc.var.lds;
    const bool flat = x_env().flat && (flags & 1) == 0;
    return XKernelCfg{hbm ? XVariant{} : xc.var, flat,
                      hbm ? kWfStackBytes + kWfSlotBytes : flat ? xc.wf_lds_bytes : xc.wf_tree_lds_bytes, xc.wf_grid[k]};
}

hipError_t wf_occupancy(const DevScene& sc, WfKernel k, const XKernelCfg& c, int* per_cu) {
    hipError_t e = hipSuccess;
    wf_dispatch(sc, c, false, [&](auto V) {
        const void* f = nullptr;
        switch (k) {
            case WK_BOUNCE: f = reinterpret_cast<const void*>(bounce_kernel(V)); break;
            case WK_SEG: f = reinterpret_cast<const void*>(seg_kernel<false>(V)); break;
            case WK_SEG_RING: f = reinterpret_cast<const void*>(seg_kernel<true>(V)); break;
            case WK_CAST: f = reinterpret_cast<const void*>(cast_kernel<false>(V)); break;
            case WK_OCCL: f = reinterpret_cast<const void*>(cast_kernel<true>(V)); break;
            case WK_AOV: f = reinterpret_cast<const void*>(aov_kernel(V)); break;
            case WK_COUNT: break;
        }
        e = f ? hipOccupancyMaxActiveBlocksPerMultiprocessor(per_cu, f, 256, c.lds_bytes) : hipErrorInvalidValue;
    });
    return e;
}

hipError_t launch_wf(const DevScene& sc, const XKernelCfg& c, XForm form, const CamDev& cam, V3 light, int w, int h, int y0,
                     const gi_opts& o, double* rgb, uint8_t* rgb8, const XScratch& xs, const unsigned* n_list_dev,
                     unsigned long long* stats, int xflags, hipStream_t stream, hipEvent_t ev_begin, hipEvent_t ev_end) {
    const TileMap m = make_map(w, h, o.shard_count, o.shard_index, y0);
    const int depth = o.depth;
    const int s0 = o.sample_end > 0 ? o.sample_begin : 0, s1 = o.sample_end > 0 ? o.sample_end : o.spp;
    const dim3 grid((unsigned)std::max(1, c.resident)), block(256);
    hipError_t e = hipSuccess;
    WFArgs a{};
    a.list = xs.list;
    a.n_list = n_list_dev;
    a.part = xs.part;
    a.s0 = (unsigned)s0;
    a.ns = (unsigned)(s1 - s0);
    if (form == XFORM_SEG) {
        a.take = xs.wcnt;
        if (ev_begin) (void)hipEventRecord(ev_begin, stream);
        wf_dispatch(sc, c, stats != nullptr, [&](auto V) {
            if (xflags & XF_SEG_RING)
                hipLaunchKernelGGL(seg_kernel<true>(V), grid, block, c.lds_bytes, stream, sc, cam, light, m, o.spp, depth, o.seed, rgb, rgb8, stats, a, xflags);
            else
                hipLaunchKernelGGL(seg_kernel<false>(V), grid, block, c.lds_bytes, stream, sc, cam, light, m, o.spp, depth, o.seed, rgb, rgb8, stats, a, xflags);
        });
        if (ev_end) (void)hipEventRecord(ev_end, stream);
        return hipGetLastError();
    }
    const unsigned long long units = (unsigned long long)m.n_local * (unsigned long long)(kWfTile * kWfTile) *
                                     (unsigned long long)(s1 - s0);
    if (ev_begin) (void)hipEventRecord(ev_begin, stream);
    for (unsigned long long u0 = 0; u0 < units; u0 += (unsigned long long)xs.wcap) {
        e = hipMemsetAsync(xs.wcnt, 0, 2 * (size_t)depth * sizeof(unsigned), stream);
        if (e != hipSuccess) return e;
        for (int b = 0; b < depth; ++b) {
            a.take = xs.wcnt + 2 * b;
            a.n_in = b > 0 ? xs.wcnt + 2 * (b - 1) + 1 : nullptr;
            a.n_out = xs.wcnt + 2 * b + 1;
            a.u0 = u0;
            a.u1 = std::min(units, u0 + (unsigned long long)xs.wcap);
            WFQ qin, qout;
            qin.cap = qout.cap = xs.wcap;
            qin.r = xs.wq[(b + 1) & 1];
            qin.id = reinterpret_cast<uint2*>(xs.wid[(b + 1) & 1]);
            qout.r = xs.wq[b & 1];
            qout.id = reinterpret_cast<uint2*>(xs.wid[b & 1]);
            wf_dispatch(sc, c, stats != nullptr, [&](auto V) {
                hipLaunchKernelGGL(bounce_kernel(V), grid, block, c.lds_bytes, stream, sc, cam, light, m, o.spp, depth, o.seed, b, rgb, rgb8, stats, a, qin, qout, xflags);
            });
        }
    }
    if (ev_end) (void)hipEventRecord(ev_end, stream);
    return hipGetLastError();
}

hipError_t launch_x_query_kat(const DevScene& sc, const XKernelCfg& c, V3 cam_pos, int n, const double* recs, int32_t* oi,
                              double* od, hipStream_t stream) {
    if (n <= 0) return hipSuccess;
    const dim3 grid((unsigned)(((long long)n + 255) / 256)), block(256);
    wf_dispatch(sc, c, false, [&](auto V) {
        using T = decltype(V);
        hipLaunchKernelGGL((k_x_query_kat<T::lds, T::w4, T::sh, T::tri, T::cn, T::flat>), grid, block, c.lds_bytes, stream, sc, cam_pos, n, recs, oi, od);
    });
    return hipGetLastError();
}

hipError_t launch_x_texel_kat(const DevScene& sc, XVariant var, int n, int mode, const double* recs, int32_t* oi, double* od,
                              hipStream_t stream) {
    if (n <= 0) return hipSuccess;
    const dim3 grid((unsigned)(((long long)n + 255) / 256)), block(256);
    wf_dispatch(sc, XKernelCfg{var, false, 0, 0}, false, [&](auto V) {
        using T = decltype(V);
        hipLaunchKernelGGL((k_x_texel_kat<T::tri>), grid, block, 0, stream, sc, n, mode, recs, oi, od);
    });
    return hipGetLastError();
}

hipError_t launch_cast(const DevScene& sc, const XKernelCfg& c, bool any, const CastIO& io, hipStream_t stream) {
    if (io.n <= 0) return hipSuccess;
    const long long want = (io.n + 255) / 256;
    const dim3 grid((unsigned)std::max<long long>(1, std::min<long long>(want, c.resident))), block(256);
    wf_dispatch(sc, c, false, [&](auto V) {
        if (any) hipLaunchKernelGGL(cast_kernel<true>(V), grid, block, c.lds_bytes, stream, sc, io);
        else hipLaunchKernelGGL(cast_kernel<false>(V), grid, block, c.lds_bytes, stream, sc, io);
    });
    return hipGetLastError();
}

hipError_t launch_aov(const DevScene& sc, const XKernelCfg& c, const CamDev& cam, const AovIO& io, hipStream_t stream) {
    if (io.cols <= 0 || io.rows <= 0) return hipSuccess;
    const long long want = (aov_batches(io.cols, io.rows) + 3) / 4;
    const dim3 grid((unsigned)std::max<long long>(1, std::min<long long>(want, c.resident))), block(256);
    wf_dispatch(sc, c, false, [&](auto V) {
        hipLaunchKernelGGL(aov_kernel(V), grid, block, c.lds_bytes, stream, sc, cam, io);
    });
    return hipGetLastError();
}

hipError_t launch_cam_rays(const CamDev& cam, int x0, int y0, int cols, int rows, double* rays, hipStream_t stream) {
    if (cols <= 0 || rows <= 0) return hipSuccess;
    const long long want = ((long long)cols * (long long)rows + 255) / 256;
    const dim3 grid((unsigned)std::min<long long>(want, 2048)), block(256);
    hipLaunchKernelGGL(k_cam_rays, grid, block, 0, stream, cam, x0, y0, cols, rows, rays);
    return hipGetLastError();
}

void wf_variant(const DevScene& sc, const XKernelCfg& c, int32_t out[6]) {
    wf_dispatch(sc, c, false, [&](auto V) {
        out[0] = V.lds; out[1] = V.w4; out[2] = V.sh; out[3] = V.tri; out[4] = V.cn; out[5] = V.flat;
    });
}

}
```

### include/gi.h

```cpp
#ifndef GI_H_
#define GI_H_

#include <stddef.h>
#include <stdint.h>

#ifdef __cplusplus
extern "C" {
#endif

#define GI_ABI_VERSION 18

typedef enum gi_status {
    GI_OK = 0,
    GI_ERR_ARG = -1,
    GI_ERR_DEVICE = -2,
    GI_ERR_SCENE = -3,
    GI_ERR_CANCELLED = -4,
    GI_ERR_NOMEM = -5,
    GI_ERR_INTERNAL = -6
} gi_status;

typedef enum gi_entity_kind {
    GI_IMP_SPHERE = 1,
    GI_IMP_TRIANGLE = 2,
    GI_EXP_QUAD = 3,
    GI_EXP_SPHERE = 4,
    GI_EXP_CUBE = 5,
    GI_EXP_CONE = 6,
    GI_EXP_RECTANGLE = 7,
    GI_EXP_BOX = 8
} gi_entity_kind;

typedef struct gi_entity_desc {
    int32_t kind;
    int32_t has_material;
    double args[11];
    double mat_color[3];
    double mat_shader[3];
    double mat_specular_power;
    double mat_reflectivity;
} gi_entity_desc;

typedef struct gi_scene_desc {
    double octree_min[3];
    double octree_max[3];
    int32_t n_entities;
    const gi_entity_desc* entities;
} gi_scene_desc;

typedef struct gi_camera {
    double pos[3];
    double up[3];
    double forward[3];
    double focal;
} gi_camera;

typedef enum gi_mode {
    GI_MODE_R = 0,
    GI_MODE_X = 1
} gi_mode;

#define GI_FLAG_STATS 1u
#define GI_FLAG_R_DFS 2u
#define GI_FLAG_TIME 4u
#define GI_FLAG_X_NO_SHADOW 8u
#define GI_FLAG_X_WF 16u
#define GI_FLAG_X_MEGA 32u
#define GI_FLAG_X_SEG 64u

typedef struct gi_opts {
    int32_t mode;
    int32_t spp;
    int32_t depth;
    int32_t shard_count;
    int32_t shard_index;
    int32_t band_rows;
    uint32_t flags;
    int32_t reserved;
    uint64_t seed;
    uint64_t* stats;
    int32_t sample_begin;
    int32_t sample_end;
} gi_opts;

#define GI_STAT_RAYS 0
#define GI_STAT_NODES 1
#define GI_STAT_PRIMS 2
#define GI_STAT_PIXELS 3
#define GI_STAT_X_PATH_MAX 4
#define GI_STAT_X_ITERS 5
#define GI_STAT_X_TRAV 6
#define GI_STAT_X_HANDLE 7
#define GI_STAT_X_HLANES 8
#define GI_STAT_X_HCLOSE 9
#define GI_STAT_X_HSHADOW 10
#define GI_STAT_X_CYC_TRAV 11
#define GI_STAT_X_CYC_HIT 12
#define GI_STAT_X_CYC_NEXT 13
#define GI_STAT_X_CYC_ALL 14
#define GI_STAT_X_RESOLVED 15
#define GI_STAT_X_IT_NODE 16
#define GI_STAT_X_LN_NODE 17
#define GI_STAT_X_IT_LEAF 18
#define GI_STAT_X_LN_LEAF 19
#define GI_STAT_X_IT_RS 20
#define GI_STAT_X_LN_RS 21
#define GI_STAT_X_IT_ST 22
#define GI_STAT_X_LN_ST 23
#define GI_STAT_R_PAIRS 24
#define GI_STAT_R_OVF_TILES 25
#define GI_STATS_N 26

#define GI_TILE 8

typedef struct gi_scene gi_scene;

typedef struct gi_scene_info {
    int32_t n_entities;
    int32_t n_nodes;
    int32_t n_leaves;
    int32_t max_depth;
    int32_t n_reachable;
    int32_t n_dropped;
    int32_t x_nodes;
    int32_t x_prims;
    int64_t device_bytes;
    int32_t x_node_bytes;
    int32_t x_lds_resident;
    int32_t x_flat_leaves;
    int32_t x_fan_leaves;
} gi_scene_info;

typedef struct gi_hit {
    int32_t entity;
    int32_t u, v;
    double point[3], normal[3];
} gi_hit;

typedef void (*gi_tile_cb)(void* user, int y0, int rows, const uint8_t* rgb8_rows, const double* rgb_rows);

int gi_abi_version(void);
const char* gi_last_error(void);
int gi_device_count(void);
int gi_device_list(int32_t* out, int cap);
const char* gi_build_id(void);

int gi_camera_init(const double pos[3], const double look_at[3], double focal, gi_camera* out);

int gi_scene_create(const gi_scene_desc* desc, gi_scene** out);
void gi_scene_destroy(gi_scene* scene);
int gi_scene_get_info(const gi_scene* scene, gi_scene_info* info);

int gi_render(gi_scene* scene, const gi_camera* cam, const double light[3], int w, int h,
              const gi_opts* opts, double* rgb, uint8_t* rgb8, const volatile int* cancel,
              gi_tile_cb cb, void* user);

int gi_render_device(gi_scene* scene, const gi_camera* cam, const double light[3], int w, int h,
                     const gi_opts* opts, double* d_rgb, uint8_t* d_rgb8, void* stream);

int64_t gi_shard_tiles(int w, int h, int shard_count);

int gi_unshard_device(int w, int h, int shard_count, const double* d_packed, const uint8_t* d_packed8,
                      double* d_rgb, uint8_t* d_rgb8, void* stream);

int gi_trace_ray(gi_scene* scene, const double origin[3], const double dir[3], const double light[3],
                 gi_hit* hit, double rgb[3]);

#define GI_RAY_DOUBLES 8
int gi_intersect_device(gi_scene* scene, int64_t n, const double* d_rays, double* d_t, int32_t* d_prim,
                        int32_t* d_entity, double* d_normal, void* stream);
int gi_occluded_device(gi_scene* scene, int64_t n, const double* d_rays, int32_t* d_occluded, void* stream);
int gi_intersect(gi_scene* scene, int64_t n, const double* rays, double* t, int32_t* prim, int32_t* entity,
                 double* normal);
int gi_occluded(gi_scene* scene, int64_t n, const double* rays, int32_t* occluded);

typedef struct gi_aov_frame { int32_t w, h, x0, y0, x1, y1; } gi_aov_frame;
typedef struct gi_aov { double* t; double* normal; double* albedo; int32_t* prim; int32_t* entity; int32_t* uv; } gi_aov;
int gi_render_aov_device(gi_scene* scene, const gi_camera* cam, const gi_aov_frame* frame, const gi_aov* d_out,
                         void* stream);
int gi_render_aov(gi_scene* scene, const gi_camera* cam, const gi_aov_frame* frame, const gi_aov* out);
int gi_camera_rays_device(const gi_camera* cam, const gi_aov_frame* frame, double* d_rays, void* stream);
int gi_camera_rays(const gi_camera* cam, const gi_aov_frame* frame, double* rays);

#define GI_DENOISE_ALBEDO_STOP 1u
typedef struct gi_denoise_params {
    int32_t levels;
    int32_t normal_pow_log2;
    uint32_t flags;
    int32_t reserved;
    double sigma_c;
    double sigma_p;
} gi_denoise_params;
typedef struct gi_denoise_io {
    const double* rgb;
    const double* t;
    const double* normal;
    const double* albedo;
    double* out_rgb;
    uint8_t* out_rgb8;
} gi_denoise_io;
int64_t gi_denoise_scratch_bytes(const gi_aov_frame* frame, const gi_denoise_params* p);
int gi_denoise_device(const gi_camera* cam, const gi_aov_frame* frame, const gi_denoise_params* p,
                      const gi_denoise_io* d_io, void* d_scratch, int64_t scratch_bytes, void* stream);
int gi_denoise(const gi_camera* cam, const gi_aov_frame* frame, const gi_denoise_params* p, const gi_denoise_io* io);

typedef struct gi_moments { double* mean; double* var; double* samples; } gi_moments;
int gi_frame_samples_info(gi_scene* scene, int32_t* w, int32_t* h, int32_t* n, int32_t* spp);
int gi_frame_moments_device(gi_scene* scene, const gi_aov_frame* frame, const gi_moments* d_out, void* stream);
int gi_frame_moments(gi_scene* scene, const gi_aov_frame* frame, const gi_moments* out);

typedef struct gi_denoise_var_params {
    int32_t levels;
    int32_t normal_pow_log2;
    uint32_t flags;
    int32_t reserved;
    double sigma_v;
    double sigma_p;
    double var_floor;
} gi_denoise_var_params;
typedef struct gi_denoise_var_io {
    const double* rgb;
    const double* var;
    const double* t;
    const double* normal;
    const double* albedo;
    double* out_rgb;
    double* out_var;
    uint8_t* out_rgb8;
} gi_denoise_var_io;
int64_t gi_denoise_var_scratch_bytes(const gi_aov_frame* frame, const gi_denoise_var_params* p);
int gi_denoise_var_device(const gi_camera* cam, const gi_aov_frame* frame, const gi_denoise_var_params* p,
                          const gi_denoise_var_io* d_io, void* d_scratch, int64_t scratch_bytes, void* stream);
int gi_denoise_var(const gi_camera* cam, const gi_aov_frame* frame, const gi_denoise_var_params* p,
                   const gi_denoise_var_io* io);

int gi_scene_kernel_ms(gi_scene* scene, float* avg_ms, int64_t* n);
int gi_scene_x_form(gi_scene* scene, const gi_opts* opts, int32_t* form);
int gi_scene_seg_ring(gi_scene* scene, const gi_opts* opts, int32_t* on);
int gi_scene_r_kernel(gi_scene* scene, const gi_opts* opts, int32_t* kernel);

typedef struct gi_octree gi_octree;
int gi_octree_create(const gi_scene_desc* desc, gi_octree** out);
void gi_octree_destroy(gi_octree* octree);
int gi_octree_intersect(const gi_octree* octree, const double origin[3], const double dir[3], int32_t* out,
                        int64_t cap, int64_t* n);

typedef struct gi_multi gi_multi;
int gi_multi_create(const gi_scene_desc* desc, int n_shards, const int* devices, gi_multi** out);
void gi_multi_destroy(gi_multi* multi);
int gi_multi_info(const gi_multi* multi, int* n_shards, int* n_devices, int* uses_rccl);
int gi_multi_render(gi_multi* multi, const gi_camera* cam, const double light[3], int w, int h, const gi_opts* opts,
                    double* rgb, uint8_t* rgb8, const volatile int* cancel, gi_tile_cb cb, void* user);

int gi_obj_parse(const char* text, int64_t len, const gi_entity_desc* tmpl, gi_entity_desc* out, int64_t cap,
                 int64_t* n);

int gi_kat_expbox(int n, const double* recs, int32_t* out);

int gi_kat_x_query(gi_scene* scene, int n, const double* recs, const double cam_pos[3], int flags, int32_t* prim1,
                   double* t1, int32_t* occl, int32_t* skip_s, int32_t* prim2, double* t2, int32_t* skip2,
                   double* skip_cos);
int gi_kat_x_variant(gi_scene* scene, int flags, int32_t out[6]);

int gi_kat_x_texel(gi_scene* scene, int n, const double* recs, int mode, double* texel, int32_t* how);

#ifdef __cplusplus
}
#endif
#endif
```

Baseline: 37130.

## Cull flat-table leaves that cannot occlude shadow rays given light position

At scene build, computes per-leaf boundary plane info and a conservative error margin. At launch, derives a per-frame live mask of flat-table leaves whose plane side relative to the light means they can still occlude. Shadow queries in the wavefront and segment kernels then iterate only over live leaves instead of the full table. This removes shadow-ray tests against leaves that geometrically cannot block the light, at the cost of extra host bookkeeping, a larger launch config struct, and correctness that depends on the conservative margin.

```diff
diff --git a/2019global_amd/__init__.py b/2019global_amd/__init__.py
--- a/2019global_amd/__init__.py
+++ b/2019global_amd/__init__.py
@@ -31,6 +31,7 @@
 FLAG_X_WF = 16
 FLAG_X_MEGA = 32
 FLAG_X_SEG = 64
+FLAG_X_ALL_LEAVES = 128
 KAT_X_TREE, KAT_X_HBM = 1, 2
 X_FORMS = ("k_mode_x", "k_wf_bounce", "k_seg")
 R_KERNELS = ("k_mode_r", "k_rf_walk", "k_mode_r_batch")
@@ -43,7 +44,7 @@
 STAT_R_PAIRS, STAT_R_OVF_TILES = 24, 25
 STATS_N = 26
 TILE = 8
-ABI_VERSION = 18
+ABI_VERSION = 19
 RAY_DOUBLES = 8
 AOV_OUTPUTS = ("t", "normal", "albedo", "prim", "entity", "uv")
 _AOV_KINDS = {"t": (np.float64, ()), "normal": (np.float64, (3,)), "albedo": (np.float64, (3,)),
@@ -143,7 +144,7 @@
 
 EXPORTS = ["gi_abi_version", "gi_last_error", "gi_camera_init", "gi_scene_create", "gi_scene_destroy",
            "gi_scene_get_info", "gi_render", "gi_render_device", "gi_shard_tiles", "gi_unshard_device",
-           "gi_trace_ray", "gi_kat_expbox", "gi_kat_x_query", "gi_kat_x_variant", "gi_kat_x_texel", "gi_scene_kernel_ms", "gi_scene_x_form", "gi_scene_seg_ring", "gi_scene_r_kernel", "gi_octree_create", "gi_octree_destroy",
+           "gi_trace_ray", "gi_kat_expbox", "gi_kat_x_query", "gi_kat_x_variant", "gi_kat_x_texel", "gi_scene_kernel_ms", "gi_scene_x_form", "gi_scene_seg_ring", "gi_scene_shadow_leaves", "gi_scene_r_kernel", "gi_octree_create", "gi_octree_destroy",
            "gi_octree_intersect", "gi_multi_create", "gi_multi_destroy", "gi_multi_info", "gi_multi_render", "gi_device_count",
            "gi_device_list", "gi_build_id", "gi_obj_parse", "gi_intersect", "gi_occluded", "gi_intersect_device",
            "gi_occluded_device", "gi_render_aov", "gi_render_aov_device", "gi_camera_rays", "gi_camera_rays_device",
@@ -214,6 +215,8 @@
         L.gi_scene_kernel_ms.argtypes = [vp, ctypes.POINTER(ctypes.c_float), ctypes.POINTER(ctypes.c_int64)]
         L.gi_scene_x_form.argtypes = [vp, ctypes.POINTER(Opts), ctypes.POINTER(ctypes.c_int32)]
         L.gi_scene_seg_ring.argtypes = [vp, ctypes.POINTER(Opts), ctypes.POINTER(ctypes.c_int32)]
+        L.gi_scene_shadow_leaves.argtypes = [vp, ctypes.POINTER(ctypes.c_double), ctypes.POINTER(ctypes.c_double),
+                                             ctypes.POINTER(ctypes.c_uint32), ctypes.POINTER(ctypes.c_uint32)]
         L.gi_scene_r_kernel.argtypes = [vp, ctypes.POINTER(Opts), ctypes.POINTER(ctypes.c_int32)]
         L.gi_octree_create.argtypes = [ctypes.POINTER(SceneDesc), ctypes.POINTER(vp)]
         L.gi_octree_destroy.argtypes = [vp]
@@ -559,6 +562,12 @@
         _check(lib().gi_scene_seg_ring(self._h, ctypes.byref(o), ctypes.byref(f)), "gi_scene_seg_ring")
         return bool(f.value)
 
+    def shadow_leaves(self, light, cam_pos):
+        b, m = ctypes.c_uint32(), ctypes.c_uint32()
+        _check(lib().gi_scene_shadow_leaves(self._h, _d3(light), _d3(cam_pos), ctypes.byref(b), ctypes.byref(m)),
+               "gi_scene_shadow_leaves")
+        return b.value, m.value
+
     def r_kernel(self, flags=0) -> str:
         o = self.opts(MODE_R, 1, 1, 0, flags=flags)
         k = ctypes.c_int32()
diff --git a/2019global_amd/csrc/gi_build.cpp b/2019global_amd/csrc/gi_build.cpp
--- a/2019global_amd/csrc/gi_build.cpp
+++ b/2019global_amd/csrc/gi_build.cpp
@@ -456,6 +456,8 @@
     hs.x_skip_b = 2.0;
     for (XPrim& p : hs.xprims) p.pad[0] = kXNoPlane;
     for (XWNode& w : hs.xwnodes) memset(w.pad, 0xFF, sizeof w.pad);
+    hs.x_planes.clear();
+    hs.x_tau = 0.0;
     double E = 0.0;
     for (const XPrim& p : hs.xprims)
         for (int k = 0; k < 3; ++k) {
@@ -509,7 +511,10 @@
         tau = std::max(tau, dev);
         s_min = std::min(s_min, s);
     }
+    hs.x_ext = E;
     if (groups.empty()) return;
+    hs.x_tau = tau;
+    for (const G& g : groups) hs.x_planes.push_back(HostScene::XPlane{{g.n.x, g.n.y, g.n.z}, g.off});
     for (XWNode& w : hs.xwnodes) {
         uint8_t* b = reinterpret_cast<uint8_t*>(w.pad);
         for (int c = 0; c < 8; ++c) {
@@ -548,6 +553,66 @@
     }
     hs.x_flat_ok = ok && hs.xflat.size() <= (size_t)GI_XFLAT_MAX;
     hs.x_fan_all = !hs.xflat.empty() && (size_t)hs.n_fan_leaves == hs.xflat.size();
+    mark_boundary_leaves(hs);
+}
+
+void mark_boundary_leaves(HostScene& hs) {
+    hs.xflat_plane.assign(hs.xflat.size(), XLeafPlane{});
+    hs.x_dead_c = INFINITY;
+    if (!hs.x_flat_ok || hs.x_planes.empty()) return;
+    const double tau = hs.x_tau;
+    double s_all = 1.0;
+    std::vector<double> lo(hs.x_planes.size(), INFINITY), hi(hs.x_planes.size(), -INFINITY);
+    for (const XPrim& p : hs.xprims) {
+        V3 pts[8];
+        int npt = 0;
+        if (p.kind == 0) {
+            const V3 v0 = ld3(p.a), e1 = ld3(p.b), e2 = ld3(p.c), e3 = e2 - e1;
+            pts[0] = v0; pts[1] = v0 + e1; pts[2] = v0 + e2;
+            npt = 3;
+            const V3 cr = cross(e1, e2);
+            const double area2 = std::sqrt(dot(cr, cr)), l1 = std::sqrt(dot(e1, e1)), l2 = std::sqrt(dot(e2, e2)),
+                         l3 = std::sqrt(dot(e3, e3));
+            if (area2 > 0.0 && std::isfinite(area2))
+                s_all = std::min(s_all, std::min(std::min(area2 / (l1 * l2), area2 / (l1 * l3)), area2 / (l2 * l3)));
+        } else {
+            for (int k = 0; k < 8; ++k)
+                pts[k] = v3(p.a[0] + ((k & 1) ? p.b[0] : -p.b[0]), p.a[1] + ((k & 2) ? p.b[0] : -p.b[0]), p.a[2] + ((k & 4) ? p.b[0] : -p.b[0]));
+            npt = 8;
+        }
+        for (size_t g = 0; g < hs.x_planes.size(); ++g) {
+            const HostScene::XPlane& pl = hs.x_planes[g];
+            for (int k = 0; k < npt; ++k) {
+                const double h = dot(ld3(pl.n), pts[k]) - pl.c;
+                lo[g] = std::isnan(h) ? -INFINITY : std::min(lo[g], h);
+                hi[g] = std::isnan(h) ? INFINITY : std::max(hi[g], h);
+            }
+        }
+    }
+    bool any = false;
+    for (size_t k = 0; k < hs.xflat.size(); ++k) {
+        const int g = hs.xflat[k].group;
+        if (g == kXNoPlane || (size_t)g >= hs.x_planes.size()) continue;
+        XLeafPlane& r = hs.xflat_plane[k];
+        for (int a = 0; a < 3; ++a) r.n[a] = hs.x_planes[g].n[a];
+        r.c = hs.x_planes[g].c;
+        r.sides = (lo[g] >= -tau ? 1 : 0) | (hi[g] <= tau ? 2 : 0);
+        any = any || r.sides != 0;
+    }
+    if (!any || !(s_all > 0.0)) return;
+    const double K = 2000.0, u = 0x1.0p-53, tmin = 1e-7, E = hs.x_ext;
+    const double eps = 32.0 * u * E / s_all + tau;
+    hs.x_dead_c = K * (2.0 * eps + 4.0 * u * E / s_all) / tmin;
+}
+
+XShadowLeaves shadow_leaves_of(const HostScene& hs) {
+    XShadowLeaves sl;
+    if (!hs.x_flat_ok || hs.xflat_plane.size() != hs.xflat.size() || hs.xflat.size() > (size_t)GI_XFLAT_MAX) return sl;
+    sl.n = (int32_t)hs.xflat.size();
+    for (int k = 0; k < sl.n; ++k) sl.pl[k] = hs.xflat_plane[(size_t)k];
+    sl.dead_c = hs.x_dead_c;
+    sl.ext = hs.x_ext;
+    return sl;
 }
 
 bool build_host_scene(const gi_scene_desc& desc, HostScene& hs, std::string& err) {
diff --git a/2019global_amd/csrc/gi_capi.cpp b/2019global_amd/csrc/gi_capi.cpp
--- a/2019global_amd/csrc/gi_capi.cpp
+++ b/2019global_amd/csrc/gi_capi.cpp
@@ -502,6 +502,7 @@
             d.x_far_r = std::isinf(d.x_far_r) ? m : std::max(d.x_far_r, m);
         }
     if ((e = x_launch_config(d, device, s->xcfg)) != hipSuccess) return hip_fail(e, "occupancy query");
+    s->xcfg.shadow = shadow_leaves_of(s->host);
     *out = s.release();
     return GI_OK;
 }
@@ -722,6 +723,19 @@
     });
 }
 
+int gi_scene_shadow_leaves(gi_scene* s, const double* light, const double* cam_pos, uint32_t* boundary_mask, uint32_t* live_mask) {
+    return guard([&]() -> int {
+        if (!s || !light || !cam_pos || !boundary_mask || !live_mask) return fail(GI_ERR_ARG, "null argument");
+        std::lock_guard<std::mutex> lk(s->mu);
+        const XShadowLeaves& sl = s->xcfg.shadow;
+        const bool on = s->dev.x_flat != 0 && sl.n > 0;
+        *boundary_mask = on ? sl.boundary_mask() : 0u;
+        *live_mask = on ? (x_launch_live(s->dev, s->xcfg, v3(cam_pos[0], cam_pos[1], cam_pos[2]), v3(light[0], light[1], light[2]), 0u) & sl.table_mask())
+                        : 0u;
+        return GI_OK;
+    });
+}
+
 int gi_scene_seg_ring(gi_scene* s, const gi_opts* o, int32_t* on) {
     return guard([&]() -> int {
         if (!s || !o || !on) return fail(GI_ERR_ARG, "null argument");
diff --git a/2019global_amd/csrc/gi_kernels.hip b/2019global_amd/csrc/gi_kernels.hip
--- a/2019global_amd/csrc/gi_kernels.hip
+++ b/2019global_amd/csrc/gi_kernels.hip
@@ -963,7 +963,8 @@
         if (!xs.wcnt || (form == XFORM_WF && (!xs.wq[0] || !xs.wq[1] || xs.wcap <= 0))) return hipErrorInvalidValue;
         const bool seg = form == XFORM_SEG;
         const XKernelCfg c{xc.var, env.flat != 0, seg ? xc.seg_lds_bytes : xc.wf_lds_bytes, xc.wf_grid[seg ? WK_SEG : WK_BOUNCE]};
-        e = launch_wf(sc, c, form, cam, light, m.w, m.h, m.y0, o, rgb, rgb8, xs, sc.work + 1, stats ? st : nullptr, xf, stream,
+        e = launch_wf(sc, c, form, cam, light, m.w, m.h, m.y0, o, rgb, rgb8, xs, sc.work + 1, stats ? st : nullptr, xf,
+                      x_launch_live(sc, xc, cam.pos, light, o.flags), stream,
                       ev_begin, ev_end);
         if (e != hipSuccess) return e;
     } else {
diff --git a/2019global_amd/csrc/gi_launch.h b/2019global_amd/csrc/gi_launch.h
--- a/2019global_amd/csrc/gi_launch.h
+++ b/2019global_amd/csrc/gi_launch.h
@@ -57,7 +57,12 @@
 XKernelCfg x_query_cfg(const XLaunchCfg& xc, int flags, WfKernel k);
 hipError_t launch_wf(const DevScene& sc, const XKernelCfg& c, XForm form, const CamDev& cam, V3 light, int w, int h, int y0,
                      const gi_opts& o, double* rgb, uint8_t* rgb8, const XScratch& xs, const unsigned* n_list_dev,
-                     unsigned long long* stats, int xflags, hipStream_t stream, hipEvent_t ev_begin, hipEvent_t ev_end);
+                     unsigned long long* stats, int xflags, uint32_t live, hipStream_t stream, hipEvent_t ev_begin, hipEvent_t ev_end);
+inline uint32_t x_launch_live(const DevScene& sc, const XLaunchCfg& xc, V3 cam_pos, V3 light, unsigned flags) {
+    const double L[3] = {light.x, light.y, light.z}, C[3] = {cam_pos.x, cam_pos.y, cam_pos.z};
+    const bool full = !sc.x_flat || (flags & (GI_FLAG_X_NO_SHADOW | GI_FLAG_X_ALL_LEAVES)) != 0;
+    return x_shadow_live(xc.shadow, L, C, (double)sc.x_far_r, full);
+}
 hipError_t launch_x_query_kat(const DevScene& sc, const XKernelCfg& c, V3 cam_pos, int n, const double* recs, int32_t* oi,
                               double* od, hipStream_t stream);
 hipError_t launch_x_texel_kat(const DevScene& sc, XVariant var, int n, int mode, const double* recs, int32_t* oi, double* od,
diff --git a/2019global_amd/csrc/gi_scene.h b/2019global_amd/csrc/gi_scene.h
--- a/2019global_amd/csrc/gi_scene.h
+++ b/2019global_amd/csrc/gi_scene.h
@@ -123,6 +123,36 @@
     uint8_t fan;
 };
 static_assert(sizeof(XFlatLeaf) == 32, "XFlatLeaf layout");
+struct XLeafPlane {
+    double n[3], c;
+    int32_t sides;
+    int32_t pad;
+};
+struct XShadowLeaves {
+    int32_t n = 0;
+    XLeafPlane pl[GI_XFLAT_MAX] = {};
+    double dead_c = INFINITY;
+    double ext = 0.0;
+    double delta(const double* L) const {
+        const double lm = std::fmax(std::fabs(L[0]), std::fmax(std::fabs(L[1]), std::fabs(L[2])));
+        return dead_c * (1.7320508075688774 * (lm + ext));
+    }
+    uint32_t table_mask() const { return n >= 32 ? ~0u : (1u << n) - 1u; }
+    uint32_t boundary_mask() const {
+        uint32_t b = 0;
+        for (int k = 0; k < n; ++k) b |= pl[k].sides ? 1u << k : 0u;
+        return b;
+    }
+    uint32_t live_mask(const double* L) const {
+        const double dl = delta(L);
+        uint32_t live = table_mask();
+        for (int k = 0; k < n; ++k) {
+            const double s = (pl[k].n[0] * L[0] + pl[k].n[1] * L[1] + pl[k].n[2] * L[2]) - pl[k].c;
+            if (((pl[k].sides & 1) && s >= dl) || ((pl[k].sides & 2) && -s >= dl)) live &= ~(1u << k);
+        }
+        return live;
+    }
+};
 
 struct HostScene {
     std::vector<RNode> rnodes;
@@ -161,9 +191,22 @@
     bool x_flat_ok = false;
     int32_t n_fan_leaves = 0;
     bool x_fan_all = false;
+    struct XPlane { double n[3], c; };
+    std::vector<XPlane> x_planes;
+    double x_tau = 0.0, x_ext = 0.0;
+    std::vector<XLeafPlane> xflat_plane;
+    double x_dead_c = INFINITY;
 };
 bool build_host_scene(const gi_scene_desc& desc, HostScene& hs, std::string& err);
 void build_xflat(HostScene& hs);
+void mark_boundary_leaves(HostScene& hs);
+XShadowLeaves shadow_leaves_of(const HostScene& hs);
+inline uint32_t x_shadow_live(const XShadowLeaves& sl, const double* light, const double* cam_pos, double far_r, bool full) {
+    const double cm = std::fmax(std::fabs(cam_pos[0]), std::fmax(std::fabs(cam_pos[1]), std::fabs(cam_pos[2])));
+    if (full || sl.n == 0 || !(cm <= far_r)) return ~0u;
+    const uint32_t live = sl.live_mask(light);
+    return live == sl.table_mask() ? ~0u : live;
+}
 
 inline void finalize_xwnodes(std::vector<XWNode>& w) {
     for (XWNode& n : w) {
@@ -292,6 +335,7 @@
     size_t wf_lds_bytes = 0;
     size_t wf_tree_lds_bytes = 0;
     int wf_grid[WK_COUNT] = {};
+    XShadowLeaves shadow;
     bool seg_ring = false;
     size_t seg_lds_bytes = 0;
 };
diff --git a/2019global_amd/csrc/gi_wf.hip b/2019global_amd/csrc/gi_wf.hip
--- a/2019global_amd/csrc/gi_wf.hip
+++ b/2019global_amd/csrc/gi_wf.hip
@@ -192,7 +192,7 @@
 }
 template <bool ANY, bool TRI>
 __device__ __forceinline__ int wf_flat(float far_r, const XFlatLeaf* tab, const uint32_t* pkw, int n, const XHot* H, V3 o, V3 d, double tmax, bool act,
-                                       double& t_out, uint32_t& nnode, uint32_t& nprim, uint32_t& nsteps, int skip, bool fan) {
+                                       double& t_out, uint32_t& nnode, uint32_t& nprim, uint32_t& nsteps, int skip, bool fan, uint32_t live) {
     const F3 of = ray_org32(o, d, far_r);
     const F3 ivf = inv_dir(d);
     const F3 no = neg_oiv(of, ivf);
@@ -223,6 +223,33 @@
         }
     };
     int k0 = 0;
+    if (ANY && live != ~0u) {
+        uint32_t rem = live & (n >= 32 ? ~0u : (1u << n) - 1u);
+        int prev = -1;
+        auto sstep = [&](const u32x8 w, int k) {
+            m <<= (k - prev - 1) & 31;
+            step(w, k);
+            prev = k;
+        };
+        while (rem != 0) {
+            const int ka = __builtin_ctz(rem);
+            rem &= rem - 1;
+            const int kb = rem ? __builtin_ctz(rem) : -1;
+            rem &= rem - 1;
+            const int kc = rem ? __builtin_ctz(rem) : -1;
+            rem &= rem - 1;
+            const int kd = rem ? __builtin_ctz(rem) : -1;
+            rem &= rem - 1;
+            const u32x8 w0 = flat_rec_uniform(tab, ka), w1 = flat_rec_uniform(tab, kb < 0 ? ka : kb);
+            const u32x8 w2 = flat_rec_uniform(tab, kc < 0 ? ka : kc), w3 = flat_rec_uniform(tab, kd < 0 ? ka : kd);
+            sstep(w0, ka);
+            if (kb >= 0) sstep(w1, kb);
+            if (kc >= 0) sstep(w2, kc);
+            if (kd >= 0) sstep(w3, kd);
+        }
+        m <<= (n - 1 - prev) & 31;
+        k0 = n;
+    }
     for (; k0 + 4 <= n; k0 += 4) {
         const u32x8 w0 = flat_rec_uniform(tab, k0), w1 = flat_rec_uniform(tab, k0 + 1);
         const u32x8 w2 = flat_rec_uniform(tab, k0 + 2), w3 = flat_rec_uniform(tab, k0 + 3);
@@ -419,8 +446,9 @@
 }
 template <bool ANY, bool LDS, bool SH, bool TRI, bool CN, bool FLAT>
 __device__ __forceinline__ int x_query(const DevScene& sc, const WFView& v, float far_r, const V3& o, const V3& d, double tmax,
-                                       bool act, double& t_out, uint32_t& nnode, uint32_t& nprim, uint32_t& st_steps, int skip) {
-    if constexpr (FLAT) return wf_flat<ANY, TRI>(far_r, v.FT, v.FP, sc.n_xflat, v.LH, o, d, tmax, act, t_out, nnode, nprim, st_steps, skip, sc.x_fan != 0);
+                                       bool act, double& t_out, uint32_t& nnode, uint32_t& nprim, uint32_t& st_steps, int skip,
+                                       uint32_t live = ~0u) {
+    if constexpr (FLAT) return wf_flat<ANY, TRI>(far_r, v.FT, v.FP, sc.n_xflat, v.LH, o, d, tmax, act, t_out, nnode, nprim, st_steps, skip, sc.x_fan != 0, live);
     else if constexpr (LDS) return wf_trace<ANY, true, false, SH, TRI, false>(far_r, v.LW, v.LH, o, d, tmax, act, v.nst, t_out, nnode, nprim, st_steps, skip);
     else if constexpr (CN) return wf_trace<ANY, false, false, SH, TRI, true>(far_r, sc.xcnodes, sc.xhot, o, d, tmax, act, v.nst, t_out, nnode, nprim, st_steps);
     else return wf_trace<ANY, false, false, SH, TRI, true>(far_r, sc.xwnodes, sc.xhot, o, d, tmax, act, v.nst, t_out, nnode, nprim, st_steps, skip);
@@ -447,7 +475,7 @@
 __device__ __forceinline__ bool x_segment(const DevScene& sc, const WFView& v, const V3& light, int depth, bool no_shadow, bool act,
                                           const KeyF& id_of, V3& o, V3& d, V3& L, V3& T,
                                           uint32_t& nnode, uint32_t& nprim, uint32_t& nrays, WFSegStats& ws,
-                                          double skip_cos = 2.0, int* splane = nullptr, float far_r = INFINITY) {
+                                          double skip_cos = 2.0, int* splane = nullptr, float far_r = INFINITY, uint32_t live = ~0u) {
     uint32_t st_steps = 0;
     uint64_t c0 = STATS ? clock64() : 0;
     bool occl = false;
@@ -468,7 +496,7 @@
     if (!no_shadow) {
         double tdummy;
         const int skip_s = x_own_plane(h.pg, h.pn, Ld, skip_cos);
-        occl = x_query<true, LDS, SH, TRI, CN, FLAT>(sc, v, INFINITY, P, Ld, h.ldist, hit, tdummy, nnode, nprim, st_steps, skip_s) >= 0;
+        occl = x_query<true, LDS, SH, TRI, CN, FLAT>(sc, v, INFINITY, P, Ld, h.ldist, hit, tdummy, nnode, nprim, st_steps, skip_s, live) >= 0;
         if (STATS) wf_wave_steps(st_steps, ws.it_s, ws.ln_s);
     }
     if (STATS) {
@@ -536,7 +564,7 @@
 template <bool STATS, bool LDS, bool W4, bool SH, bool TRI, bool CN, bool FLAT>
 __global__ __launch_bounds__(256, (LDS && W4) ? GI_WF_MIN_WAVES_LDS : GI_WF_MIN_WAVES) void k_wf_bounce(
     DevScene sc, CamDev cam, V3 light, TileMap m, int spp, int depth, uint64_t seed, int b, double* rgb, uint8_t* rgb8,
-    unsigned long long* stats, WFArgs a, WFQ qin, WFQ qout, int xflags) {
+    unsigned long long* stats, WFArgs a, WFQ qin, WFQ qout, int xflags, uint32_t shadow_live) {
     unsigned n_in;
     if (b == 0) {
         const unsigned long long tot = (unsigned long long)*a.n_list * (unsigned long long)a.ns;
@@ -608,7 +636,7 @@
         const float far_r = ray_far_r(sc, cam.pos);
         int splane = 254;
         const bool cont = x_segment<false, LDS, SH, TRI, CN, FLAT>(sc, v, light, depth, no_shadow, act, [&] { return PathId{key, smp, b}; }, o, d, L, T,
-                                                             nnode, nprim, nrays, ws, skip_cos, &splane, far_r);
+                                                             nnode, nprim, nrays, ws, skip_cos, &splane, far_r, shadow_live);
         const unsigned long long mc = __ballot(cont);
         if (mc) {
             const int leader = __ffsll((long long)mc) - 1;
@@ -685,7 +713,7 @@
 template <bool STATS, bool LDS, bool W4, bool SH, bool TRI, bool CN, bool FLAT, bool RING>
 __global__ __launch_bounds__(256, (LDS && W4) ? GI_WF_MIN_WAVES_LDS : GI_WF_MIN_WAVES) void k_seg(
     DevScene sc, CamDev cam, V3 light, TileMap m, int spp, int depth, uint64_t seed, double* rgb, uint8_t* rgb8,
-    unsigned long long* stats, WFArgs a, int xflags) {
+    unsigned long long* stats, WFArgs a, int xflags, uint32_t shadow_live) {
     extern __shared__ int4 lds_dyn[];
     const WFView v = wf_stage<LDS, FLAT>(sc, lds_dyn);
     const bool no_shadow = (xflags & XF_NO_SHADOW) != 0;
@@ -805,7 +833,7 @@
         const bool cont = x_segment<STATS, LDS, SH, TRI, CN, FLAT>(
             sc, v, light, depth, no_shadow, live,
             [&] { return PathId{slot_get_u64(v.pl, 6), (unsigned)(slot_get_u64(v.pl, 7) >> 32), splane >> kSegPlaneBits}; },
-            o, d, L, T, nnode, nprim, nrays, ws, skip_cos, &splane, far_r);
+            o, d, L, T, nnode, nprim, nrays, ws, skip_cos, &splane, far_r, shadow_live);
         if (live) {
             if (cont) {
                 splane += 1 << kSegPlaneBits;
@@ -1115,7 +1143,7 @@
 
 hipError_t launch_wf(const DevScene& sc, const XKernelCfg& c, XForm form, const CamDev& cam, V3 light, int w, int h, int y0,
                      const gi_opts& o, double* rgb, uint8_t* rgb8, const XScratch& xs, const unsigned* n_list_dev,
-                     unsigned long long* stats, int xflags, hipStream_t stream, hipEvent_t ev_begin, hipEvent_t ev_end) {
+                     unsigned long long* stats, int xflags, uint32_t live, hipStream_t stream, hipEvent_t ev_begin, hipEvent_t ev_end) {
     const TileMap m = make_map(w, h, o.shard_count, o.shard_index, y0);
     const int depth = o.depth;
     const int s0 = o.sample_end > 0 ? o.sample_begin : 0, s1 = o.sample_end > 0 ? o.sample_end : o.spp;
@@ -1132,9 +1160,9 @@
         if (ev_begin) (void)hipEventRecord(ev_begin, stream);
         wf_dispatch(sc, c, stats != nullptr, [&](auto V) {
             if (xflags & XF_SEG_RING)
-                hipLaunchKernelGGL(seg_kernel<true>(V), grid, block, c.lds_bytes, stream, sc, cam, light, m, o.spp, depth, o.seed, rgb, rgb8, stats, a, xflags);
+                hipLaunchKernelGGL(seg_kernel<true>(V), grid, block, c.lds_bytes, stream, sc, cam, light, m, o.spp, depth, o.seed, rgb, rgb8, stats, a, xflags, live);
             else
-                hipLaunchKernelGGL(seg_kernel<false>(V), grid, block, c.lds_bytes, stream, sc, cam, light, m, o.spp, depth, o.seed, rgb, rgb8, stats, a, xflags);
+                hipLaunchKernelGGL(seg_kernel<false>(V), grid, block, c.lds_bytes, stream, sc, cam, light, m, o.spp, depth, o.seed, rgb, rgb8, stats, a, xflags, live);
         });
         if (ev_end) (void)hipEventRecord(ev_end, stream);
         return hipGetLastError();
@@ -1158,7 +1186,7 @@
             qout.r = xs.wq[b & 1];
             qout.id = reinterpret_cast<uint2*>(xs.wid[b & 1]);
             wf_dispatch(sc, c, stats != nullptr, [&](auto V) {
-                hipLaunchKernelGGL(bounce_kernel(V), grid, block, c.lds_bytes, stream, sc, cam, light, m, o.spp, depth, o.seed, b, rgb, rgb8, stats, a, qin, qout, xflags);
+                hipLaunchKernelGGL(bounce_kernel(V), grid, block, c.lds_bytes, stream, sc, cam, light, m, o.spp, depth, o.seed, b, rgb, rgb8, stats, a, qin, qout, xflags, live);
             });
         }
     }
diff --git a/include/gi.h b/include/gi.h
--- a/include/gi.h
+++ b/include/gi.h
@@ -8,7 +8,7 @@
 extern "C" {
 #endif
 
-#define GI_ABI_VERSION 18
+#define GI_ABI_VERSION 19
 
 typedef enum gi_status {
     GI_OK = 0,
@@ -67,6 +67,7 @@
 #define GI_FLAG_X_WF 16u
 #define GI_FLAG_X_MEGA 32u
 #define GI_FLAG_X_SEG 64u
+#define GI_FLAG_X_ALL_LEAVES 128u
 
 typedef struct gi_opts {
     int32_t mode;
@@ -237,6 +238,8 @@
 int gi_scene_kernel_ms(gi_scene* scene, float* avg_ms, int64_t* n);
 int gi_scene_x_form(gi_scene* scene, const gi_opts* opts, int32_t* form);
 int gi_scene_seg_ring(gi_scene* scene, const gi_opts* opts, int32_t* on);
+int gi_scene_shadow_leaves(gi_scene* scene, const double* light, const double* cam_pos, uint32_t* boundary_mask,
+                           uint32_t* live_mask);
 int gi_scene_r_kernel(gi_scene* scene, const gi_opts* opts, int32_t* kernel);
 
 typedef struct gi_octree gi_octree;
```

After: 38320, median of 6. 3.2% higher.
